# getanteon/alaz

Measured on AMD Instinct MI355X. Metric: L7 edge-events/s ingested->scored service-map, higher is better.
Workload: dtype u64; 1 GPU; C3 device-resident replay: 10000 pods / 5000 services / 1000000 edges, 10000000 HTTP l7 events per window already in HBM, 2-layer SAGE + MLP score, partitioned K1 (variant 0, 8-byte records, 512 partitions); 2-batch HBM ring (value excludes PCIe: see end_to_end with --full); events_per_window=10000000, layers=2, windows_in_flight=1, parallelism=1 GPU

## Files before the change

### alaz_amd/csrc/servicegraph.hip

```cpp
#include <hip/hip_runtime.h>
#include <hip/hip_ext.h>

#include <algorithm>
#include <cmath>
#include <cstdio>
#include <cstring>
#include <chrono>
#include <condition_variable>
#include <thread>
#include <mutex>
#include <string>
#include <unordered_map>
#include <vector>

#include <dlfcn.h>

#include "join_host.hpp"
#include "sg_plan.hpp"
#include "sg_kernels.h"
#include "sg_sel.h"
#include "sg_trend.h"
#include "sg_node_trend.h"
#include "sg_rank.h"
#include "sg_incident.h"
// ... 72 lines not shown

    sg_stats st{};
    u64 h_ctr[C_COUNT] = {};
    std::vector<u32> last_obips;
    bool warm_on = true;
    u32 cold_streak = 0;
    u32 kw_epoch = 0;
    u32 in_fused_slices = 0;
    u64 closes = 0; u32 timing_stride = 1;
    u32 obip_streak = 0; u64 plain_left = 0;

    unsigned timing = 0;
    hipEvent_t win_ta = nullptr;
    u32 k6_epoch = 0;
    u32 rp_epoch = 0;

    struct WinSlot {
        Dev d{}; hipStream_t stream = nullptr; u32* ob_list = nullptr; u32* ob_n = nullptr; u64 events_in = 0;
        bool closed = false, plain = false;
        u64 halo_ovf_seen = 0;
        u64* h_note = nullptr; u64 note_seen = 0;
        u64* scr_sum = nullptr; u64* scr_max = nullptr; double* scr_mu = nullptr;
    };
    std::vector<WinSlot> slots = std::vector<WinSlot>(1);
    int cur = 0;
    struct LastRun { int slot = -1; hipStream_t stream = nullptr; } last;
    std::vector<TimingRec> trecs;
    std::vector<hipEvent_t> ev_pool;
    struct Xchg { u32* ob_local = nullptr; u32* ob_all = nullptr; u32* req = nullptr; u32* serve = nullptr; float* rows_out = nullptr; float* rows_in = nullptr; u32 capp = 0, ob_stride = 0; } xc;
    struct SelScratch { sgplan::SelPlan plan; u32* keys = nullptr; u32* hist = nullptr; u32* blk = nullptr; u32* state = nullptr; u64* pairs = nullptr;
                        u64* n = nullptr; u64* h_n = nullptr; hipEvent_t ev = nullptr; bool pending = false; };
    struct Sel : SelScratch { sg_edge_out* stage = nullptr; u32* stage_idx = nullptr; u64 stage_cap = 0; } sel;
    template <class Row>
    struct Baseline { bool on = false; sg_trend_params p{}; sgplan::TrendPlan plan; char* mem = nullptr; TrendSoA buf[2] = {}; u64* ctl = nullptr;
                      u32* blk = nullptr; K8Thread* th = nullptr; std::vector<Row*> rows; std::vector<char> valid; u32 w = 0; hipEvent_t ev = nullptr;
                      bool pending = false; Row* stage = nullptr; u32* stage_idx = nullptr; u64 stage_cap = 0; };
    Baseline<sg_edge_trend> trend;
    struct Vanished { bool on = false; sg_vanished_params p{}; sgplan::VanishedPlan plan; char* mem = nullptr; u32* th = nullptr; u32* blk = nullptr;
                      std::vector<sg_edge_vanished*> rows; std::vector<u64*> count; std::vector<char> valid; } vanished;
    struct RollupState { bool on = false; char* mem = nullptr; u32* dst = nullptr; K9Side* tout = nullptr; K9Side* tin = nullptr;
                         K9Side* part = nullptr; u32* blk = nullptr; std::vector<sg_node_out*> rows; std::vector<u64*> count; std::vector<char> valid;
                         hipEvent_t ev = nullptr; bool pending = false; };
    template <class Plan>
    struct Rollup : RollupState { Plan plan; };
    Rollup<sgplan::NodesPlan> nodes;
    Baseline<sg_node_trend> ntrend;
    template <class Row>
    struct IdxSel : SelScratch { u64* ctr = nullptr; u32* idx = nullptr; Row* stage = nullptr; char* mem = nullptr; u64 stage_rows = 0; };
    using NSel = IdxSel<sg_node_out>;
    NSel nsel;
    struct RankState { bool on = false; sg_rank_params p{}; char* mem = nullptr; u32* pos = nullptr; u32* src = nullptr; u32* dst = nullptr;
                       u64* W = nullptr; u64* R = nullptr; u64* base = nullptr; u64* t = nullptr; u64* part = nullptr; u64* seed_sum = nullptr;
                       sg_node_rank* stage = nullptr; u32* stage_idx = nullptr; std::vector<sg_node_rank*> rows; std::vector<char> valid;
                       hipEvent_t ev = nullptr; bool pending = false; };
    template <class Plan>
    struct Rank : RankState { Plan plan; typename Plan::Weight* w = nullptr; };
    Rank<sgplan::RankPlan> rank;
    struct IncidentState { bool on = false; sg_incident_params p{}; char* mem = nullptr; u32* pos = nullptr; u32* parent = nullptr;
                           u32* flag = nullptr; u32* lab = nullptr; u32* num = nullptr; u32* kinc = nullptr; u32* esrc = nullptr;
                           K12Keys* keys = nullptr; u32* blk = nullptr; u32* stage = nullptr; u32* stage_idx = nullptr;
                           std::vector<sg_incident_out*> rows; std::vector<u64*> count; std::vector<u32*> node_inc; std::vector<char> valid;
                           hipEvent_t ev = nullptr; bool pending = false; };
    template <class Plan>
    struct Incidents : IncidentState { Plan plan; };
    Incidents<sgplan::IncidentPlan> inc;
    struct Tracks { bool on = false; sg_track_params p{}; sgplan::TrackPlan plan; char* mem = nullptr; u32* mtrack = nullptr; u32* mlast = nullptr;
                    sg_track_entry* tab[2] = {nullptr, nullptr}; TrkState* st[2] = {nullptr, nullptr}; u32 cur = 0; u64 w = 0;
                    u32* cand = nullptr; u32* kept = nullptr; u32* moved = nullptr; u32* joined = nullptr; u32* pos = nullptr; u32* tv = nullptr;
                    u64* claim = nullptr; u32* blk = nullptr; std::vector<sg_incident_track*> rows; std::vector<sg_track_entry*> ended;
                    std::vector<u64*> ended_count; std::vector<char> valid; hipEvent_t ev = nullptr; bool pending = false; };
    Tracks trk;
    struct Groups { bool on = false; sg_group_params p{}; sgplan::GroupPlan plan; char* mem = nullptr; u32* map = nullptr; void* keys[2] = {nullptr, nullptr};
                    u32* idx[2] = {nullptr, nullptr}; u32* hist = nullptr; u32* chunkcnt = nullptr; K14Acc* part = nullptr; uint2* meta = nullptr;
                    u32* blk = nullptr; u32* stage = nullptr; u32* stage_idx = nullptr; std::vector<sg_group_edge*> rows; std::vector<u64*> count;
                    std::vector<u32*> row_group, perm; std::vector<char> valid; hipEvent_t ev = nullptr; bool pending = false;
                    std::vector<u32> h_map; u32* h_up = nullptr; hipEvent_t up_ev = nullptr; bool up_pending = false; u32 dirty_lo = 0, dirty_hi = 0;
                    u32 hi_group = 0; } grp;
    Baseline<sg_edge_trend> gtrend;
    Vanished gvanished;
    IdxSel<sg_group_edge> gsel;
    Rollup<sgplan::GroupNodesPlan> gnodes;
    Baseline<sg_node_trend> gntrend;
    NSel gnsel;
    Rank<sgplan::GroupRankPlan> grank;
    Incidents<sgplan::GroupIncidentPlan> ginc;
    Tracks gtrk;
    struct QuantSpace { bool on = false; char* mem = nullptr; u32* pos = nullptr; u32* tgt[2] = {nullptr, nullptr}; u64* part = nullptr;
                        unsigned char* stage = nullptr; u32* stage_idx = nullptr; std::vector<u64*> hist; std::vector<u32*> quant;
                        std::vector<char> valid; hipEvent_t ev = nullptr; bool pending = false; };
    struct Quantiles { sgplan::QuantPlan plan; u32 n_q = 0; u32 qm[SG_Q_MAX] = {}; QuantSpace sp[3]; } qnt;
    struct QuantTrend { u32 qi = 0; Baseline<sg_node_trend> nodes; Baseline<sg_edge_trend> groups; Baseline<sg_node_trend> workloads; } qtr;
};

namespace {

sg_engine::WinSlot& work(sg_engine* e) { return e->slots[e->cur]; }
int ran_slot(const sg_engine* e) { return e->last.slot >= 0 ? e->last.slot : e->cur; }
sg_engine::WinSlot& ran(sg_engine* e) { return e->slots[ran_slot(e)]; }

#define HIP_TRY(e, call)                                                                       \
    do {                                                                                       \
        hipError_t _r = (call);                                                                \
        if (_r != hipSuccess) {                                                                \
            (e)->err = std::string(#call) + ": " + hipGetErrorString(_r);                      \
            return _r == hipErrorOutOfMemory ? SG_ENOMEM : SG_ENODEV;                          \
        }                                                                                      \
    } while (0)

template <typename T>
int dev_alloc(sg_engine* e, T** p, size_t n, int fill = 0) {
    void* q = nullptr;
    size_t bytes = std::max<size_t>(n, 1) * sizeof(T);
    constexpr size_t kArenaMax = (size_t)32 << 20, kArenaChunk = (size_t)256 << 20, kArenaAlign = 4096;
    if (e->plan.arena_on && bytes < kArenaMax) {
        const size_t need = (bytes + kArenaAlign - 1) & ~(kArenaAlign - 1);
        if (need > e->arena_left) {
            void* c = nullptr;
            HIP_TRY(e, hipMalloc(&c, kArenaChunk));
            e->allocs.push_back(c);
            e->arena_base = static_cast<char*>(c); e->arena_left = kArenaChunk;
        }
        q = e->arena_base; e->arena_base += need; e->arena_left -= need;
    } else {
        HIP_TRY(e, hipMalloc(&q, bytes));
        e->allocs.push_back(q);
    }
    HIP_TRY(e, hipMemsetAsync(q, fill, bytes, e->slots[0].stream));
    *p = (T*)q;
    return SG_OK;
}

hipStream_t pick(sg_engine* e, void* s) { return s ? (hipStream_t)s : work(e).stream; }
hipStream_t pick_ran(sg_engine* e, void* s) { return s ? (hipStream_t)s : e->last.slot >= 0 ? e->last.stream : work(e).stream; }

hipEvent_t get_event(sg_engine* e) {
    if (!e->ev_pool.empty()) { hipEvent_t v = e->ev_pool.back(); e->ev_pool.pop_back(); return v; }
    hipEvent_t v; hipEventCreate(&v); return v;
}

struct Timed {
    sg_engine* e; hipStream_t s; TimingRec r; bool on;
    Timed(sg_engine* e_, hipStream_t s_, int kernel) : e(e_), s(s_), on(e_ && ((e_->timing >> kernel) & 1u)) {
        if (on) { r.kernel = kernel; r.a = get_event(e); r.b = get_event(e); hipEventRecord(r.a, s); }
    }
    ~Timed() { if (on) { hipEventRecord(r.b, s); e->trecs.push_back(r); } }
};

static_assert(sgplan::kK1bWarmU == K1B_WARM_U, "sg_plan.hpp's copy of pass B's warm U");
constexpr int k4_threads(int fi, bool proj, bool split) { return split ? (proj ? 512 : 256) : (fi == 32 ? 1024 : 512); }
template <class FnT, const auto& Keys> struct Family { typedef FnT Fn; static constexpr auto& keys = Keys; };
struct K1aWide : Family<K1aFn, sgplan::kK1aWideKeys> { template <size_t I> static Fn at() { constexpr auto k = keys[I]; return k1a_partition<(bool)k[0], (bool)k[1], (bool)k[2]>; } };
struct K1aTile : Family<K1aFn, sgplan::kK1aTileKeys> { template <size_t I> static Fn at() { constexpr auto k = keys[I]; return k1a_tile_partition<k[0], (bool)k[1], k[2]>; } };
struct K1aTeam : Family<K1aFn, sgplan::kK1aTeamKeys> { template <size_t I> static Fn at() { constexpr auto k = keys[I]; return k1a_team_partition<k[0], (bool)k[1], 2, 1024, k[2]>; } };
struct K1bMerge : Family<K1bFn, sgplan::kK1bMergeKeys> { template <size_t I> static Fn at() {
    constexpr auto k = keys[I]; if constexpr (k[2]) return k1b_merge<k[0], (bool)k[1]>; else return k1b_merge_wide<k[0], (bool)k[1]>; } };
struct K1bStream : Family<K1bFn, sgplan::kK1bStreamKeys> { template <size_t I> static Fn at() {
    constexpr auto k = keys[I]; if constexpr (k[4]) return k1b_stream_merge<k[0], k[1], (bool)k[2], k[3]>; else return k1b_stream_merge_wide<k[0], k[1], (bool)k[2], k[3]>; } };
struct K4Layer : Family<K4LayerFn, sgplan::kK4LayerKeys> { template <size_t I> static Fn at() {
    constexpr auto k = keys[I]; return k4_sage_layer<k[0], (bool)k[1], (bool)k[2], k4_threads(k[0], k[2], k[3]), (bool)k[3]>; } };
constexpr K2RowptrFn kK2Rowptr[2] = {k2_rowptr<K2_RP_ROWS, false>, k2_rowptr<K2_RP_ROWS_DH, true>};
constexpr K4GatherFn kK4Gather[2] = {k4_gather<32>, k4_gather<64>};
constexpr K5ProjFn kK5Proj[2] = {k5_node_proj<false>, k5_node_proj<true>};
constexpr K5ScoreFn kK5Score[2] = {k5_edge_score<false>, k5_edge_score<true>};
template <class F, size_t... I>
const std::array<typename F::Fn, sizeof...(I)>& kernel_table(std::index_sequence<I...>) {
    static const std::array<typename F::Fn, sizeof...(I)> t{{F::template at<I>()...}};
    return t;
}
template <class F> const auto& kernel_table() { return kernel_table<F>(std::make_index_sequence<F::keys.size()>{}); }
template <class F, class... A>
typename F::Fn kernel_of(bool& ok, A... args) {
    const int i = sgplan::find_key(F::keys, sgplan::Key<sizeof...(A)>{{(int)args...}});
    if (i < 0) ok = false;
    return i < 0 ? nullptr : kernel_table<F>()[i];
}
template <class... K>
hipError_t lds_limit(size_t bytes, K... kernels) {
    for (const void* f : {reinterpret_cast<const void*>(kernels)...}) {
        const hipError_t r = hipFuncSetAttribute(f, hipFuncAttributeMaxDynamicSharedMemorySize, (int)bytes);
        if (r != hipSuccess) return r;
    }
    return hipSuccess;
}
template <class F>
hipError_t lds_limit_all(size_t bytes) { hipError_t r = hipSuccess; for (const auto f : kernel_table<F>()) if (r == hipSuccess) r = lds_limit(bytes, f); return r; }

int plan_pass_a(sg_engine* e) {
    sgplan::PassA pa = e->pa;
    if (!sgplan::plan_pass_a(e->plan, e->jt.l1_entries, e->jt.blocks_bytes(), e->ov, &pa)) { e->err = "K1 pass A: the join tables' level 1 and the piece counters do not fit a CU's LDS (fewer partitions / IP blocks needed)"; return SG_ENOSPC; }
    const sgplan::PassAKernel k = sgplan::choose_pass_a(e->plan, pa, e->cfg);
    bool ok = true;
    const K1aFn f = k.family == sgplan::K1A_TEAM ? kernel_of<K1aTeam>(ok, k.l2, k.sharded, k.pb)
                  : k.family == sgplan::K1A_TILE ? kernel_of<K1aTile>(ok, k.l2, k.sharded, k.nsub) : kernel_of<K1aWide>(ok, k.l2, k.sharded, k.hist);
    if (!ok) { e->err = "K1 pass A: the library holds no kernel for family " + std::to_string(k.family) + ", level 2 mode " + std::to_string(k.l2); return SG_ENODEV; }
    e->pa = pa; e->kn.k1a = k; e->fn.k1a = f;
    return SG_OK;
}
int resolve_kernels(sg_engine* e) {
    const sgplan::Kernels& k = e->kn;
    sg_engine::Fns& f = e->fn;
    bool ok = true;
    if (k.k1b_family == sgplan::K1B_STREAM) {
        f.k1b = kernel_of<K1bStream>(ok, k.k1b_u, k.k1b_spt, k.k1b_pack, 0, k.k1b_share);
        if (k.k1b_warm) f.k1b_try = kernel_of<K1bStream>(ok, sgplan::kK1bWarmU, k.k1b_spt, k.k1b_pack, 1, k.k1b_share);
        if (k.k1b_warm) f.k1b_cold = kernel_of<K1bStream>(ok, sgplan::kK1bWarmU, k.k1b_spt, k.k1b_pack, 2, k.k1b_share);
    } else if (k.k1b_family == sgplan::K1B_MERGE) f.k1b = kernel_of<K1bMerge>(ok, k.k1b_u, k.k1b_hist, k.k1b_share);
    f.k2_rowptr = kK2Rowptr[k.k2_dh]; f.k5_proj = kK5Proj[k.k5_mfma];
    for (int w = 0; w < 2; w++) for (int pj = 0; pj < 2; pj++) f.k4_layer[w][pj] = kernel_of<K4Layer>(ok, w ? 64 : 32, k.k4_mfma, pj, k.k4_split);
    if (!ok) { e->err = "the library holds no kernel for one of the plan's choices (sg_plan.hpp choose_kernels)"; return SG_ENODEV; }
    return SG_OK;
}


void join_view(const sg_engine* e, Dev& d) {
    d.jl1mask = e->jt.l1_entries - 1;
    d.jl2_words = e->jt.use_blocks ? e->jt.blocks_used * 256u : 0u;
    d.ck_n = e->jt.ck_n;
    d.jstage_bytes = (u32)((size_t)e->jt.l1_entries * 8 + (e->pa.l2_in_lds ? e->jt.blocks_bytes() : 0));
    d.jl2_in_lds = e->pa.l2_in_lds ? 1u : 0u;
    d.k1a_ct = e->pa.k1a_ct;
}

int sync_tables(sg_engine* e, hipStream_t s) {
    sgjoin::Table& jt = e->jt;
    if (!jt.need_full && jt.dirty.empty()) return SG_OK;
    for (hipStream_t ks : e->k1_streams) if (ks != s) { HIP_TRY(e, hipEventRecord(e->k1_ev, ks)); HIP_TRY(e, hipStreamWaitEvent(s, e->k1_ev, 0)); }
    e->k1_streams.clear();
    if (jt.rebuilds == 0 && !jt.rebuild()) { e->err = "join table build failed: raise max_ips"; return SG_ENOSPC; }
    if (jt.need_full) {
        HIP_TRY(e, hipEventSynchronize(e->blob_ev));
        std::memcpy(e->h_blob, jt.blob, (size_t)jt.L.words * 4);
        HIP_TRY(e, hipMemcpyAsync(e->d_blob, e->h_blob, (size_t)jt.L.words * 4, hipMemcpyHostToDevice, s));
        HIP_TRY(e, hipEventRecord(e->blob_ev, s));
        jt.uploaded_full();
        e->st.join_full_uploads++;
    } else {
        std::vector<std::pair<u32, u32>> log;
        jt.take_dirty(log);
        std::unordered_map<u32, u32> last;
        last.reserve(log.size() * 2);
        for (auto& kv : log) last[kv.first] = kv.second;
        const int slot = e->upd_next; e->upd_next = (slot + 1) % kUpdSlots;
        HIP_TRY(e, hipEventSynchronize(e->upd_ev[slot]));
        u32 n = 0;
        for (auto& kv : last) e->h_upd[slot][n++] = make_uint2(kv.first, kv.second);
        HIP_TRY(e, hipMemcpyAsync(e->d_upd[slot], e->h_upd[slot], (size_t)n * sizeof(uint2), hipMemcpyHostToDevice, s));
        hipLaunchKernelGGL(k_join_apply, dim3((n + 255) / 256), dim3(256), 0, s, e->d_blob, (const uint2*)e->d_upd[slot], n);
        HIP_TRY(e, hipEventRecord(e->upd_ev[slot], s));
        e->st.join_word_updates += n;
    }
    HIP_TRY(e, hipEventRecord(e->tab_ev, s));
    e->tab_seq++; e->tab_stream = s;
    return e->plan.variant == 0 ? plan_pass_a(e) : SG_OK;
}
int order_after_tables(sg_engine* e, hipStream_t s) {
    if (e->tab_seq) {
        u64* seen = nullptr;
        for (auto& kv : e->seen_seq) if (kv.first == s) seen = &kv.second;
        if (!seen) { e->seen_seq.push_back({s, 0}); seen = &e->seen_seq.back().second; }
        if (*seen != e->tab_seq) { if (e->tab_stream != s) HIP_TRY(e, hipStreamWaitEvent(s, e->tab_ev, 0)); *seen = e->tab_seq; }
    }
    if (std::find(e->k1_streams.begin(), e->k1_streams.end(), s) == e->k1_streams.end()) e->k1_streams.push_back(s);
    return SG_OK;
}

void rotate_window(sg_engine* e) { e->cur = (e->cur + 1) % (int)e->slots.size(); }

int launch_k1(sg_engine* e, const sg_event* d_ev, size_t n, hipStream_t s) {
    if (n == 0) return SG_OK;
    sg_engine::WinSlot& w = work(e);
    const size_t kMaxHist = (size_t)65535 * 256;
    if (w.d.hist && w.d.variant == 0 && n > kMaxHist) {
        for (size_t o = 0; o < n; o += kMaxHist) { const int rc = launch_k1(e, d_ev + o, std::min(kMaxHist, n - o), s); if (rc) return rc; }
        return SG_OK;
    }
    const size_t kMaxTeam = (size_t)1 << 25;
    if (w.d.variant == 0 && w.d.narrow && e->pa.k1a_team && n > kMaxTeam) {
        for (size_t o = 0; o < n; o += kMaxTeam) { const int rc = launch_k1(e, d_ev + o, std::min(kMaxTeam, n - o), s); if (rc) return rc; }
        return SG_OK;
    }
    int rc = sync_tables(e, s);
    if (rc) return rc;
    if ((rc = order_after_tables(e, s))) return rc;
    if (((e->timing >> 10) & 1u) && w.events_in == 0 && !e->win_ta) { e->win_ta = get_event(e); hipEventRecord(e->win_ta, s); }
    Dev da = w.d;
    join_view(e, da);
    u32 rot0 = w.d.k1a_rot, tb0 = w.d.k1a_ticket_base;
    if (w.d.variant == 0) {
        const bool tk = ((e->timing >> 1) & 1u) && e->closes % e->timing_stride == 0;
        hipEvent_t ta = tk ? get_event(e) : nullptr, tb = tk ? get_event(e) : nullptr;
        da.batch_state = w.events_in == 0 ? 1u : 0u;
        da.k1a_rot = w.d.k1a_rot;
        rot0 = w.d.k1a_rot; tb0 = w.d.k1a_ticket_base;
        if (w.d.narrow && !e->pa.k1a_team) {
            const u64 per = (n + w.d.nwg - 1) / w.d.nwg, chunk = per >= 4096 ? 4096 : (per + 1023) / 1024 * 1024;
            w.d.k1a_rot = (u32)((w.d.k1a_rot + (n + chunk - 1) / chunk) % w.d.nwg);
        }
        if (w.d.narrow && e->pa.k1a_team) {
            w.d.k1a_rot = (u32)((w.d.k1a_rot + k1m_tiles(n, w.d.nwg, e->pa.k1a_teams, e->pa.k1a_nt)) % ((u64)e->pa.k1a_teams * w.d.nwg));
            da.k1a_ticket_base = w.d.k1a_ticket_base;
            {
                const unsigned long long nt_ = k1m_tiles(n, w.d.nwg, e->pa.k1a_teams, e->pa.k1a_nt), units_ = (unsigned long long)e->pa.k1a_teams * w.d.nwg;
                if (!(w.d.ablate & 0x4u)) w.d.k1a_ticket_base += (u32)((nt_ > units_ ? nt_ - units_ : 0) + std::min(units_, nt_));
            }
        }
        const u32 threads = !w.d.narrow ? K1A_THREADS : e->pa.k1a_team ? 1024 : K1T_THREADS;
        hipExtLaunchKernelGGL(e->fn.k1a, dim3(w.d.nwg), dim3(threads), (uint32_t)e->pa.k1a_lds, s, ta, tb, 0u, da, d_ev, (u64)n);
        if (tk) { TimingRec r; r.a = ta; r.b = tb; r.kernel = 1; e->trecs.push_back(r); }
    } else {
        Timed t(e, s, 1);
        u64 want = (n + 255) / 256;
        int grid = (int)std::min<u64>(want, (u64)e->plan.k1_grid);
        hipLaunchKernelGGL(k1_resolve_aggregate, dim3(grid), dim3(256), 0, s, da, d_ev, (u64)n);
    }
    {
        const hipError_t lr = hipGetLastError();
        if (lr != hipSuccess) {
            w.d.k1a_rot = rot0; w.d.k1a_ticket_base = tb0;
            e->err = std::string("K1 pass A launch: ") + hipGetErrorString(lr);
            return lr == hipErrorOutOfMemory ? SG_ENOMEM : SG_ENODEV;
        }
    }
    e->st.events_in += n;
    w.events_in += n;
    return SG_OK;
}

int table_upsert(sg_engine* e, bool svc, u32 ip, u32 node_id, uint8_t kind) {
    if (node_id >= e->cfg.max_known_nodes) { e->err = "node_id beyond max_known_nodes"; return SG_ENOSPC; }
    auto& m = svc ? e->jt.svc_ip : e->jt.pod_ip;
    if (m.find(ip) == m.end() && e->jt.pod_ip.size() + e->jt.svc_ip.size() >= e->cfg.max_ips) { e->err = "join table full (max_ips)"; return SG_ENOSPC; }
    if (!e->jt.upsert(svc, ip, node_id)) { e->err = "join table build failed: raise max_ips"; return SG_ENOSPC; }
    e->jt.set_kind(node_id, kind);
    e->n_known = std::max(e->n_known, node_id + 1);
    return SG_OK;
}

size_t weights_count(u32 L) {
    size_t n = 0;
    for (u32 l = 0; l < L; l++) n += 2 * (size_t)(l == 0 ? SG_F_IN : SG_F_HID) * SG_F_HID + SG_F_HID;
    return n + 2 * SG_F_HID * SG_F_HID + SG_F_EDGE * SG_F_HID + SG_F_HID + SG_F_HID + 1;
}
size_t layer_offset(u32 l) {
    size_t n = 0;
    for (u32 k = 0; k < l; k++) n += 2 * (size_t)(k == 0 ? SG_F_IN : SG_F_HID) * SG_F_HID + SG_F_HID;
    return n;
}

void launch_halo_lists(sg_engine* e, hipStream_t s, u32* req, u32 capp) {
    sg_engine::WinSlot& w = work(e);
    if (e->plan.k6_one_wg) {
        if (w.d.ncap <= K6_FLAGS_LDS) hipLaunchKernelGGL(k6_halo_build_padded<true>, dim3(1), dim3(1024), 0, s, w.d, req, capp);
        else hipLaunchKernelGGL(k6_halo_build_padded<false>, dim3(1), dim3(1024), 0, s, w.d, req, capp);
        return;
    }
    hipLaunchKernelGGL(k6_halo_lists, dim3(((size_t)w.d.ncap + 1023) / 1024), dim3(1024), 0, s, w.d, req, capp, ++e->k6_epoch, 1u);
}
int do_close(sg_engine* e, hipStream_t s, const u32* d_union, const u32* d_union_n, u32 ob_mode = 1, u32 stride = 0, u32 gworld = 0, bool fuse_in = false) {
    sg_engine::WinSlot& w = work(e);
    int rc = sync_tables(e, s);
    if (rc) return rc;
    Dev dloc = w.d;
    if (dloc.warm && w.h_note) {
        volatile u64* note = w.h_note;
        const u64 seq = note[0];
        if (seq != w.note_seen) {
            w.note_seen = seq;
            const u64 v = note[1];
            const u32 cold = (u32)(v & 0xFFu); const bool obip = (v & 0x100ull) != 0;
            e->cold_streak = cold == 2 ? e->cold_streak + 1 : 0;
            e->obip_streak = (cold == 1 && obip) ? e->obip_streak + 1 : 0;
            if (e->cold_streak >= 3) { e->plain_left = 32; e->cold_streak = 0; }
            if (e->obip_streak >= 4) { e->plain_left = 64; e->obip_streak = 0; }
        }
    }
    if (dloc.warm && e->plain_left) { e->plain_left--; dloc.warm = 0; }
    w.plain = w.d.warm && !dloc.warm;
    const u32 par = w.d.k1b_par & 1u;
    if (e->plan.prepare_fold && dloc.k1b_order) { dloc.k1b_cnt += (size_t)par * dloc.np; dloc.k1b_order += (size_t)par * dloc.np; }
    const Dev& d = dloc;
    bool warm_try = d.warm && e->warm_on;
    const u32 wt = warm_try ? 1u : 0u;
    const bool fold = sgplan::close_folds(e->plan, d.warm != 0, warm_try, ob_mode);
    if (!fold) {
        Timed tp(e, s, 2);
        if (ob_mode == 1) hipLaunchKernelGGL(kc_prepare, dim3(1), dim3(1024), 0, s, d, (u64)e->n_known, (u64)e->n_labels_decl, w.ob_list, (const u32*)w.ob_n, e->plan.ob_list_cap, 1u, (const u32*)nullptr, 0u, 0u, wt);
        else if (ob_mode == 0) hipLaunchKernelGGL(kc_prepare, dim3(1), dim3(1024), 0, s, d, (u64)e->n_known, (u64)e->n_labels_decl, const_cast<u32*>(d_union), d_union_n, e->plan.ob_list_cap, 0u, (const u32*)nullptr, 0u, 0u, wt);
        else hipLaunchKernelGGL(kc_prepare, dim3(1), dim3(1024), 0, s, d, (u64)e->n_known, (u64)e->n_labels_decl, w.ob_list, (const u32*)w.ob_n, e->plan.ob_list_cap, 2u, d_union, stride, gworld, wt);
    }
    if (d.variant == 0) {
        const bool tk = ((e->timing >> 7) & 1u) && e->closes % e->timing_stride == 0;
        hipEvent_t ta = tk ? get_event(e) : nullptr, tb = tk ? get_event(e) : nullptr;
        Dev db = d; db.batch_state = w.events_in == 0 ? 2u : 0u;
        db.kept_compact = d.warm;
        const dim3 grid(d.narrow ? d.npb : d.np), block(e->plan.k1b_threads);
        if (d.warm && warm_try) {
            Dev dt = db; dim3 gt = grid;
            if (fold) {
                dt.fold = 1u; dt.warm_try = wt; gt.x += 1;
                dt.pf_n_known = (u64)e->n_known; dt.pf_n_labels_decl = (u64)e->n_labels_decl; dt.pf_list = w.ob_list; dt.pf_list_cap = e->plan.ob_list_cap;
                dt.k1b_cnt_prev = w.d.k1b_order ? w.d.k1b_cnt + (size_t)(par ^ 1u) * d.np : nullptr;
                dt.k1b_order_next = w.d.k1b_order ? w.d.k1b_order + (size_t)(par ^ 1u) * d.np : nullptr;
            }
            hipExtLaunchKernelGGL(e->fn.k1b_try, gt, block, (uint32_t)e->plan.k1b_lds, s, ta, tb, 0u, dt);
            if (tk) { TimingRec r; r.a = ta; r.b = tb; r.kernel = 7; e->trecs.push_back(r); ta = get_event(e); tb = get_event(e); }
        }
        hipExtLaunchKernelGGL(d.warm ? e->fn.k1b_cold : e->fn.k1b, grid, block, (uint32_t)e->plan.k1b_lds, s, ta, tb, 0u, db);
        if (tk) { TimingRec r; r.a = ta; r.b = tb; r.kernel = 7; e->trecs.push_back(r); }
    }
    {
        Timed t(e, s, 2);
        Dev dk = d;
        dk.kept_compact = d.warm;
        if (d.warm) {
            dk.rowptr = d.k_rowptr; dk.col = d.k_col; dk.csr_from = d.k_from; dk.acc_csr = d.k_acc; dk.max_edges = (u64)d.npb * d.pcap;
            dk.st_sum = w.scr_sum; dk.st_max = w.scr_max; dk.row_mu = w.scr_mu; dk.row_sd = w.scr_mu + d.ncap + 1;
        }
        if (d.variant == 1) {
            const u32 ntiles = e->plan.ecap / K2_TILE;
            hipLaunchKernelGGL(k2_edge_count, dim3(ntiles), dim3(256), 0, s, d);
            hipLaunchKernelGGL(k2_scan_tiles, dim3(1), dim3(1024), 0, s, d, ntiles);
            hipLaunchKernelGGL(k2_edge_compact, dim3(ntiles), dim3(256), 0, s, d);
        }
        if (d.dh_g) hipLaunchKernelGGL(k2_deg_hist, dim3(d.dh_g), dim3(K2_DH_THREADS), ((size_t)d.ncap + 1) * sizeof(u32), s, dk);
        const size_t rpr = d.dh_g ? K2_RP_ROWS_DH : K2_RP_ROWS;
        hipLaunchKernelGGL(e->fn.k2_rowptr, dim3(((size_t)d.ncap + rpr) / rpr), dim3(1024), 0, s, dk, ++e->rp_epoch);
        if (d.variant == 1) hipLaunchKernelGGL(k2_scatter_table, dim3(grid_for(e->cfg.max_edges, 256)), dim3(256), 0, s, d);
        else hipLaunchKernelGGL(k2_scatter_parts, dim3(d.npb), dim3(256), 0, s, dk);
        hipLaunchKernelGGL(k2_rowsort_gather, dim3(std::max(2, std::min(4096, 2 * K2_LONG_WGS + grid_for(d.ncap, 8)))), dim3(256), 2 * (size_t)d.k2_sortw * sizeof(u32), s, dk);
        if (d.warm) {
            const unsigned kg = (unsigned)(((u64)d.npb * d.pcap + KW_CH - 1) / KW_CH) + KW_CAPW;
            hipLaunchKernelGGL(kw_compact, dim3(kg), dim3(KW_THREADS), (size_t)KW_ROWS * 5 * sizeof(u64), s, d, ++e->kw_epoch, dk.st_sum, dk.st_max, (u64)(e->closes + 1), e->slots.size() > 1 ? 1u : 0u);
        }
    }
    {
        Timed t3(e, s, 8);
        const u32 fin = d.warm ? (u32)std::min<u64>(64, ((u64)d.ncap + 255) / 256) : 1u;
        if (fuse_in && e->plan.k3_fuse_allowed) {
            const u32 finp = d.warm ? (fin + 3) / 4 : 1u;
            hipLaunchKernelGGL(k3_in_part, dim3(e->plan.k3_ranges * e->plan.k3_slices + finp), dim3(1024), e->plan.k3in_lds, s, d, e->plan.k3_slices, finp);
            e->in_fused_slices = e->plan.k3_slices;
        } else {
            hipLaunchKernelGGL(k3_in_part, dim3(e->plan.k3_ranges * e->plan.k3_slices), dim3(1024), e->plan.k3in_lds, s, d, e->plan.k3_slices, 0u);
            hipLaunchKernelGGL(k3_in_reduce, dim3(grid_for((u64)d.ncap * 6, 256, 1024) + fin), dim3(256), 0, s, d, e->plan.k3_slices, fin);
            e->in_fused_slices = 0;
        }
    }
    HIP_TRY(e, hipGetLastError());
    w.closed = true;
    w.events_in = 0;
    e->closes++;
    if (e->plan.prepare_fold) w.d.k1b_par ^= 1u;
    return SG_OK;
}

int do_features(sg_engine* e, hipStream_t s) {
    const Dev& d = work(e).d;
    Timed t(e, s, 3);
    const int nbn = grid_for(d.ncap, 128), nbe = grid_for(e->cfg.max_edges, 256, 4096);
    hipLaunchKernelGGL(k3_node_features, dim3(nbn + nbe), dim3(256), 0, s, d, (u32)nbn, e->in_fused_slices);
// ... 1217 lines not shown
    return copy_counted(e, x.count[e->cur], x.rows[e->cur], sizeof(sg_incident_out), out, cap, n);
}
int node_incident_read(sg_engine* e, const NodeSpace& ns, const char* call, const uint32_t* node_index, size_t n_index, uint32_t* out, size_t cap, size_t* n) {
    const sg_engine::IncidentState& x = *ns.inc;
    if (const int rc = stage_ready(e, x, call, ns.inc_w)) return rc;
    u64 cnt = 0;
    HIP_TRY(e, hipMemcpy(&cnt, ns.roll->count[e->cur], sizeof(u64), hipMemcpyDeviceToHost));
    const std::string beyond = std::string(call) + ": a node index beyond the window's " + ns.rows_of;
    return copy_indexed(e, (const u32*)x.node_inc[e->cur], (size_t)cnt, node_index, n_index, out, cap, n, x.stage, x.stage_idx,
                        std::max<size_t>(ns.cap, 1), beyond.c_str());
}
int incidents_buffer(sg_engine* e, const NodeSpace& ns, const char* call, void** d_incidents, void** d_count, void** d_node_incident) {
    const sg_engine::IncidentState& x = *ns.inc;
    int slot;
    if (const int rc = stage_slot(e, x, call, ns.inc_w, &slot)) return rc;
    *d_incidents = x.rows[slot]; *d_count = x.count[slot]; *d_node_incident = x.node_inc[slot];
    return SG_OK;
}
template <class MakePlan>
int tracks_set(sg_engine* e, const NodeSpace& ns, const char* call, const sg_track_params* p, u32 ncap, MakePlan plan) {
    if (!ns.inc->on) { e->err = std::string(call) + ": " + ns.inc_w.off; return SG_ESTATE; }
    if (e->closing || e->flush_open) { e->err = std::string(call) + " while a flush is open"; return SG_ESTATE; }
    sg_track_params q{};
    if (p && sgplan::check_tracks(*p, ncap, &q)) { e->err = std::string(call) + ": bad parameters"; return SG_EINVAL; }
    sg_engine::Tracks& x = *ns.trk;
    free_stage(x);
    if (!p) return SG_OK;
    const u32 slots = (u32)e->slots.size();
    x.p = q;
    x.plan = plan(q.max_tracks, slots);
    const sgplan::TrackPlan& P = x.plan;
    HIP_TRY(e, hipEventCreateWithFlags(&x.ev, hipEventDisableTiming));
    if (const int rc = alloc_block(e, &x.mem, P.total_bytes, call, [&x] { free_stage(x); })) return rc;
    x.mtrack = at<u32>(x.mem, P.member_off[0]); x.mlast = at<u32>(x.mem, P.member_off[1]);
    for (int k = 0; k < 2; k++) { x.tab[k] = at<sg_track_entry>(x.mem, P.table_off[k]); x.st[k] = at<TrkState>(x.mem, P.state_off[k]); }
    x.cand = at<u32>(x.mem, P.inc_off[0]); x.kept = at<u32>(x.mem, P.inc_off[1]); x.moved = at<u32>(x.mem, P.inc_off[2]);
    x.joined = at<u32>(x.mem, P.inc_off[3]); x.pos = at<u32>(x.mem, P.inc_off[4]); x.tv = at<u32>(x.mem, P.inc_off[5]);
    x.claim = at<u64>(x.mem, P.claim_off);
    x.blk = at<u32>(x.mem, P.blk_off);
    for (u32 k = 0; k < slots; k++) {
        char* s = x.mem + P.slot.off + k * P.slot.bytes;
        x.rows.push_back(at<sg_incident_track>(s, P.slot_rows)); x.ended.push_back(at<sg_track_entry>(s, P.slot_ended));
        x.ended_count.push_back(at<u64>(s, P.slot_count));
    }
    hipError_t rc = hipMemset(x.mtrack, 0xFF, P.member_bytes);
    if (rc == hipSuccess) rc = hipDeviceSynchronize();
    if (rc != hipSuccess) { free_stage(x); e->err = std::string(call) + ": hipMemset: " + hipGetErrorString(rc); return SG_ENODEV; }
    x.valid.assign(slots, 0);
    x.on = true;
    return SG_OK;
}
int tracks_read(sg_engine* e, const NodeSpace& ns, const char* call, sg_incident_track* out, size_t cap, size_t* n) {
    const sg_engine::Tracks& x = *ns.trk;
    if (const int rc = stage_ready(e, x, call, ns.trk_w)) return rc;
    return copy_counted(e, ns.inc->count[e->cur], x.rows[e->cur], sizeof(sg_incident_track), out, cap, n);
}
int tracks_ended(sg_engine* e, const NodeSpace& ns, const char* call, sg_track_entry* out, size_t cap, size_t* n) {
    const sg_engine::Tracks& x = *ns.trk;
    if (const int rc = stage_ready(e, x, call, ns.trk_w)) return rc;
    return copy_counted(e, x.ended_count[e->cur], x.ended[e->cur], sizeof(sg_track_entry), out, cap, n);
}
int tracks_buffer(sg_engine* e, const NodeSpace& ns, const char* call, void** d_tracks, void** d_ended, void** d_ended_count) {
    const sg_engine::Tracks& x = *ns.trk;
    int slot;
    if (const int rc = stage_slot(e, x, call, ns.trk_w, &slot)) return rc;
    *d_tracks = x.rows[slot]; *d_ended = x.ended[slot]; *d_ended_count = x.ended_count[slot];
    return SG_OK;
}
int track_state(sg_engine* e, const NodeSpace& ns, const char* call, TrkState* st) {
    sg_engine::Tracks& x = *ns.trk;
    if (!x.on) { e->err = std::string(call) + ": " + ns.trk_w.off; return SG_ESTATE; }
    if (x.pending) HIP_TRY(e, hipEventSynchronize(x.ev));
    HIP_TRY(e, hipMemcpy(st, x.st[x.cur], sizeof(TrkState), hipMemcpyDeviceToHost));
    return SG_OK;
}
int track_entries(sg_engine* e, const NodeSpace& ns, const char* call, sg_track_entry* out, size_t cap, size_t* n) {
    TrkState st{};
    if (const int rc = track_state(e, ns, call, &st)) return rc;
    const sg_engine::Tracks& x = *ns.trk;
    if (n) *n = st.n;
    const size_t take = std::min((size_t)st.n, cap);
    if (out && take) HIP_TRY(e, hipMemcpy(out, x.tab[x.cur], take * sizeof(sg_track_entry), hipMemcpyDeviceToHost));
    return SG_OK;
}
int track_stats(sg_engine* e, const NodeSpace& ns, const char* call, sg_track_stats* out) {
    TrkState st{};
    if (const int rc = track_state(e, ns, call, &st)) return rc;
    out->windows = ns.trk->w; out->live = st.n; out->opened = st.opened; out->dropped_cap = st.dropped;
    return SG_OK;
}
}

extern "C" {

uint32_t sg_abi_version(void) { return SG_ABI_VERSION; }
size_t sg_weights_count(uint32_t layers) { return weights_count(layers); }
uint32_t sg_hash32(uint32_t x) { return sg_fmix32(x); }

const char* sg_last_error(sg_handle h) { return h ? h->err.c_str() : "null handle"; }

int sg_create(const sg_config* cfg_in, sg_handle* out) {
    if (!cfg_in || !out) return SG_EINVAL;
    *out = nullptr;
    sg_config c;
    if (const int rc = sgplan::check_config(*cfg_in, &c)) return rc;
    const sg_config* cfg = &c;
    int ndev = 0;
    if (hipGetDeviceCount(&ndev) != hipSuccess || ndev <= 0 || cfg->device < 0 || cfg->device >= ndev) return SG_ENODEV;
    hipDeviceProp_t prop;
    if (hipGetDeviceProperties(&prop, cfg->device) != hipSuccess) return SG_ENODEV;
    if (std::strncmp(prop.gcnArchName, "gfx950", 6) != 0) return SG_ENODEV;
    sg_engine* e = new sg_engine();
    e->cfg = *cfg;
    auto fail = [&](int rc) { std::fprintf(stderr, "sg_create: %s\n", e->err.c_str()); sg_destroy(e); return rc; };
#define CR(call) do { int _rc = (call); if (_rc) return fail(_rc); } while (0)
#define CH(call) do { hipError_t _r = (call); if (_r != hipSuccess) { e->err = std::string(#call) + ": " + hipGetErrorString(_r); return fail(_r == hipErrorOutOfMemory ? SG_ENOMEM : SG_ENODEV); } } while (0)
#ifdef SG_DEV_KNOBS
    e->ov = sgplan::from_env();
#endif
    sgplan::DeviceFacts facts;
    facts.cus = prop.multiProcessorCount; facts.lds_bytes = kLdsBytes;
    CR(sgplan::make_plan(*cfg, facts, e->ov, &e->plan, &e->err));
    const sgplan::Plan& P = e->plan;
    CH(hipSetDevice(cfg->device));
    e->slots.resize(P.n_slots);
    CH(hipStreamCreateWithFlags(&e->slots[0].stream, hipStreamNonBlocking));
    CH(hipEventCreateWithFlags(&e->tab_ev, hipEventDisableTiming));

    Dev base{}; Dev& d = base;
    sgplan::plan_to_dev(P, *cfg, d);
    const u64 ME = cfg->max_edges;
    {
        const sgjoin::Layout L = sgjoin::Table::make_layout(cfg->max_ips, cfg->max_known_nodes, P.max_blocks);
        e->jt_mirror.assign(L.words, 0);
        e->jt.init(L, e->jt_mirror.data(), d.variant == 0);
        e->jt.max_dirty = kUpdCap;
        CR(dev_alloc(e, &e->d_blob, L.words));
        CH(hipHostMalloc((void**)&e->h_blob, (size_t)L.words * 4));
        CH(hipEventCreateWithFlags(&e->blob_ev, hipEventDisableTiming));
        CH(hipEventCreateWithFlags(&e->k1_ev, hipEventDisableTiming));
        for (int i = 0; i < kUpdSlots; i++) {
            CH(hipHostMalloc((void**)&e->h_upd[i], (size_t)2 * kUpdCap * sizeof(uint2)));
            CR(dev_alloc(e, &e->d_upd[i], (size_t)2 * kUpdCap));
            CH(hipEventCreateWithFlags(&e->upd_ev[i], hipEventDisableTiming));
        }
        d.jl1 = reinterpret_cast<const u64*>(e->d_blob + L.off_l1);
        d.jl2 = e->d_blob + L.off_l2;
        d.iptab = reinterpret_cast<const u64*>(e->d_blob + L.off_ck); d.ipmask = L.ipcap - 1;
        d.iptab2 = reinterpret_cast<const u64*>(e->d_blob + L.off_ck2); d.ipmask2 = L.ip2cap - 1;
        d.kind = reinterpret_cast<const uint8_t*>(e->d_blob + L.off_kind);
    }
    if (d.variant == 0) {
        CR(plan_pass_a(e));
        CH(lds_limit_all<K1aWide>(kLdsBytes)); CH(lds_limit_all<K1aTile>(kLdsBytes)); CH(lds_limit_all<K1aTeam>(kLdsBytes));
        CH(lds_limit_all<K1bMerge>(P.k1b_lds)); CH(lds_limit_all<K1bStream>(P.k1b_lds));
        CH(lds_limit((size_t)KW_ROWS * 5 * sizeof(u64), kw_compact));
    }
    e->kn = sgplan::choose_kernels(P, e->pa, *cfg);
    CR(resolve_kernels(e));
    CH(lds_limit(2 * (size_t)d.k2_sortw * sizeof(u32), k2_rowsort_gather));
    if (d.dh_g) CH(lds_limit(((size_t)d.ncap + 1) * sizeof(u32), k2_deg_hist));
    CH(lds_limit(P.k3in_lds, k3_in_part));
    CR(dev_alloc(e, &d.dbg, (size_t)4 * 4096 * 8));
    CR(dev_alloc(e, &d.clk, (size_t)4));
    CR(dev_alloc(e, &e->d_W, weights_count(cfg->layers)));
    d.W = e->d_W;
    {
        float* tab = nullptr;
        CR(dev_alloc(e, &tab, (size_t)SG_L1P_TAB));
        hipLaunchKernelGGL(k_l1p_table, dim3((SG_L1P_TAB + 255) / 256), dim3(256), 0, e->slots[0].stream, tab);
        CH(hipStreamSynchronize(e->slots[0].stream));
        d.l1p_tab = tab;
    }
    auto alloc_window = [&](sg_engine::WinSlot& slot) -> int {
        Dev& w = slot.d;
#define LR(call) do { int _rc = (call); if (_rc) return _rc; } while (0)
        size_t eslots = ME;
        if (w.variant == 0) {
            eslots = std::max<size_t>(ME, (size_t)w.npb * w.pcap);
            if (w.narrow) { LR(dev_alloc(e, &w.slab8, (size_t)w.np * w.nwg * w.punits)); LR(dev_alloc(e, &w.hdr8, (size_t)w.np * w.nwg));
                            if (P.k1b_order) {
                                const size_t halves = P.prepare_fold ? 2 : 1;
                                LR(dev_alloc(e, &w.k1b_cnt, halves * w.np)); LR(dev_alloc(e, &w.k1b_order, halves * w.np));
                                std::vector<u32> ident(halves * w.np);
                                for (size_t i = 0; i < ident.size(); i++) ident[i] = (u32)(i % w.np);
                                HIP_TRY(e, hipStreamSynchronize(e->slots[0].stream));
                                HIP_TRY(e, hipMemcpy(w.k1b_order, ident.data(), ident.size() * sizeof(u32), hipMemcpyHostToDevice));
                            } }
            else { LR(dev_alloc(e, &w.slab_s, (size_t)w.np * w.nwg * w.pslots)); LR(dev_alloc(e, &w.hdr, (size_t)w.np * w.nwg)); }
            LR(dev_alloc(e, &w.ovf, (size_t)w.ovf_cap * 9));
            LR(dev_alloc(e, &w.ovf_p, (size_t)w.ovf_cap));
            LR(dev_alloc(e, &w.part_n, w.npb));
            LR(dev_alloc(e, &w.acc_src, (size_t)w.npb * w.pcap * 4));
            LR(dev_alloc(e, &w.e_rank, (size_t)w.npb * w.pcap));
            if (w.dh_g) LR(dev_alloc(e, &w.dh_hist, (size_t)w.dh_g * w.dh_ns));
            if (w.warm) {
                const size_t KC = (size_t)w.npb * w.pcap;
                LR(dev_alloc(e, &w.wk_keys, (size_t)w.npb * w.k1b_ht, 0xFF)); LR(dev_alloc(e, &w.wk_pos, (size_t)w.npb * w.k1b_ht, 0xFF));
                LR(dev_alloc(e, &w.pos_of_slot, KC, 0xFF));
                LR(dev_alloc(e, &w.k_acc, KC * 4)); LR(dev_alloc(e, &w.k_col, KC)); LR(dev_alloc(e, &w.k_from, KC)); LR(dev_alloc(e, &w.k_rowptr, (size_t)w.ncap + 2));
                LR(dev_alloc(e, &w.kw_tot, (KC + KW_CH - 1) / KW_CH + 2));
                LR(dev_alloc(e, &w.k_col2, KC)); LR(dev_alloc(e, &w.k_from2, KC)); LR(dev_alloc(e, &w.k_rowptr2, (size_t)w.ncap + 2));
                LR(dev_alloc(e, &w.k_slot, 2 * KC));
                LR(dev_alloc(e, &w.dc_rowptr, (size_t)w.ncap + 2)); LR(dev_alloc(e, &w.dc_col, KC)); LR(dev_alloc(e, &w.dc_from, KC)); LR(dev_alloc(e, &w.dc_acc, KC * 4));
                LR(dev_alloc(e, &w.dc_slot, KC)); LR(dev_alloc(e, &w.dc_ip, KC)); LR(dev_alloc(e, &w.dl_img, KC));
                LR(dev_alloc(e, &w.deg2, ((size_t)w.ncap + 1) * SG_DEG_REP * SG_DEG_STRIDE));
                LR(dev_alloc(e, &slot.scr_sum, (size_t)w.ncap * SG_NODE_STAT_SUM_WORDS)); LR(dev_alloc(e, &slot.scr_max, (size_t)w.ncap * SG_NODE_STAT_MAX_WORDS)); LR(dev_alloc(e, &slot.scr_mu, 2 * ((size_t)w.ncap + 1)));
                void* dn = nullptr;
                HIP_TRY(e, hipHostMalloc((void**)&slot.h_note, 64, hipHostMallocMapped));
                slot.h_note[0] = slot.h_note[1] = 0;
                HIP_TRY(e, hipHostGetDevicePointer(&dn, slot.h_note, 0));
                w.host_note = (u64*)dn;
            }
        }
        const size_t KE = P.kept_edges;
        LR(dev_alloc(e, &w.ekeys, P.ecap, 0xFF));
        LR(dev_alloc(e, &w.eacc, (size_t)P.ecap * 4));
        if (w.variant == 1) w.acc_src = w.eacc;
        LR(dev_alloc(e, &w.obkeys, P.obcap));
        LR(dev_alloc(e, &w.wgstat, (size_t)SG_MAX_K1_WGS * WS_WORDS));
        LR(dev_alloc(e, &w.ctr, C_COUNT));
        LR(dev_alloc(e, &w.ob_sorted, w.max_obip));
        LR(dev_alloc(e, &slot.ob_list, P.ob_list_cap));
        LR(dev_alloc(e, &slot.ob_n, 4));
        LR(dev_alloc(e, &w.tile_cnt, P.ecap / K2_TILE));
        LR(dev_alloc(e, &w.tile_off, P.ecap / K2_TILE));
        LR(dev_alloc(e, &w.e_slot, ME)); LR(dev_alloc(e, &w.e_from, eslots)); LR(dev_alloc(e, &w.e_to, eslots));
        LR(dev_alloc(e, &w.longrows, (size_t)w.ncap + 1));
        LR(dev_alloc(e, &w.deg, ((size_t)w.ncap + 1) * SG_DEG_REP * SG_DEG_STRIDE)); LR(dev_alloc(e, &w.rp_tot, ((size_t)w.ncap + K2_RP_ROWS_DH) / K2_RP_ROWS_DH + 1)); LR(dev_alloc(e, &w.k6_tot, (((size_t)w.ncap + 1023) / 1024 + 1) * 16)); LR(dev_alloc(e, &w.k1a_ticket, 4)); LR(dev_alloc(e, &w.lb_ticket, 4)); w.k1a_ticket_base = 0; w.k1a_rot = 0; LR(dev_alloc(e, &w.rowptr, (size_t)w.ncap + 1)); LR(dev_alloc(e, &w.cursor, (size_t)w.ncap + 1));
        LR(dev_alloc(e, &w.col, ME)); LR(dev_alloc(e, &w.cs, KE)); LR(dev_alloc(e, &w.csr_from, ME));
        LR(dev_alloc(e, &w.sort_k, 2 * KE)); LR(dev_alloc(e, &w.sort_v, 2 * KE));
        LR(dev_alloc(e, &w.acc_csr, ME * 4));
        if (w.hist) { LR(dev_alloc(e, &w.hist_src, (w.variant == 0 ? (size_t)w.npb * w.pcap : (size_t)P.ecap) * SG_HIST_BINS)); LR(dev_alloc(e, &w.hist_csr, ME * SG_HIST_BINS)); }
        LR(dev_alloc(e, &w.st_sum, (size_t)w.ncap * SG_NODE_STAT_SUM_WORDS)); LR(dev_alloc(e, &w.st_max, (size_t)w.ncap * SG_NODE_STAT_MAX_WORDS));
        LR(dev_alloc(e, &w.x0, (size_t)w.ncap * SG_F_IN));
        for (u32 l = 1; l <= cfg->layers; l++) LR(dev_alloc(e, &w.h[l], (size_t)w.ncap * SG_F_HID));
        LR(dev_alloc(e, &w.P, (size_t)w.ncap * SG_F_HID)); LR(dev_alloc(e, &w.Q, (size_t)w.ncap * SG_F_HID));
        LR(dev_alloc(e, &w.nmean, (size_t)w.ncap * SG_F_HID));
        LR(dev_alloc(e, &w.hub_items, w.hub_cap)); LR(dev_alloc(e, &w.hub_base, (size_t)w.ncap + 1)); LR(dev_alloc(e, &w.hub_part, (size_t)w.hub_cap * SG_F_HID));
        LR(dev_alloc(e, &w.efeat, ME * SG_F_EDGE)); LR(dev_alloc(e, &w.latz, ME)); LR(dev_alloc(e, &w.errr, ME));
        LR(dev_alloc(e, &w.row_mu, (size_t)w.ncap + 1)); LR(dev_alloc(e, &w.row_sd, (size_t)w.ncap + 1));
        LR(dev_alloc(e, &w.rows, ME));
        LR(dev_alloc(e, &w.in_part, (size_t)P.k3_ranges * P.k3_slices * K3_IN_NR * 6));
        LR(dev_alloc(e, &w.alive_keys, w.alive_cap)); LR(dev_alloc(e, &w.alive_csr, KE));
        LR(dev_alloc(e, &w.act_l, (size_t)w.ncap + 1)); LR(dev_alloc(e, &w.act_p, (size_t)w.ncap + 1));
        std::vector<u64> init((size_t)SG_MAX_K1_WGS * WS_WORDS, 0);
        for (int i = 0; i < SG_MAX_K1_WGS; i++) init[(size_t)i * WS_WORDS + WS_TMIN] = ~0ull;
        HIP_TRY(e, hipMemcpy(w.wgstat, init.data(), init.size() * sizeof(u64), hipMemcpyHostToDevice));
#undef LR
        return SG_OK;
    };
    CH(hipStreamSynchronize(e->slots[0].stream));
    for (sg_engine::WinSlot& slot : e->slots) {
        slot.d = base;
        if (!slot.stream) CH(hipStreamCreateWithFlags(&slot.stream, hipStreamNonBlocking));
        CR(alloc_window(slot));
    }
    CH(hipStreamCreateWithFlags(&e->copy_stream, hipStreamNonBlocking)); CH(hipStreamCreateWithFlags(&e->copy_stream2, hipStreamNonBlocking));
    CH(hipStreamCreateWithFlags(&e->rd_stream, hipStreamNonBlocking)); CH(hipEventCreateWithFlags(&e->score_ev, hipEventDisableTiming));
    CH(hipHostMalloc((void**)&e->h_ctr_pin, sizeof(e->h_ctr)));
    for (int i = 0; i < P.n_stage; i++) {
        CH(hipEventCreateWithFlags(&e->copied_ev[i], hipEventDisableTiming));
        CH(hipHostMalloc((void**)&e->h_stage[i], (size_t)e->cfg.max_batch * sizeof(sg_event)));
        CR(dev_alloc(e, &e->d_stage[i], e->cfg.max_batch));
        CH(hipEventCreateWithFlags(&e->stage_ev[i], hipEventDisableTiming));
    }
    CH(hipDeviceSynchronize());
#undef CR
#undef CH
    *out = e;
    return SG_OK;
}

int sg_destroy(sg_handle e) {
    if (!e) return SG_EINVAL;
    hipDeviceSynchronize();
    for (sg_engine::WinSlot& w : e->slots) { if (w.stream) hipStreamDestroy(w.stream); if (w.h_note) hipHostFree(w.h_note); }
    for (void* p : e->allocs) hipFree(p);
    if (e->h_blob) hipHostFree(e->h_blob);
    for (int i = 0; i < kUpdSlots; i++) { if (e->h_upd[i]) hipHostFree(e->h_upd[i]); if (e->upd_ev[i]) hipEventDestroy(e->upd_ev[i]); }
    if (e->blob_ev) hipEventDestroy(e->blob_ev);
    if (e->k1_ev) hipEventDestroy(e->k1_ev);
    for (int i = 0; i < kStageSlots; i++) { if (e->h_stage[i]) hipHostFree(e->h_stage[i]); if (e->stage_ev[i]) hipEventDestroy(e->stage_ev[i]); if (e->copied_ev[i]) hipEventDestroy(e->copied_ev[i]); }
    for (auto& r : e->registered) hipHostUnregister(const_cast<char*>(r.first));
    if (e->copy_stream) hipStreamDestroy(e->copy_stream);
    if (e->copy_stream2) hipStreamDestroy(e->copy_stream2);
    if (e->rd_stream) hipStreamDestroy(e->rd_stream);
    if (e->score_ev) hipEventDestroy(e->score_ev);
    for (auto& r : e->w_readers) hipEventDestroy(r.second);
    if (e->h_ctr_pin) hipHostFree(e->h_ctr_pin);
    if (e->h_rows) hipHostFree(e->h_rows);
    if (e->h_rows_old) hipHostFree(e->h_rows_old);
    if (e->sel.stage) hipFree(e->sel.stage);
    if (e->sel.stage_idx) hipFree(e->sel.stage_idx);
    if (e->sel.h_n) hipHostFree(e->sel.h_n);
    if (e->sel.ev) hipEventDestroy(e->sel.ev);
    free_edge_trend(edge_space(e));
    free_nodes(e);
    free_groups(e);
    free_idxsel(e->nsel);
    free_idxsel(e->gsel);
    for (auto& r : e->trecs) { hipEventDestroy(r.a); hipEventDestroy(r.b); }
    for (auto v : e->ev_pool) hipEventDestroy(v);
    if (e->tab_ev) hipEventDestroy(e->tab_ev);
    delete e;
    return SG_OK;
}

int sg_geometry_get(sg_handle e, sg_geometry* out) {
    if (!e || !out) return SG_EINVAL;
    std::lock_guard<std::mutex> g(e->mu);
    const sgplan::Plan& p = e->plan; const sgplan::PassA& a = e->pa;
    out->k1_variant = p.variant; out->k1_narrow = p.narrow; out->partitions = p.np; out->table_slots = p.k1b_ht; out->pass_b_split = p.k1b_split;
    out->pass_a_workgroups = p.nwg; out->cache_slots = a.k1a_ct; out->join_l2_in_lds = a.l2_in_lds ? (p.narrow && a.l2_u16 ? 2u : 1u) : 0u;
    out->tile_records = p.narrow ? (a.k1a_team ? 4u * a.k1a_nt / a.k1a_teams : K1T_TS(a.k1a_nsub)) : 0u; out->pass_a_teams = p.narrow && a.k1a_team ? a.k1a_teams : 0u; out->endpoint_bits = p.narrow ? p.nb : 0u;
    out->piece_bytes = p.variant != 0 ? 0u : (p.narrow ? p.punits * 8u : p.pslots * 16u);
    out->warm_windows = p.warm;
    return SG_OK;
}

int sg_prepare_fold_get(sg_handle e, uint32_t* out) {
    if (!e || !out) return SG_EINVAL;
    std::lock_guard<std::mutex> g(e->mu);
    *out = e->plan.prepare_fold ? 1u : 0u;
    return SG_OK;
}

int sg_upsert_pod(sg_handle e, uint32_t ip, uint32_t node_id) {
    if (!e) return SG_EINVAL;
    std::lock_guard<std::mutex> g(e->mu);
    return table_upsert(e, false, ip, node_id, SG_NODE_POD);
}
int sg_upsert_service(sg_handle e, uint32_t ip, uint32_t node_id) {
    if (!e) return SG_EINVAL;
    std::lock_guard<std::mutex> g(e->mu);
    return table_upsert(e, true, ip, node_id, SG_NODE_SERVICE);
}
int sg_delete_pod(sg_handle e, uint32_t ip) {
    if (!e) return SG_EINVAL;
    std::lock_guard<std::mutex> g(e->mu);
    if (!e->jt.erase(false, ip)) { e->err = "join table rebuild failed"; return SG_ENOSPC; }
    return SG_OK;
}
int sg_delete_service(sg_handle e, uint32_t ip) {
    if (!e) return SG_EINVAL;
    std::lock_guard<std::mutex> g(e->mu);
    if (!e->jt.erase(true, ip)) { e->err = "join table rebuild failed"; return SG_ENOSPC; }
    return SG_OK;
}

int sg_set_clock(sg_handle e, uint64_t first_kernel_ns, uint64_t first_user_ns) {
    if (!e) return SG_EINVAL;
    std::lock_guard<std::mutex> g(e->mu);
    e->first_kernel = first_kernel_ns; e->first_user = first_user_ns;
    return SG_OK;
}

int sg_set_label_count(sg_handle e, uint32_t n_labels) {
    if (!e) return SG_EINVAL;
    std::lock_guard<std::mutex> g(e->mu);
    if (n_labels > e->cfg.max_labels) { e->err = "label count beyond max_labels"; return SG_ENOSPC; }
    e->n_labels_decl = std::max(e->n_labels_decl, n_labels);
    return SG_OK;
}

int sg_load_weights(sg_handle e, const float* w, size_t n) {
    if (!e || !w) return SG_EINVAL;
    std::lock_guard<std::mutex> g(e->mu);
    if (n != weights_count(e->cfg.layers)) { e->err = "weight count mismatch"; return SG_EINVAL; }
    for (auto& r : e->w_readers) HIP_TRY(e, hipEventSynchronize(r.second));
    for (auto& r : e->w_readers) hipEventDestroy(r.second);
    e->w_readers.clear();
    HIP_TRY(e, hipMemcpy(e->d_W, w, n * sizeof(float), hipMemcpyHostToDevice));
    e->have_w = true;
    return SG_OK;
}

namespace {
int stage_take(sg_engine* e) {
    for (int k = 0; k < e->plan.n_stage; k++) {
        const int c = (e->stage_next + k) % e->plan.n_stage;
        if (!e->stage_busy[c] && hipEventQuery(e->stage_ev[c]) != hipErrorNotReady) { e->stage_busy[c] = true; e->stage_next = (c + 1) % e->plan.n_stage; e->pending_copies++; return c; }
    }
    return -1;
}
hipStream_t stage_stream(sg_engine* e) { return (e->plan.n_copy == 2 && (e->copy_rr++ & 1)) ? e->copy_stream2 : e->copy_stream; }
int stage_finish(sg_engine* e, int slot, size_t n, hipStream_t cs, bool copy_ok) {
    sg_engine::WinSlot& w = work(e);
    int rc = SG_OK;
    if (!copy_ok) { e->err = "hipMemcpyAsync (staging ring)"; rc = SG_ENODEV; }
    if (rc == SG_OK) {
        hipEventRecord(e->copied_ev[slot], cs);
        hipStreamWaitEvent(w.stream, e->copied_ev[slot], 0);
        e->st.h2d_bytes += n * sizeof(sg_event);
        rc = launch_k1(e, e->d_stage[slot], n, w.stream);
    }
    hipEventRecord(e->stage_ev[slot], w.stream);
    e->stage_busy[slot] = false; e->pending_copies--;
    e->cv.notify_all();
    return rc;
}
int stage_submit(sg_engine* e, int slot, const sg_event* src, size_t n) {
    hipStream_t cs = stage_stream(e);
    const bool ok = hipMemcpyAsync(e->d_stage[slot], src, n * sizeof(sg_event), hipMemcpyHostToDevice, cs) == hipSuccess;
    return stage_finish(e, slot, n, cs, ok);
}
constexpr size_t kStagePiece = ((size_t)4 << 20) / sizeof(sg_event);
}

int sg_ingest(sg_handle e, const sg_event* events, size_t n) {
    if (!e || (!events && n)) return SG_EINVAL;
    std::unique_lock<std::mutex> g(e->mu);
    if (n > e->cfg.max_batch) { e->err = "batch larger than max_batch"; return SG_EINVAL; }
    if (n == 0) return SG_OK;
    if (e->closing) { e->st.ingest_waits++; e->cv.wait(g, [&] { return !e->closing; }); }
    const int slot = stage_take(e);
    if (slot < 0) {
        e->st.events_dropped_ring += n;
        return SG_EAGAIN;
    }
    hipStream_t cs = stage_stream(e);
    g.unlock();
    bool ok = true;
    for (size_t o = 0; o < n && ok; o += kStagePiece) {
        const size_t m = std::min(kStagePiece, n - o);
        std::memcpy(e->h_stage[slot] + o, events + o, m * sizeof(sg_event));
        ok = hipMemcpyAsync(e->d_stage[slot] + o, e->h_stage[slot] + o, m * sizeof(sg_event), hipMemcpyHostToDevice, cs) == hipSuccess;
    }
    g.lock();
    return stage_finish(e, slot, n, cs, ok);
}

int sg_ingest_pinned(sg_handle e, const sg_event* events, size_t n) {
    if (!e || (!events && n)) return SG_EINVAL;
    std::unique_lock<std::mutex> g(e->mu);
    if (n > e->cfg.max_batch) { e->err = "batch larger than max_batch"; return SG_EINVAL; }
    if (n == 0) return SG_OK;
    {
        const char* p = reinterpret_cast<const char*>(events);
        bool ok = false;
        for (auto& r : e->registered) ok |= p >= r.first && p + n * sizeof(sg_event) <= r.first + r.second;
        if (!ok) { e->err = "sg_ingest_pinned: the events are not inside memory registered with sg_host_register"; return SG_EINVAL; }
    }
    if (e->closing) { e->st.ingest_waits++; e->cv.wait(g, [&] { return !e->closing; }); }
    const int slot = stage_take(e);
    if (slot < 0) { e->st.events_dropped_ring += n; return SG_EAGAIN; }
    return stage_submit(e, slot, events, n);
}
int sg_ingest_bulk(sg_handle e, const sg_event* events, size_t n, int pinned, uint64_t* retries) {
    if (!e || (!events && n)) return SG_EINVAL;
    const size_t step = e->cfg.max_batch;
    uint64_t waits = 0;
    for (size_t o = 0; o < n; o += step) {
        const size_t m = std::min(step, n - o);
        for (;;) {
            const int rc = pinned ? sg_ingest_pinned(e, events + o, m) : sg_ingest(e, events + o, m);
            if (rc == SG_OK) break;
            if (rc != SG_EAGAIN) { if (retries) *retries = waits; return rc; }
            { std::lock_guard<std::mutex> g(e->mu); e->st.events_dropped_ring -= m; }
            waits++;
            std::this_thread::sleep_for(std::chrono::microseconds(20));
        }
    }
    if (retries) *retries = waits;
    return SG_OK;
}
int sg_host_register(sg_handle e, void* p, size_t bytes) {
    if (!e || !p || !bytes) return SG_EINVAL;
    std::lock_guard<std::mutex> g(e->mu);
    if (hipHostRegister(p, bytes, hipHostRegisterDefault) != hipSuccess) { e->err = "hipHostRegister failed"; return SG_ENOMEM; }
    e->registered.push_back({reinterpret_cast<const char*>(p), bytes});
    return SG_OK;
}
int sg_host_unregister(sg_handle e, void* p) {
    if (!e || !p) return SG_EINVAL;
    std::lock_guard<std::mutex> g(e->mu);
    for (size_t i = 0; i < e->registered.size(); i++) if (e->registered[i].first == reinterpret_cast<const char*>(p)) {
        hipDeviceSynchronize();
        hipHostUnregister(p);
        e->registered.erase(e->registered.begin() + (long)i);
// ... 1497 lines not shown
```

### alaz_amd/csrc/sg_k1_team.h

```cpp
#pragma once

#define K1M_OOB     0x80000000u
#define K1M_RARE    0xFFFFFFFEu

static inline unsigned long long k1m_tiles(unsigned long long n, unsigned nwg, unsigned teams, unsigned nt) {
    const unsigned long long units = (unsigned long long)teams * nwg, tt = nt / teams, per = (n + units - 1) / units;
    const unsigned long long grp = per >= 4 * tt ? 4 * tt : (per + tt - 1) / tt * tt;
    return (n + grp - 1) / grp;
}
template <int L2M, bool SHARDED, int TEAMS, int NT, int NPB>
__global__ __launch_bounds__(NT) void k1a_team_partition(Dev d, const sg_event* __restrict__ ev, u64 n) {
    constexpr u32 K1M_THREADS = NT;
    constexpr u32 K1M_TILE_ALL = 4 * NT;
    constexpr u32 K1M_TT = K1M_THREADS / TEAMS;
    constexpr u32 K1M_TW = K1M_TT / 64;
    constexpr u32 K1M_GROUP = 4 * K1M_TT;
    constexpr u32 K1M_TS = K1M_TILE_ALL / TEAMS;
    constexpr u32 K1M_NR = 4;
    extern __shared__ __attribute__((aligned(16))) unsigned char smem[];
    const u32 CT = d.k1a_ct;
    constexpr u32 NP = 1u << NPB;
    u32* fcn = reinterpret_cast<u32*>(smem);
    u32* fcw = fcn + NP;
    u32* tcnt = fcw + NP;
    u64* red = reinterpret_cast<u64*>(tcnt + 4 * TEAMS * NP);
    u32* bar = reinterpret_cast<u32*>(red + 8);
    u64* tiles = reinterpret_cast<u64*>(bar + 16);
    uint4* jl = reinterpret_cast<uint4*>(tiles + K1M_TILE_ALL + 4);
    const u32 jl1_bytes = (d.jl1mask + 1) * 8u;
    const u32 jlds = L2M == 2 ? jl1_bytes + ((d.jstage_bytes - jl1_bytes) >> 1) : d.jstage_bytes;
    u64* ckey = reinterpret_cast<u64*>(reinterpret_cast<unsigned char*>(jl) + ((jlds + 15u) & ~15u));
    u64* cacc = ckey + CT;
    const u64* l1 = reinterpret_cast<const u64*>(jl);
    const u32* l2 = L2M == 1 ? reinterpret_cast<const u32*>(l1 + d.jl1mask + 1) : d.jl2;
    const unsigned short* l2h = reinterpret_cast<const unsigned short*>(l1 + d.jl1mask + 1);
    const u32 w = blockIdx.x, t = threadIdx.x, lane = t & 63u;
    const u32 wave_all = (u32)__builtin_amdgcn_readfirstlane((int)(t >> 6)), team = TEAMS == 2 ? (wave_all >= K1M_TW ? 1u : 0u) : 0u, wv = wave_all - team * K1M_TW;
    const u32 tt = t - team * K1M_TT;
    u32* bcnt = tcnt + team * 4 * NP;
    u32* boff = bcnt + 2 * NP;
    u32* pbase = boff + NP;
    u64* tile = tiles + team * (K1M_TS + 2);
    u32* mybar = bar + 8 * team;
    const uint4* __restrict__ pe = reinterpret_cast<const uint4*>(ev);
    const u32 units = (u32)TEAMS * d.nwg;
    const u64 per = (n + units - 1) / units;
    const u32 grp = per >= K1M_GROUP ? K1M_GROUP : (u32)((per + K1M_TT - 1) / K1M_TT * K1M_TT);
    const u64 ngroup = (n + grp - 1) / grp, ntile = ngroup;
    const u32 rot = d.k1a_rot % units;
    const u32 unit = (team * d.nwg + w + units - rot) % units, unit_other = ((1u - team) * d.nwg + w + units - rot) % units;
    const bool first = d.batch_state == 1u;
    if ((u64)unit >= ntile && (TEAMS == 1 || (u64)unit_other >= ntile)) {
        if (first) for (u32 p = t; p < NP; p += K1M_THREADS) d.hdr8[(size_t)p * d.nwg + w] = make_uint2(0u, 0u);
        return;
    }
    SG_STAMP(d, 0, 0);
    auto kd = [&]() -> const Dev& {
        const __attribute__((address_space(4))) Dev* kp = (const __attribute__((address_space(4))) Dev*)__builtin_amdgcn_kernarg_segment_ptr();
        asm volatile("" : "+s"(kp));
        return *(const Dev*)kp;
    };
    const bool clk_me = w == 0 && t == 0;
    const u64 clk_c0 = clk_me ? __builtin_readcyclecounter() : 0ull, clk_r0 = clk_me ? wall_clock64() : 0ull;
    u32 st_acc = 0, st_dsrc = 0, st_maxlabel = 0, st_misr = 0; u64 st_tmin = ~0ull, st_tmax = 0;
    const u32 nb = d.nb, nbmask = (1u << nb) - 1u, pshift = nb - d.pb, rbmask = (1u << d.rb) - 1u, bmask = CT / 2 - 1, jm = d.jl1mask;
    const u32 max_known = d.max_known, max_labels = d.max_labels, sn = d.sn;
    const bool ck_any = d.ck_n != 0;
    u32 bar_target = 0;
    auto team_barrier = [&]() {
        if constexpr (TEAMS == 1) { lds_barrier(); return; }
        bar_target += K1M_TW;
        asm volatile("s_waitcnt lgkmcnt(0)" : : : "memory");
        if (lane == 0) __hip_atomic_fetch_add(mybar, 1u, __ATOMIC_RELAXED, __HIP_MEMORY_SCOPE_WORKGROUP);
        while ((int)(lds_fresh_u32(mybar) - bar_target) < 0) __builtin_amdgcn_s_sleep(1);
        asm volatile("" : : : "memory");
    };

    auto general = [&](const u64 idx) {
        const Dev& d = kd();
        const uint4* q2 = pe + 2 * idx;
        const uint4 xa = q2[0], xb = q2[1];
        K1Ev e;
        K1Local L;
        const bool ok = k1_resolve(d, xa, xb, L, e);
        if (!ok) { k1_red_add(red, L); return; }
        u32 Lm, Rm;
        sg_kmix(ci_of_ref(d, (u32)(e.key >> 32)), ci_of_ref(d, (u32)e.key), nbmask, &Lm, &Rm);
        const u32 part = Lm >> pshift;
        const u64 mk = ((u64)Lm << nb) | Rm;
        if (e.alive) { emit_wide(d, fcw, w, part, mk, 0ull, 0u, 1u, L); k1_red_add(red, L); return; }
        const u32 bkt = Rm & bmask;
        const int slot = cache_claim(ckey, bkt, mk, lds_fresh_u64(&ckey[2 * bkt]), lds_fresh_u64(&ckey[2 * bkt + 1]));
        if (slot >= 0) k1a_cache_add<false>(cacc, (u32)slot, e.dur, e.err);
        else if (e.dur >> 32) emit_wide(d, fcw, w, part, mk, e.dur, e.err, 0u, L);
        else emit_narrow_direct(d, fcn, w, part, (u32)mk & rbmask, (u32)e.dur, e.err, L);
        k1_red_add(red, L);
    };
    constexpr u32 KSH = L2M == 2 ? 14u : 30u, IDM = L2M == 2 ? 0x3FFFu : 0x3FFFFFFFu;

#define K1M_F_ACC 1u
#define K1M_F_RARE 2u
#define K1M_F_ERR 4u
    auto front2 = [&](const u32 tq, const u32 i0, const u32 gcount, const v4u_t A0, const v4u_t B0, const v4u_t A1, const v4u_t B1,
                      u32 (&Lm)[2], u32 (&Rm)[2], u32 (&dur)[2], u32 (&fl)[2]) {
        const v4u_t A[2] = {A0, A1}, B[2] = {B0, B1};
        u32 vs[2], vd[2];
        {
            u64 s1[2], s2[2], d1[2], d2[2];
#pragma unroll
            for (int i = 0; i < 2; i++) {
                const u32 b = A[i].x >> 8, c = A[i].y >> 8;
                s1[i] = l1[(__umul24(b, SG_JL1_K1) >> 9) & jm]; s2[i] = l1[(__umul24(b, SG_JL1_K2) >> 11) & jm];
                d1[i] = l1[(__umul24(c, SG_JL1_K1) >> 9) & jm]; d2[i] = l1[(__umul24(c, SG_JL1_K2) >> 11) & jm];
            }
#pragma unroll
            for (int i = 0; i < 2; i++) {
                const u32 b = A[i].x >> 8, c = A[i].y >> 8;
                const u32 blk = (u32)s1[i] == b ? (u32)(s1[i] >> 32) : ((u32)s2[i] == b ? (u32)(s2[i] >> 32) : 0u);
                const u32 blkd = (u32)d1[i] == c ? (u32)(d1[i] >> 32) : ((u32)d2[i] == c ? (u32)(d2[i] >> 32) : 0u);
                const u32 ix = (blk << 8) | (A[i].x & 255u), ixd = (blkd << 8) | (A[i].y & 255u);
                vs[i] = L2M == 2 ? (u32)l2h[ix] : l2[ix];
                vd[i] = L2M == 2 ? (u32)l2h[ixd] : l2[ixd];
            }
        }
#pragma unroll
        for (int i = 0; i < 2; i++) {
            const bool inr = tq + (i0 + (u32)i) * K1M_TT < gcount;
            const u32 flags = A[i].w >> 24, label = A[i].z;
            const u32 ks = vs[i] >> KSH, kd = vd[i] >> KSH;
            bool r = ((flags & SG_EV_ALIVE) != 0) | (ks == 3u) | (kd == 3u) | (B[i].y != 0u) |
                     ((kd == 0u) & ((label == 0u) | (label > max_labels))) | (ck_any & ((vs[i] == 0u) | (vd[i] == 0u)));
            r &= inr;
            const bool fastv = inr & !r;
            bool a = fastv & (ks == 1u);
            st_dsrc += (fastv & (ks != 1u)) ? 1u : 0u;
            u32 cf = vs[i] & IDM;
            u32 ct = kd ? (vd[i] & IDM) : (max_known + label - 1u);
            { const u32 lb = (a & (kd == 0u)) ? label : 0u; st_maxlabel = lb > st_maxlabel ? lb : st_maxlabel; }
            if (flags & SG_EV_REVERSE) { const u32 x_ = cf; cf = ct; ct = x_; }
            if (SHARDED) { const bool mine = (owner_hash_ref(ref_of_ci(d, cf)) % d.world) == d.rank; st_misr += (a & !mine) ? 1u : 0u; a &= mine; }
            const u32 status = A[i].w & 0xFFFFu, proto = (A[i].w >> 16) & 0xFFu;
            const u32 err = is_error(proto, status);
            const u64 wt = (u64)B[i].z | ((u64)B[i].w << 32);
            st_acc += a ? 1u : 0u;
            st_tmin = (a && wt < st_tmin) ? wt : st_tmin; st_tmax = (a && wt > st_tmax) ? wt : st_tmax;
            sg_kmix(cf & nbmask, ct & nbmask, nbmask, &Lm[i], &Rm[i]);
            dur[i] = B[i].x;
            fl[i] = (a ? K1M_F_ACC : 0u) | (r ? K1M_F_RARE : 0u) | (err ? K1M_F_ERR : 0u);
        }
    };
    auto back2 = [&](const u32 (&Lm)[2], const u32 (&Rm)[2], const u32 (&dur)[2], const u32 (&fl)[2], u32* bc, u32* lo, u32* hi, u32* pr) {
        ulonglong2 kk[2]; u64 mk[2];
#pragma unroll
        for (int i = 0; i < 2; i++) { mk[i] = ((u64)Lm[i] << nb) | Rm[i]; kk[i] = reinterpret_cast<const ulonglong2*>(ckey)[Rm[i] & bmask]; }
        int slot[2]; bool claim = false;
#pragma unroll
        for (int i = 0; i < 2; i++) {
            const u32 bk = Rm[i] & bmask;
            slot[i] = kk[i].x == mk[i] ? (int)(2u * bk) : (kk[i].y == mk[i] ? (int)(2u * bk + 1u) : -1);
            claim |= ((fl[i] & K1M_F_ACC) != 0) & (slot[i] < 0) & ((kk[i].x == SG_EKEY_EMPTY) | (kk[i].y == SG_EKEY_EMPTY));
        }
        if (__builtin_amdgcn_ballot_w64(claim)) {
#pragma unroll
            for (int i = 0; i < 2; i++)
                if ((fl[i] & K1M_F_ACC) && slot[i] < 0 && (kk[i].x == SG_EKEY_EMPTY || kk[i].y == SG_EKEY_EMPTY)) slot[i] = cache_claim(ckey, Rm[i] & bmask, mk[i], kk[i].x, kk[i].y);
        }
        u32 rank[2];
#pragma unroll
        for (int i = 0; i < 2; i++) rank[i] = atomicAdd(&bc[Lm[i] >> pshift], ((fl[i] & K1M_F_ACC) && slot[i] < 0) ? 1u : 0u);
#pragma unroll
        for (int i = 0; i < 2; i++) if ((fl[i] & K1M_F_ACC) && slot[i] >= 0) k1a_cache_add<false>(cacc, (u32)slot[i], (u64)dur[i], (fl[i] >> 2) & 1u);
#pragma unroll
        for (int i = 0; i < 2; i++) {
            const bool travel = (fl[i] & K1M_F_ACC) && slot[i] < 0;
            lo[i] = dur[i]; hi[i] = ((u32)mk[i] & rbmask) | ((fl[i] & K1M_F_ERR) ? 0x80000000u : 0u);
            pr[i] = travel ? ((Lm[i] >> pshift) | (rank[i] << K1T_RANK_SHIFT)) : ((fl[i] & K1M_F_RARE) ? K1M_RARE : K1T_NONE);
        }
    };

    {
        for (u32 p = t; p < NP; p += K1M_THREADS) {
            uint2 h = make_uint2(0u, 0u);
            if (!first) h = d.hdr8[(size_t)p * d.nwg + w];
            fcn[p] = h.x; fcw[p] = h.y;
        }
        for (u32 k = t; k < 4 * TEAMS * NP; k += K1M_THREADS) tcnt[k] = 0u;
        for (u32 k = t; k < CT; k += K1M_THREADS) ckey[k] = SG_EKEY_EMPTY;
        for (u32 k = t; k < CT * 4; k += K1M_THREADS) cacc[k] = 0;
        if (t < 8) red[t] = t == WS_TMIN ? ~0ull : 0ull;
        if (t < 16) bar[t] = 0u;
        k1a_stage_join<K1M_THREADS, L2M>(d, jl, t);
        lds_barrier();
        SG_STAMP(d, 0, 1);
    }
    const bool packb = 2u * nb <= 31u;
    const u32 rb = d.rb;
    u64* const slab_w = d.slab8 + (size_t)w * d.punits;
    const u32 nwpun = d.nwg * d.punits;
    const __amdgpu_buffer_rsrc_t slab_rsrc = __builtin_amdgcn_make_buffer_rsrc(slab_w, 0, (int)(u32)(((size_t)NP * d.nwg - w) * d.punits * 8u), 0x00020000);
    auto ovf_record = [&](const u32 b, const u32 remv, const u32 dur, const u32 err) { const Dev& d = kd(); K1Local L; ovf8_single(d, b, ((u64)b << d.rb) | remv, (u64)dur, err, 0u, L); k1_red_add(red, L); };
    auto copy_out = [&](const u32 pc) {
        const u32* bc = bcnt + pc * NP;
        if (packb) {
            u32 tq = tt; asm volatile("" : "+v"(tq));
            const u32 total = boff[NP - 1] + bc[NP - 1];
            const u32 pbm = (1u << d.pb) - 1u, strip = ~(pbm << rb);
            constexpr u32 NPOS = K1M_TS / K1M_TT;
            u64 rec[NPOS]; u32 pb_[NPOS], bo_[NPOS];
#pragma unroll
            for (u32 k = 0; k < NPOS; k++) rec[k] = tile[tq + k * K1M_TT];
#pragma unroll
            for (u32 k = 0; k < NPOS; k++) { const u32 b = ((u32)(rec[k] >> 32) >> rb) & pbm; pb_[k] = pbase[b]; bo_[k] = boff[b]; }
            u32 ovm = 0;
#pragma unroll
            for (u32 k = 0; k < NPOS; k++) {
                const u32 i = tq + k * K1M_TT, h = (u32)(rec[k] >> 32), b = (h >> rb) & pbm;
                const u32 pos = pb_[k] + (i - bo_[k]);
                const bool valid = i < total;
                if SG_ABL(d, 0x2u) { if (valid & (pos < sn)) slab_w[(u64)b * nwpun + pos] = (rec[k] & 0xFFFFFFFFull) | ((u64)(h & strip) << 32); }
                else { v2u_t dv; dv.x = (u32)rec[k]; dv.y = h & strip;
                  __builtin_amdgcn_raw_buffer_store_b64(dv, slab_rsrc, (valid & (pos < sn)) ? (b * nwpun + pos) * 8u : K1M_OOB, 0, 0); }
                ovm |= (valid & (pos >= sn)) ? (1u << k) : 0u;
            }
            if (__builtin_amdgcn_ballot_w64(ovm != 0)) {
#pragma unroll 1
                for (u32 k = 0; k < NPOS; k++) if ((ovm >> k) & 1u) {
                    const u64 r = tile[tq + k * K1M_TT];
                    const u32 h = (u32)(r >> 32);
                    ovf_record((h >> rb) & pbm, h & rbmask, (u32)r, h >> 31);
                }
            }
        } else {
            const u32 bpw = NP / K1M_TW;
#pragma unroll 1
            for (u32 b4 = 0; b4 < bpw; b4 += 4) {
                const u32 b = wv * bpw + b4 + (lane >> 4), j0 = lane & 15u;
                const u32 cnt = bc[b], off = boff[b], pos0 = pbase[b];
                u64* dst = piece8(d, b, w);
#pragma unroll 1
                for (u32 j = j0; j < cnt; j += 16) {
                    const u64 rec = tile[off + j];
                    const u32 pos = pos0 + j;
                    if (pos < sn) dst[pos] = rec;
                    else ovf_record(b, (u32)(rec >> 32) & rbmask, (u32)rec, (u32)(rec >> 63));
                }
            }
        }
    };
    bool havep = false; u32 pcur = 0, cur = 0;
    u64 tk_p1 = 0, tk_wait = 0, tk_scan = 0, tk_p3 = 0, tk_b3 = 0, tk_p4 = 0, tk_ld = 0, tk_fa = 0;
#ifdef SG_K1_PHASE_STAMPS
    const bool stamp = SG_ABL(d, 0x100u) != 0;
#else
    constexpr bool stamp = false;
#endif
    const u32 n32 = (u32)n, ngroup32 = (u32)ngroup;
    auto gbounds = [&](const u32 g, u32& first, u32& count) {
        first = g * grp; count = g < ngroup32 ? (first + grp < n32 ? grp : n32 - first) : 0u;
    };
    const bool dyn = !SG_ABL(d, 0x4u);
    u32* nxt2 = bar + 8 * team + 4;
    const u32 ntile32 = (u32)ntile;
    for (u32 j = unit; j < ntile32; cur ^= 1u) {
        u32* bc = bcnt + cur * NP;
        u32 lo[K1M_NR], hi[K1M_NR], pr[K1M_NR];
        u32 ttl = tt, lanel = lane; asm volatile("" : "+v"(ttl), "+v"(lanel));
        const u64 tk0 = stamp ? wall_clock64() : 0ull;
        {
            if (havep) { const u64 tq = stamp ? wall_clock64() : 0ull; copy_out(pcur); if (stamp) tk_p4 += wall_clock64() - tq; }
            u32 f0, c0;
            gbounds(j, f0, c0);
            v4u_t eaa0, eba0, eaa1, eba1, eaa2, eba2, eaa3, eba3;
            {
                const u32 x0 = ttl, x1 = x0 + K1M_TT, x2 = x1 + K1M_TT, x3 = x2 + K1M_TT, fb = f0 * 32u;
                const u32 o0 = x0 < c0 ? fb + x0 * 32u : 0u, o1 = x1 < c0 ? fb + x1 * 32u : 0u, o2 = x2 < c0 ? fb + x2 * 32u : 0u, o3 = x3 < c0 ? fb + x3 * 32u : 0u;
#define K1M_LD2(A, B, vo) asm volatile("global_load_dwordx4 %0, %2, %3\n\tglobal_load_dwordx4 %1, %2, %3 offset:16" : "=&v"(A), "=&v"(B) : "v"(vo), "s"(pe) : "memory")
                K1M_LD2(eaa0, eba0, o0); K1M_LD2(eaa1, eba1, o1); K1M_LD2(eaa2, eba2, o2); K1M_LD2(eaa3, eba3, o3);
#undef K1M_LD2
            }
            u32 tkv = 0;
            const bool drawer = dyn && wv == 0 && lanel == 0;
            if (drawer) asm volatile("global_atomic_add %0, %1, %2, off sc0" : "=&v"(tkv) : "v"(d.k1a_ticket), "v"(1u) : "memory");
            const u64 tl0 = stamp ? wall_clock64() : 0ull;
            asm volatile("s_waitcnt vmcnt(0)" : "+v"(eaa0), "+v"(eba0), "+v"(eaa1), "+v"(eba1), "+v"(eaa2), "+v"(eba2), "+v"(eaa3), "+v"(eba3), "+v"(tkv) : : "memory");
            if (stamp) tk_ld += wall_clock64() - tl0;
            if (drawer) { asm volatile("" : "+v"(tkv)); nxt2[cur] = tkv - d.k1a_ticket_base + units; }
            {
                u32 Lm[2], Rm[2], du[2], fl[2];
                front2(ttl, 0u, c0, eaa0, eba0, eaa1, eba1, Lm, Rm, du, fl);
                back2(Lm, Rm, du, fl, bc, lo, hi, pr);
            }
            __builtin_amdgcn_sched_barrier(0);
            {
                u32 Lm[2], Rm[2], du[2], fl[2];
                front2(ttl, 2u, c0, eaa2, eba2, eaa3, eba3, Lm, Rm, du, fl);
                back2(Lm, Rm, du, fl, bc, lo + 2, hi + 2, pr + 2);
            }
        }
        const u64 tk1 = stamp ? wall_clock64() : 0ull;
        team_barrier();
        const u64 tk2 = stamp ? wall_clock64() : 0ull;
        tk_p1 += tk1 - tk0; tk_wait += tk2 - tk1;
        {
            constexpr u32 pl = NP >> 6; const u32 b0 = lanel * pl;
            const bool own = (lanel % K1M_TW) == wv;
            u32* bprev = bcnt + (cur ^ 1u) * NP;
            if constexpr ((pl & 3u) == 0 && pl <= 16) {
                constexpr u32 nq = pl >> 2;
                uint4 cq[4];
                u32 s = 0;
#pragma unroll
                for (u32 k = 0; k < 4; k++) { cq[k] = k < nq ? reinterpret_cast<const uint4*>(bc + b0)[k] : make_uint4(0u, 0u, 0u, 0u); s += cq[k].x + cq[k].y + cq[k].z + cq[k].w; }
                const u32 incl = wave_incl_scan_u32(s, lanel);
                u32 run = incl - s;
                uint4 pbv[4];
                if (own) {
#pragma unroll
                    for (u32 k = 0; k < 4; k++) if (k < nq) {
                        pbv[k].x = atomicAdd(&fcn[b0 + 4 * k], cq[k].x); pbv[k].y = atomicAdd(&fcn[b0 + 4 * k + 1], cq[k].y);
                        pbv[k].z = atomicAdd(&fcn[b0 + 4 * k + 2], cq[k].z); pbv[k].w = atomicAdd(&fcn[b0 + 4 * k + 3], cq[k].w);
                    }
                }
#pragma unroll
                for (u32 k = 0; k < 4; k++) if (k < nq) {
                    uint4 o; o.x = run; run += cq[k].x; o.y = run; run += cq[k].y; o.z = run; run += cq[k].z; o.w = run; run += cq[k].w;
                    reinterpret_cast<uint4*>(boff + b0)[k] = o;
                }
                if (own) {
#pragma unroll
                    for (u32 k = 0; k < 4; k++) if (k < nq) {
                        reinterpret_cast<uint4*>(pbase + b0)[k] = pbv[k];
                        reinterpret_cast<uint4*>(bprev + b0)[k] = make_uint4(0u, 0u, 0u, 0u);
                    }
                }
            } else {
                u32 s = 0;
                for (u32 k = 0; k < pl; k++) s += bc[b0 + k];
                const u32 incl = wave_incl_scan_u32(s, lane);
                u32 run = incl - s;
                for (u32 k = 0; k < pl; k++) {
                    const u32 c = bc[b0 + k]; boff[b0 + k] = run; run += c;
                    if (own) { pbase[b0 + k] = atomicAdd(&fcn[b0 + k], c); bprev[b0 + k] = 0u; }
                }
            }
        }
        const u64 tk3 = stamp ? wall_clock64() : 0ull;
        {
            u32 of_[K1M_NR];
#pragma unroll
            for (int i = 0; i < (int)K1M_NR; i++) of_[i] = boff[pr[i] < K1M_RARE ? (pr[i] & ((1u << K1T_RANK_SHIFT) - 1u)) : 0u];
#pragma unroll
            for (int i = 0; i < (int)K1M_NR; i++) {
                const u32 pt_ = pr[i] & ((1u << K1T_RANK_SHIFT) - 1u);
                const u32 at = pr[i] < K1M_RARE ? of_[i] + (pr[i] >> K1T_RANK_SHIFT) : K1M_TS;
                tile[at] = (u64)lo[i] | ((u64)(hi[i] | (packb ? pt_ << rb : 0u)) << 32);
            }
        }
        const u64 tk4 = stamp ? wall_clock64() : 0ull;
        team_barrier();
        const u64 tk5 = stamp ? wall_clock64() : 0ull;
        {
            u32 rmask = 0;
#pragma unroll
            for (int i = 0; i < (int)K1M_NR; i++) rmask |= (pr[i] == K1M_RARE) ? (1u << i) : 0u;
            if (__builtin_amdgcn_ballot_w64(rmask != 0)) {
                const u64 e0 = (u64)j * grp + ttl;
#pragma unroll 1
                for (u32 k = 0; k < K1M_NR; k++) if ((rmask >> k) & 1u) general(e0 + (u64)k * K1M_TT);
            }
        }
        {
            const u64 tmin = wave_min_u64(st_tmin), tmax = wave_max_u64(st_tmax);
            const u32 ac = wave_sum_u32(st_acc);
            if (lanel == 0 && ac) { atomicMin(&red[WS_TMIN], tmin); atomicMax(&red[WS_TMAX], tmax); atomicAdd(&red[WS_ACCEPTED], (u64)ac); }
            if (__builtin_amdgcn_ballot_w64((st_dsrc | st_misr | st_maxlabel) != 0u)) {
                if (st_dsrc) atomicAdd(&red[WS_DROPPED_SRC], (u64)st_dsrc);
                if (st_misr) atomicAdd(&red[WS_MISROUTED], (u64)st_misr);
                if (st_maxlabel) atomicMax(&red[WS_MAXLABEL], (u64)st_maxlabel);
            }
            st_acc = st_dsrc = st_maxlabel = st_misr = 0; st_tmin = ~0ull; st_tmax = 0;
        }
        havep = true; pcur = cur;
        if (stamp) { tk_scan += tk3 - tk2; tk_p3 += tk4 - tk3; tk_b3 += tk5 - tk4; }
        j = dyn ? (u32)__builtin_amdgcn_readfirstlane((int)lds_fresh_u32(nxt2 + cur)) : j + units;
    }
    if (havep) copy_out(pcur);
    SG_STAMP(d, 0, 3);
    if (stamp && tt == 0 && blockIdx.x < 2048) { u64* g = d.dbg + ((size_t)2 * 4096 + blockIdx.x * 2 + team) * 8; g[0] = tk_p1; g[1] = tk_wait; g[2] = tk_scan; g[3] = tk_p3; g[4] = tk_b3; g[5] = tk_p4; g[6] = tk_ld; g[7] = tk_fa; }
    lds_barrier();
    SG_STAMP(d, 0, 4);
    {
    const Dev& d = kd();
    K1Local L;
    for (u32 s = t; s < CT; s += K1M_THREADS) {
        const u64 k = ckey[s];
        if (k == SG_EKEY_EMPTY) continue;
        const u64 x0 = cacc[s * 4];
        const u32 part = (u32)(k >> d.rb), rem = (u32)k & rbmask;
        if ((x0 & 0xFFFFFFFFull) == 1ull) {
            const u64 dur = cacc[s * 4 + 1];
            if (dur >> 32) emit_wide(d, fcw, w, part, k, dur, (u32)(x0 >> 32), 0u, L);
            else emit_narrow_direct(d, fcn, w, part, rem, (u32)dur, (u32)(x0 >> 32), L);
        } else if ((x0 & 0xFFFFFFFFull) != 0ull) emit_agg8(d, fcw, w, part, k, x0, cacc[s * 4 + 1], cacc[s * 4 + 2], cacc[s * 4 + 3], L, first);
    }
    k1_red_add(red, L);
    {
        const u64 tmin = wave_min_u64(st_tmin), tmax = wave_max_u64(st_tmax);
        const u32 ac = wave_sum_u32(st_acc), ds = wave_sum_u32(st_dsrc), mr = wave_sum_u32(st_misr);
        const u32 ml = (u32)wave_max_u64((u64)st_maxlabel);
        if (lane == 0) {
            if (ac) { atomicMin(&red[WS_TMIN], tmin); atomicMax(&red[WS_TMAX], tmax); atomicAdd(&red[WS_ACCEPTED], (u64)ac); }
            if (ds) atomicAdd(&red[WS_DROPPED_SRC], (u64)ds);
            if (mr) atomicAdd(&red[WS_MISROUTED], (u64)mr);
            if (ml) atomicMax(&red[WS_MAXLABEL], (u64)ml);
        }
    }
    lds_barrier();
    for (u32 p = t; p < NP; p += K1M_THREADS) { const u32 c = fcn[p]; d.hdr8[(size_t)p * d.nwg + w] = make_uint2(c < sn ? c : sn, fcw[p]); }
    SG_STAMP(d, 0, 5);
    if (t == 0) k1_publish_wg(d, red);
    SG_STAMP(d, 0, 6);
    if (clk_me) { atomicAdd(&d.clk[0], __builtin_readcyclecounter() - clk_c0); atomicAdd(&d.clk[1], wall_clock64() - clk_r0); }
    }
}
```

### alaz_amd/csrc/sg_plan.hpp

```cpp
#pragma once
#include <algorithm>
#include <array>
#include <cmath>
#include <cstdint>
#include <cstdlib>
#include <cstring>
#include <initializer_list>
#include <optional>
#include <string>
#include <vector>

#include "../../include/servicegraph.h"
#include "sg_sizes.h"

namespace sgplan {

typedef uint32_t u32;
typedef uint64_t u64;

constexpr size_t kLdsBytes = 160 * 1024;
constexpr int kStageSlots = 32;
constexpr size_t kPrepareLds = 4096;

inline u32 next_pow2(u64 v) { u64 p = 1; while (p < v) p <<= 1; return (u32)p; }
inline int grid_for(u64 items, int per_block, int cap = 2048) {
    u64 g = (items + per_block - 1) / per_block;
    return (int)std::max<u64>(1, std::min<u64>(g, (u64)cap));
}

struct DeviceFacts {
    int cus = 256;
    size_t lds_bytes = kLdsBytes;
};

struct Overrides {
    typedef std::optional<std::string> Knob;
    Knob ablate, np, ht, ct, nwg, nsub, split, warm, k1a, k1_narrow, k1_legacy, k1b_u, k1b_threads, k1b_pack, k1b_no_order,
         l2_global, l2_u32, dh_g, k3_slices, k3_no_fuse, k4_fused, k5_grid, k6_one_wg, dense_valu, copy_streams, stage_slots, arena, no_fold;
};
struct KnobName { const char* name; Overrides::Knob Overrides::*field; };
constexpr KnobName kKnobs[] = {
    {"SG_ABLATE", &Overrides::ablate}, {"SG_NP", &Overrides::np}, {"SG_HT", &Overrides::ht}, {"SG_CT", &Overrides::ct},
    {"SG_NWG", &Overrides::nwg}, {"SG_NSUB", &Overrides::nsub}, {"SG_SPLIT", &Overrides::split}, {"SG_WARM", &Overrides::warm},
    {"SG_K1A", &Overrides::k1a}, {"SG_K1_NARROW", &Overrides::k1_narrow}, {"SG_K1_LEGACY", &Overrides::k1_legacy},
    {"SG_K1B_U", &Overrides::k1b_u}, {"SG_K1B_THREADS", &Overrides::k1b_threads}, {"SG_K1B_PACK", &Overrides::k1b_pack},
    {"SG_K1B_NO_ORDER", &Overrides::k1b_no_order}, {"SG_L2_GLOBAL", &Overrides::l2_global}, {"SG_L2_U32", &Overrides::l2_u32},
    {"SG_DH_G", &Overrides::dh_g}, {"SG_K3_SLICES", &Overrides::k3_slices}, {"SG_K3_NO_FUSE", &Overrides::k3_no_fuse},
    {"SG_K4_FUSED", &Overrides::k4_fused}, {"SG_K5_GRID", &Overrides::k5_grid}, {"SG_K6_ONE_WG", &Overrides::k6_one_wg},
    {"SG_DENSE_VALU", &Overrides::dense_valu}, {"SG_COPY_STREAMS", &Overrides::copy_streams}, {"SG_STAGE_SLOTS", &Overrides::stage_slots},
    {"SG_ARENA", &Overrides::arena}, {"SG_NO_FOLD", &Overrides::no_fold},
};
#ifdef SG_DEV_KNOBS
inline Overrides from_env() {
    Overrides o;
    for (const KnobName& k : kKnobs) if (const char* v = std::getenv(k.name)) o.*k.field = std::string(v);
    return o;
}
#endif
inline int ival(const Overrides::Knob& k) { return std::atoi(k->c_str()); }
inline u64 uval(const Overrides::Knob& k) { return std::strtoull(k->c_str(), nullptr, 0); }

struct Plan {
    u32 variant = 0, narrow = 0, hist = 0, agg_slots = 3, nb = 0, np = 0, pb = 0, nwg = 256, k1b_split = 1, k1b_ht = 0, npb = 0, rb = 0,
        pcap = 0, sa = 0, sn = 0, sw = 0, punits = 0, ss = 0, pslots = 0, ovf_cap = 0, warm = 0;
    u32 k1b_threads = 1024, k1b_u = 4;
    bool k1b_pack = false;
    bool k1b_order = false;
    size_t k1b_lds = 0;
    bool prepare_fold = false;
    u32 ecap = 0, obcap = 0, ob_list_cap = 0, ncap = 0, max_obip = 1, alive_cap = 0, hub_cap = 0, max_blocks = 0;
    u64 kept_edges = 0;
    u32 max_known = 0;
    u32 k3_ranges = 1, k3_slices = 8;
    size_t k3in_lds = 0;
    u32 k2_sortw = 0, dh_g = 0, dh_ppw = 0, dh_ns = 0;
    bool k4_split = false;
    u32 k5_grid = 0;
    bool k3_fuse_allowed = true;
    bool k6_one_wg = false;
    bool use_mfma = true;
    u32 cus = 1;
    int k1_grid = 0, n_copy = 1, n_stage = 16;
    bool arena_on = false;
    u32 n_slots = 1;
    u32 ablate = 0;
};

struct PassA {
    bool l2_u16 = false, k1a_team = false, l2_in_lds = false;
    u32 k1a_nsub = 2, k1a_teams = 2, k1a_nt = 1024, k1a_ct = 2048;
    size_t k1a_lds = 0;
};

inline int check_config(const sg_config& in, sg_config* out) {
    constexpr uint32_t kCfgMin = 88;
    if (in.struct_size < kCfgMin || in.struct_size > 4096) return SG_EINVAL;
    sg_config c; std::memset(&c, 0, sizeof c);
    std::memcpy(&c, &in, std::min<size_t>(in.struct_size, sizeof c));
    c.struct_size = (uint32_t)sizeof c;
    if (c.abi_version != SG_ABI_VERSION || c.layers < 1 || c.layers > SG_MAX_LAYERS || c.max_edges == 0 ||
        c.max_known_nodes == 0 || c.world == 0 || c.rank >= c.world || c.max_known_nodes > 0x3FFFFFFFu)
        return SG_EINVAL;
    if (c.max_batch == 0) c.max_batch = 1u << 20;
    if (c.max_ips == 0) c.max_ips = c.max_known_nodes;
    if (c.max_window_events == 0) c.max_window_events = c.max_batch;
    *out = c;
    return SG_OK;
}

inline int make_plan(const sg_config& cfg, const DeviceFacts& dev, const Overrides& ov, Plan* out, std::string* why) {
    sg_config chk;
    if (check_config(cfg, &chk) != SG_OK) { if (why) *why = "invalid config"; return SG_EINVAL; }
    Plan p;
    const size_t lds = dev.lds_bytes;
    if (ov.arena) p.arena_on = ival(ov.arena) != 0;
    p.k1_grid = std::min<int>(SG_MAX_K1_WGS, dev.cus * 8);
    p.cus = (u32)std::max(1, dev.cus);
    p.use_mfma = !(ov.dense_valu && (*ov.dense_valu)[0] == '1');
    p.max_known = cfg.max_known_nodes;

    const u64 ME = cfg.max_edges;
    p.ecap = next_pow2(std::max<u64>(2 * ME, K2_TILE));
    p.obcap = next_pow2(std::max<u64>(2 * (u64)cfg.max_outbound_ips, 64));
    p.ob_list_cap = next_pow2(std::max<u64>((u64)cfg.max_outbound_ips * std::max<u32>(cfg.world, 1), 64));
    p.max_obip = std::max<u32>(cfg.max_outbound_ips, 1);
    p.ncap = cfg.max_known_nodes + cfg.max_labels + p.max_obip;

    p.variant = cfg.k1_variant == 1 ? 1u : 0u;
    p.hist = (cfg.flags & SG_CFG_EDGE_HISTOGRAM) ? 1u : 0u;
    p.agg_slots = p.hist ? 5u : 3u;
    const u64 cn = (u64)cfg.max_known_nodes + cfg.max_labels + p.obcap;
    u32 nb = 12; while ((1ull << nb) < cn && nb < 31) nb++;
    bool narrow = p.variant == 0 && !p.hist && cfg.k1_variant != 2 && !ov.k1_legacy && nb <= 24;
    const bool small_window = ME < (1ull << 18) && cfg.max_window_events <= (2ull << 20);
    if (cfg.k1_variant == 0 && small_window && !ov.k1_narrow) narrow = false;
    u64 np = 0;
    if (narrow) {
        np = next_pow2(std::max<u64>((ME + 2699) / 2700, 256));
        u32 pbt = 0; while ((1ull << pbt) < np) pbt++;
        if (np > 2048 || 2 * nb - pbt > 31) narrow = false;
    }
    p.k1b_split = 1;
    if (narrow) {
        if (ME / np > 1150) { p.k1b_split = 2; p.k1b_ht = 2048; }
        else p.k1b_ht = ME / np > 550 ? 2048 : 1024;
        if (ov.split) { const int x = ival(ov.split); if (x == 1 || x == 2) { p.k1b_split = (u32)x; p.k1b_ht = ME / (np * x) > 1150 ? 4096 : (ME / (np * x) > 550 ? 2048 : 1024); } }
    } else {
        np = next_pow2(std::max<u64>((ME + 1249) / 1250, 256));
        if (np > 4096) np = 4096;
        if (cfg.k1_variant != 1 && ME > (u64)4096 * 1400) p.variant = 1;
        p.k1b_ht = ME / np > 600 ? 2048 : 1024;
        if (p.hist && p.k1b_ht == 2048) { p.k1b_ht = 1024; np = std::min<u64>(4096, np * 2); }
    }
    p.np = (u32)np; p.nwg = 256;
    if (ov.np) { const u64 x = uval(ov.np); if (x >= 64 && x <= (narrow ? 2048u : 4096u) && (x & (x - 1)) == 0) p.np = (u32)x; }
    if (ov.ht) { const u64 x = uval(ov.ht); if (x >= 256 && x <= (narrow ? 4096u : 2048u) && (x & (x - 1)) == 0) p.k1b_ht = (u32)x; }
    if (ov.nwg) { const u64 x = uval(ov.nwg); if (x >= 1 && x <= (u64)SG_MAX_K1_WGS) p.nwg = (u32)x; }
    p.pb = 0; while ((1u << p.pb) < p.np) p.pb++;
    if (narrow && 2 * nb - p.pb > 31) { p.np = (u32)np; p.pb = 0; while ((1u << p.pb) < p.np) p.pb++; }
    p.narrow = (narrow && p.variant == 0) ? 1u : 0u;
    if (!p.narrow) p.k1b_split = 1;
    p.warm = (p.narrow && !p.hist && !(cfg.flags & SG_CFG_NO_WARM) && ((cfg.flags & SG_CFG_WARM) || ME >= (1ull << 18))) ? 1u : 0u;
    if (ov.warm) p.warm = (ival(ov.warm) != 0 && p.narrow && !p.hist) ? 1u : 0u;
    p.npb = p.np * p.k1b_split;
    p.nb = nb; p.rb = 2 * nb - p.pb;
    p.pcap = p.narrow ? p.k1b_ht * 13 / 16 : p.k1b_ht * 3 / 4;
    const double m = (double)cfg.max_window_events / ((double)p.np * p.nwg);
    p.sa = std::min<u32>(24, std::max<u32>(8, (2 * 2048 / p.np + 6 + 1) & ~1u));
    if (p.narrow) {
        p.sn = ((u32)(2.0 * m + 8.0 * std::sqrt(m + 1.0) + 24.0) + 1u) & ~1u;
        p.sn = std::min<u32>(p.sn, (1u << 20) - 16);
        p.sw = std::min<u32>(64, std::max<u32>(8, p.sn / 8));
        p.punits = (p.sn + 2 * p.sw + 5 * p.sa + 15) / 16 * 16;
        p.sn = p.punits - 2 * p.sw - 5 * p.sa;
        p.ss = 0; p.pslots = 0;
    } else {
        p.ss = (u32)(2.0 * m + 8.0 * std::sqrt(m + 1.0) + 24.0);
        p.ss = (p.ss + p.agg_slots * p.sa + 7) / 8 * 8 - p.agg_slots * p.sa;
        p.ss = std::min<u32>(p.ss, (1u << 20) - 8);
        p.pslots = p.ss + p.agg_slots * p.sa;
    }
    p.ovf_cap = 1u << 16;
    p.k1b_threads = 1024u;
    if (p.variant == 0)
        p.k1b_lds = p.narrow ? ((size_t)p.k1b_ht * 36 + 8 + (size_t)p.k1b_ht / 4 + 12 + 15) / 16 * 16 : (size_t)p.k1b_ht * (8 + 32 + (p.hist ? 4 * SG_HIST_BINS : 0));
    if (p.narrow) p.k1b_u = 2 * p.k1b_lds > lds && m > 24.0 ? 8 : 4;
    if (ov.k1b_u) { if (ival(ov.k1b_u) == 8) p.k1b_u = 8; if (ival(ov.k1b_u) == 4) p.k1b_u = 4; }
    if (p.k1b_u == 8) p.warm = 0;
    p.k1b_pack = p.narrow && (u64)p.sn * p.nwg < 65536ull;
    if (ov.k1b_pack) { if (ival(ov.k1b_pack) == 0) p.k1b_pack = false; }
    if (ov.k1b_threads) { const u64 x = uval(ov.k1b_threads); if ((x == 256 && !p.narrow) || x == 512 || x == 1024) p.k1b_threads = (u32)x; }
    if (p.narrow && p.k1b_ht / p.k1b_threads > 4) p.k1b_threads = 1024u;
    p.k1b_order = p.narrow && !ov.k1b_no_order;
    p.prepare_fold = p.warm && p.narrow && p.variant == 0 && cfg.world <= 1 && p.k1b_threads == 1024u && p.k1b_lds >= kPrepareLds &&
                     !(ov.no_fold && ival(ov.no_fold) != 0);
    p.max_blocks = p.variant == 0 ? (u32)std::min<u64>(1024, std::max<u64>(64, (u64)cfg.max_ips / 32)) : 2u;
    if (p.variant == 0) p.ecap = K2_TILE;
    p.alive_cap = cfg.max_alive ? cfg.max_alive : 65536u;
    p.kept_edges = p.warm ? std::max<u64>(ME, (u64)p.npb * p.pcap) : ME;
    p.hub_cap = (u32)std::min<u64>(p.kept_edges / 256 + 16, 1u << 24);

    p.k3_ranges = (p.ncap + K3_IN_NR - 1) / K3_IN_NR;
    p.k3_slices = (u32)std::min<u64>((u64)p.k3_ranges * K3_IN_SMAX <= p.cus ? K3_IN_SMAX : 32, std::max<u64>(8, ME / 8192));
    if (ov.k3_slices) { const u64 x = uval(ov.k3_slices); if (x >= 1 && x <= 256) p.k3_slices = (u32)x; }
    p.k3in_lds = (size_t)K3_IN_NR * 48;
    {
        const u64 bw = ((u64)p.ncap + 31) / 32;
        p.k2_sortw = bw <= K2_SORT_LDS ? K2_SORT_LDS : (u32)std::min<u64>(K2_SORT_LDS_MAX, (bw + 255) / 256 * 256);
    }
    {
        u32 g = std::min<u32>(K2_DH_GMAX, p.variant == 0 ? p.npb : 0u);
        if (ME < (1ull << 19)) g = 0;
        if (p.warm) g = 0;
        else if (ov.dh_g) { const u64 x = uval(ov.dh_g); g = (x >= 16 && x <= K2_DH_GMAX && (x & (x - 1)) == 0 && p.variant == 0 && x <= p.npb) ? (u32)x : 0u; }
        if (g >= 16 && (g & (g - 1)) == 0 && p.npb % g == 0 && ((size_t)p.ncap + 1) * sizeof(u32) <= 128u * 1024u && (u64)p.npb * p.pcap < (1ull << 32)) {
            p.dh_g = g; p.dh_ppw = p.npb / g; p.dh_ns = (p.ncap + 1 + 63u) & ~63u;
        }
    }
    p.ablate = ov.ablate ? (u32)std::strtoul(ov.ablate->c_str(), nullptr, 0) : 0u;
    p.k4_split = cfg.max_edges > (1u << 17);
    if (ov.k4_fused) p.k4_split = ival(ov.k4_fused) == 0;
    p.k5_grid = (u32)grid_for(cfg.max_edges, 32, 3 * (int)p.cus);
    if (ov.k5_grid) { const int x = ival(ov.k5_grid); if (x >= 1 && x <= 65535) p.k5_grid = (u32)std::min(grid_for(cfg.max_edges, 32, 65535), x); }
    p.k3_fuse_allowed = !ov.k3_no_fuse;
    p.k6_one_wg = (bool)ov.k6_one_wg;
    if (ov.copy_streams) p.n_copy = ival(ov.copy_streams) == 2 ? 2 : 1;
    if (ov.stage_slots) p.n_stage = std::min(kStageSlots, std::max(2, ival(ov.stage_slots)));
    p.n_slots = std::min<u32>(std::max<u32>(cfg.windows_in_flight, 1), 8);
    *out = p;
    return SG_OK;
}

inline bool plan_pass_a(const Plan& p, uint32_t l1_entries, size_t l2_bytes, const Overrides& ov, PassA* out) {
    PassA a;
    const size_t lds_cap = kLdsBytes;
    const size_t l1b = (size_t)l1_entries * 8, l2b = l2_bytes;
    const size_t stage_max = (size_t)K1A_NJ * K1A_THREADS * 16;
    if (p.narrow) {
        a.l2_u16 = p.max_known <= 16384 && !ov.l2_u32;
        const size_t l2lds = a.l2_u16 ? l2b / 2 : l2b;
        if (ov.nsub) { const int x = ival(ov.nsub); if (x == 1 || x == 2) a.k1a_nsub = (u32)x; }
        const bool want_tile = ov.k1a && *ov.k1a == "tile", force_team = ov.k1a && *ov.k1a == "team";
        const size_t fixed_tile = (size_t)p.np * 24 + 64 + (size_t)K1T_TS(a.k1a_nsub) * 8 + l1b;
        const int teams = 2, nt = 1024;
        const size_t stage_team = (size_t)K1A_NJ * nt * 16;
        const bool team_ok = (p.np == 256 || p.np == 512 || p.np == 1024) && (size_t)p.np * p.nwg * p.punits * 8 < ((size_t)1 << 31) && l1b <= stage_team;
        a.k1a_teams = (u32)teams; a.k1a_nt = (u32)nt;
        const size_t fixed_team = K1M_LDS_FIXED(p.np, teams, nt) + l1b;
        auto pick = [&](size_t fixed, u32 ct_min, size_t stage_cap, u32& ct, bool& in_lds) {
            ct = 0; in_lds = false;
            for (u32 c : {1024u, 512u, 256u, 128u}) if (c >= ct_min && (size_t)c * 40 + fixed + l2lds <= lds_cap && l1b + l2b <= stage_cap) { in_lds = true; ct = c; break; }
            if (!ct) for (u32 c : {1024u, 512u, 256u, 128u, 64u}) if (c >= ct_min && (size_t)c * 40 + fixed <= lds_cap) { ct = c; break; }
        };
        u32 ct = 0; bool in_lds = false;
        if (!want_tile && team_ok) { pick(fixed_team, force_team ? 64u : 256u, stage_team, ct, in_lds); a.k1a_team = ct != 0; }
        if (!ct) pick(fixed_tile, 64u, stage_max, ct, in_lds);
        const size_t fixed = a.k1a_team ? fixed_team : fixed_tile;
        a.l2_in_lds = in_lds;
        if (ov.l2_global) a.l2_in_lds = false;
        if (ov.ct) { const u32 x = (u32)std::strtoul(ov.ct->c_str(), nullptr, 0); if (x >= 64 && x <= 2048 && (x & (x - 1)) == 0 && (size_t)x * 40 + fixed + (a.l2_in_lds ? l2lds : 0) <= lds_cap) ct = x; }
        if (!ct || l1b > stage_max) return false;
        a.k1a_ct = ct;
        a.k1a_lds = (size_t)ct * 40 + fixed + (a.l2_in_lds ? l2lds : 0);
        *out = a;
        return true;
    }
    const size_t fixed = (size_t)p.np * 4 + 64 + l1b;
    const size_t slot = p.hist ? 72 : 40;
    u32 ct = 0;
    for (u32 c : {2048u, 1024u, 512u}) if ((size_t)c * slot + fixed + l2b <= lds_cap && l1b + l2b <= stage_max) { a.l2_in_lds = true; ct = c; break; }
    if (!ct) for (u32 c : {2048u, 1024u, 512u, 256u, 128u, 64u}) if ((size_t)c * slot + fixed <= lds_cap) { ct = c; break; }
    if (ov.ct) { const u32 x = (u32)std::strtoul(ov.ct->c_str(), nullptr, 0); if (x >= 64 && x <= 2048 && (x & (x - 1)) == 0 && (size_t)x * slot + fixed + (a.l2_in_lds ? l2b : 0) <= lds_cap) ct = x; }
    if (ov.l2_global) a.l2_in_lds = false;
    if (!ct || l1b > stage_max) return false;
    a.k1a_ct = ct;
    a.k1a_lds = (size_t)ct * slot + fixed + (a.l2_in_lds ? l2b : 0);
    *out = a;
    return true;
}

enum K1aFamily { K1A_GLOBAL = 0, K1A_WIDE = 1, K1A_TILE = 2, K1A_TEAM = 3 };
enum K1bFamily { K1B_NONE = 0, K1B_MERGE = 1, K1B_STREAM = 2 };
constexpr int kK1bWarmU = 2;
struct PassAKernel {
    int family = K1A_GLOBAL;
    int l2 = 0;
    bool sharded = false, hist = false;
    int nsub = 0, pb = 0;
};
struct Kernels {
    PassAKernel k1a;
    int k1b_family = K1B_NONE, k1b_u = 0, k1b_spt = 0;
    bool k1b_pack = false, k1b_hist = false, k1b_share = false, k1b_warm = false;
    bool k2_dh = false;
    bool k4_split = false, k4_mfma = true;
    bool k5_mfma = true;
};
inline PassAKernel choose_pass_a(const Plan& p, const PassA& a, const sg_config& cfg) {
    PassAKernel k;
    if (p.variant != 0) return k;
    k.sharded = cfg.world > 1;
    if (!p.narrow) { k.family = K1A_WIDE; k.l2 = a.l2_in_lds ? 1 : 0; k.hist = p.hist != 0; return k; }
    k.l2 = a.l2_in_lds ? (a.l2_u16 ? 2 : 1) : 0;
    if (a.k1a_team) { k.family = K1A_TEAM; k.pb = p.np == 256 ? 8 : p.np == 512 ? 9 : 10; }
    else { k.family = K1A_TILE; k.nsub = a.k1a_nsub == 2 ? 2 : 1; }
    return k;
}
inline Kernels choose_kernels(const Plan& p, const PassA& a, const sg_config& cfg) {
    Kernels k;
    k.k1a = choose_pass_a(p, a, cfg);
    if (p.variant == 0) {
        k.k1b_share = p.npb > p.cus && 2 * p.k1b_lds <= kLdsBytes;
        const u32 spt = p.k1b_ht / p.k1b_threads;
        k.k1b_u = p.k1b_u == 8 ? 8 : 4;
        if (p.warm || p.narrow) { k.k1b_family = K1B_STREAM; k.k1b_spt = spt >= 4 ? 4 : spt == 2 ? 2 : 1; k.k1b_pack = p.k1b_pack; k.k1b_warm = p.warm != 0; }
        else { k.k1b_family = K1B_MERGE; k.k1b_hist = p.hist != 0; if (k.k1b_hist) k.k1b_u = 4; }
    }
    k.k2_dh = p.dh_g != 0;
    k.k4_split = p.k4_split; k.k4_mfma = p.use_mfma; k.k5_mfma = p.use_mfma;
    return k;
}

template <size_t N> using Key = std::array<int, N>;
template <size_t... L>
constexpr std::array<Key<sizeof...(L)>, (L * ...)> product(const int (&... v)[L]) {
    std::array<Key<sizeof...(L)>, (L * ...)> out{};
    for (size_t i = 0; i < out.size(); i++) { size_t r = i, k = 0; ((out[i][k++] = v[r % L], r /= L), ...); }
    return out;
}
template <size_t N, size_t A, size_t B>
constexpr std::array<Key<N>, A + B> concat(const std::array<Key<N>, A>& a, const std::array<Key<N>, B>& b) {
    std::array<Key<N>, A + B> out{};
    for (size_t i = 0; i < A; i++) out[i] = a[i];
    for (size_t i = 0; i < B; i++) out[A + i] = b[i];
    return out;
}
template <size_t N, size_t M>
int find_key(const std::array<Key<N>, M>& dom, const Key<N>& k) { for (size_t i = 0; i < M; i++) if (dom[i] == k) return (int)i; return -1; }

inline constexpr auto kK1aWideKeys = product({0, 1}, {0, 1}, {0, 1});
inline constexpr auto kK1aTileKeys = product({0, 1, 2}, {0, 1}, {1, 2});
inline constexpr auto kK1aTeamKeys = product({0, 1, 2}, {0, 1}, {8, 9, 10});
inline constexpr auto kK1bMergeKeys = concat(product({4, 8}, {0}, {0, 1}), product({4}, {1}, {0, 1}));
inline constexpr auto kK1bStreamKeys = concat(product({4, 8}, {1, 2, 4}, {0, 1}, {0}, {0, 1}),
                                              product({kK1bWarmU}, {1, 2, 4}, {0, 1}, {1, 2}, {0, 1}));
inline constexpr auto kK4LayerKeys = product({32, 64}, {0, 1}, {0, 1}, {0, 1});

constexpr u64 kTrendAlign = 256;
inline u64 trend_align(u64 b) { return (b + kTrendAlign - 1) / kTrendAlign * kTrendAlign; }
struct Piece { const char* name; u64 off, bytes; };
struct Slots { u64 off = 0, bytes = 0; };
struct SlotPiece { const char* name; u64 bytes; u64* rel; };
struct Block {
    u64 align = kTrendAlign, end = 0;
    std::vector<Piece> pieces;
    u64 up(u64 b) const { return (b + align - 1) / align * align; }
    u64 take(const char* name, u64 bytes) {
        const u64 off = up(end);
        pieces.push_back({name, off, bytes});
        end = off + bytes;
        return off;
    }
    Slots slots(u32 n, std::initializer_list<SlotPiece> ps) {
        Slots s;
        for (u32 k = 0; k < std::max<u32>(n, 1); k++) {
            const u64 first = up(end);
            for (const SlotPiece& p : ps) { const u64 off = take(p.name, p.bytes); if (!k) *p.rel = off - first; }
            if (!k) { s.off = first; s.bytes = up(end) - first; }
        }
        return s;
    }
};

constexpr u32 kSelThreads = 256, kSelMaxWgs = 1024, kSelRowsPerWg = 2048, kSelStateWords = 8;
struct SelPlan {
    u32 wgs = 0;
    u64 key_bytes = 0;
    u64 hist_bytes = 0;
    u64 blk_bytes = 0;
    u64 pair_bytes = 0;
    u64 state_bytes = 0;
    u64 scratch_bytes = 0;
    u64 stage_rows = 0;
    u64 pair_off = 0, n_off = 0, state_off = 0, blk_off = 0, hist_off = 0, key_off = 0;
    std::vector<Piece> layout;
};
inline SelPlan plan_select(u64 max_edges, bool used) {
    SelPlan s;
    if (!used) return s;
    s.wgs = (u32)std::max<u64>(1, std::min<u64>(kSelMaxWgs, (max_edges + kSelRowsPerWg - 1) / kSelRowsPerWg));
    s.key_bytes = max_edges * 4;
    s.hist_bytes = (u64)s.wgs * 256 * 4;
    s.blk_bytes = (u64)s.wgs * 4 * 4;
    s.pair_bytes = (u64)SG_SELECT_MAX_K * 8;
    s.state_bytes = kSelStateWords * 4 + 8;
    s.stage_rows = max_edges;
    Block b; b.align = 8;
    s.pair_off = b.take("pairs", s.pair_bytes);
    s.n_off = b.take("state", s.state_bytes); s.state_off = s.n_off + 8;
    s.blk_off = b.take("blk", s.blk_bytes);
    s.hist_off = b.take("hist", s.hist_bytes);
    s.key_off = b.take("keys", s.key_bytes);
    s.scratch_bytes = b.end; s.layout = std::move(b.pieces);
    return s;
}
struct IndexSelPlan {
    SelPlan sel;
    u64 stage_rows = 0;
    u64 stage_bytes = 0;
    u64 ctr_bytes = 0;
    u64 idx_bytes = 0;
    u64 sel_bytes = 0;
    u64 stage_off = 0, ctr_off = 0, idx_off = 0, sel_off = 0;
    u64 total_bytes = 0;
    std::vector<Piece> layout;
};
inline IndexSelPlan plan_index_select(u64 rows, u64 stage_rows, u64 row_bytes, u64 counter_bytes) {
    IndexSelPlan n;
    n.sel = plan_select(rows, true);
    n.stage_rows = stage_rows;
    n.stage_bytes = trend_align(stage_rows * row_bytes);
    n.ctr_bytes = trend_align(counter_bytes);
    n.idx_bytes = trend_align(rows * 4);
    n.sel_bytes = trend_align(n.sel.scratch_bytes);
    Block b;
    n.stage_off = b.take("stage", n.stage_bytes);
    n.ctr_off = b.take("ctr", n.ctr_bytes);
    n.idx_off = b.take("idx", n.idx_bytes);
    n.sel_off = b.take("sel", n.sel_bytes);
    n.total_bytes = b.end; n.layout = std::move(b.pieces);
    return n;
}
using NodeSelPlan = IndexSelPlan;
inline NodeSelPlan plan_node_select(u32 ncap, u64 counter_bytes) {
    const u64 NC = std::max<u32>(ncap, 1);
    return plan_index_select(NC, NC, sizeof(sg_node_out), counter_bytes);
}
inline size_t select_sort_lds(u32 k) { return (size_t)next_pow2(std::max<u32>(k, 1)) * 8; }

constexpr u32 kTrendThreads = 256, kTrendMaxWgs = 1024, kTrendPerThread = 8, kTrendCtlWords = 8;
constexpr u64 kTrendMaxEntries = 1ull << 31;
inline int check_trend(const sg_trend_params& p, u64 max_edges, sg_trend_params* out) {
    if (p.struct_size != sizeof(sg_trend_params) || p.reserved != 0 || p.shift > 10 || p.max_entries > kTrendMaxEntries) return SG_EINVAL;
    sg_trend_params r = p;
    if (!r.shift) r.shift = 4;
    if (!r.warmup) r.warmup = 4;
    if (!r.ttl) r.ttl = 64;
    if (!r.max_entries) r.max_entries = std::min<u64>(kTrendMaxEntries, 2 * std::max<u64>(max_edges, 1));
    if (!r.lat_floor_ns) r.lat_floor_ns = 1000;
    if (!r.err_floor) r.err_floor = 10486;
    *out = r;
    return SG_OK;
}
struct TrendPlan {
    u64 entries = 0;
    u32 wgs = 0;
    u64 soa_bytes = 0;
    u64 ctl_bytes = 0;
    u64 blk_bytes = 0;
    u64 thread_bytes = 0;
    u64 rows_bytes = 0;
    u64 total_bytes = 0;
    u64 soa_off[2] = {}, ctl_off = 0, blk_off = 0, thread_off = 0;
    Slots slot; u64 slot_rows = 0;
    u64 soa_from_key = 0, soa_to_key = 0, soa_stat[4] = {}, soa_n = 0, soa_last = 0;
    std::vector<Piece> layout, soa_layout;
};
inline TrendPlan plan_baseline(const sg_trend_params& p, u64 samples, u64 row_bytes, u32 slots) {
    TrendPlan t;
    t.entries = p.max_entries;
    const u64 T = p.max_entries + samples, per_wg = (u64)kTrendThreads * kTrendPerThread;
    t.wgs = (u32)std::max<u64>(1, std::min<u64>(kTrendMaxWgs, (T + per_wg - 1) / per_wg));
    t.soa_bytes = trend_align(p.max_entries * (2 * 8 + 4 * 8 + 2 * 4));
    t.ctl_bytes = trend_align(kTrendCtlWords * 8);
    t.blk_bytes = trend_align((u64)t.wgs * 4 * 4);
    t.thread_bytes = trend_align((u64)t.wgs * kTrendThreads * 16);
    t.rows_bytes = trend_align(row_bytes);
    Block b;
    t.soa_off[0] = b.take("soa0", t.soa_bytes); t.soa_off[1] = b.take("soa1", t.soa_bytes);
    t.ctl_off = b.take("ctl", t.ctl_bytes);
    t.blk_off = b.take("blk", t.blk_bytes);
    t.thread_off = b.take("thread", t.thread_bytes);
    t.slot = b.slots(slots, {{"rows", t.rows_bytes, &t.slot_rows}});
    t.total_bytes = b.end; t.layout = std::move(b.pieces);
    Block q; q.align = 4;
    const u64 C = p.max_entries;
    t.soa_from_key = q.take("from_key", C * 8); t.soa_to_key = q.take("to_key", C * 8);
    const char* const stat[4] = {"lat_mean", "lat_dev", "err_mean", "err_dev"};
    for (int k = 0; k < 4; k++) t.soa_stat[k] = q.take(stat[k], C * 8);
    t.soa_n = q.take("n", C * 4); t.soa_last = q.take("last", C * 4);
    t.soa_layout = std::move(q.pieces);
    return t;
}
inline TrendPlan plan_trend(u64 max_edges, u32 slots, const sg_trend_params& p) {
    return plan_baseline(p, max_edges, std::max<u64>(max_edges, 1) * sizeof(sg_edge_trend), slots);
// ... 628 lines not shown
```

### alaz_amd/csrc/sg_sizes.h

```cpp
#pragma once

#define SG_MAX_K1_WGS 2048

#define K1A_THREADS 1024
#define K1A_NJ      6
#define K1T_THREADS 1024
#define K1T_CHUNK   4096u
#define K1T_TS(NSUB) (K1T_CHUNK * (NSUB))
#define K1M_LDS_FIXED(np, teams, nt) ((size_t)(np) * 4 * (2 + 4 * (teams)) + 128 + ((size_t)(nt) * 4 + 4) * 8)

#define K2_TILE 2048
#define K2_DH_GMAX 128
#define K2_SORT_LDS 4096
#define K2_SORT_LDS_MAX 16384

#define K3_IN_NR    3072
#define K3_IN_SMAX  48

#define KW_ROWS 512
```

### alaz_amd/engine.py

```python
from __future__ import annotations

import ctypes as C
import os
from collections import namedtuple
from typing import Optional, Tuple

import numpy as np

from .replay import EDGE_OUT_DTYPE, EVENT_DTYPE

_HERE = os.path.dirname(os.path.abspath(__file__))
LIB_PATH = os.environ.get("SG_LIB_PATH") or os.path.join(_HERE, "lib", "libservicegraph.so")
LIB_DEV_PATH = os.path.join(_HERE, "lib", "libservicegraph_dev.so")
DEV_KNOBS = ("SG_ABLATE", "SG_NP", "SG_HT", "SG_CT", "SG_NWG", "SG_NSUB", "SG_SPLIT", "SG_WARM", "SG_K1A", "SG_K1_NARROW", "SG_K1_LEGACY", "SG_K1B_U",
             "SG_K1B_THREADS", "SG_K1B_PACK", "SG_K1B_NO_ORDER", "SG_L2_GLOBAL", "SG_L2_U32", "SG_DH_G", "SG_K3_SLICES", "SG_K3_NO_FUSE", "SG_K4_FUSED", "SG_K5_GRID", "SG_K6_ONE_WG", "SG_DENSE_VALU",
             "SG_COPY_STREAMS", "SG_STAGE_SLOTS", "SG_ARENA", "SG_NO_FOLD")

SG_OK, SG_EINVAL, SG_ENOMEM, SG_ENODEV, SG_ENOSPC, SG_EAGAIN, SG_ESTATE = 0, -22, -12, -19, -28, -11, -71
SELECT_MAX_K = 16384
F_IN, F_HID, F_EDGE = 32, 64, 8
STAT_SUM_WORDS, STAT_MAX_WORDS = 12, 2
REF_KNOWN, REF_LABEL, REF_OBIP = 0, 1, 2

TREND_DTYPE = np.dtype([("lat_dev", "<f4"), ("err_dev", "<f4"), ("base_mean_us", "<f4"), ("windows_seen", "<u4")])
TREND_ENTRY_DTYPE = np.dtype([("from_key", "<u8"), ("to_key", "<u8"), ("lat_mean", "<f8"), ("lat_dev", "<f8"), ("err_mean", "<f8"),
                              ("err_dev", "<f8"), ("n", "<u4"), ("last", "<u4")])
NODE_DTYPE = np.dtype([(f"{side}_{f}", "<u8") for f in ("count", "err", "sum_ns", "sumsq_us", "max_ns", "score_q32") for side in ("out", "in")]
                      + [(f, "<u4") for f in ("ref", "out_edges", "in_edges", "out_alive", "in_alive", "out_worst_row", "in_worst_row")]
                      + [(f, "<f4") for f in ("out_score_max", "in_score_max", "score")])
NODE_TREND_DTYPE = np.dtype([(f, "<f4") for f in ("in_lat_dev", "in_err_dev", "out_lat_dev", "out_err_dev", "in_base_mean_us", "out_base_mean_us")]
                            + [("in_seen", "<u4"), ("out_seen", "<u4")])
RANK_DTYPE = np.dtype([("rank", "<u8"), ("ref", "<u4"), ("share", "<f4")])
RANK_SEED = dict(score=0, uniform=1)
RANK_DEFAULTS = dict(iters=0, damping_q8=0, seed="score", seed_min_score=0.0)
INCIDENT_DTYPE = np.dtype([(f, "<u8") for f in ("count", "err", "sum_ns", "score_q32", "rank_sum")]
                          + [(f, "<u4") for f in ("first_node", "nodes", "edges", "worst_row", "top_node", "culprit_node")]
                          + [("value_max", "<f4"), ("reserved", "<u4")])
NO_INCIDENT = 0xFFFFFFFF
INCIDENT_DEFAULTS = dict(by="score", min_value=0.0)
TRACK_DTYPE = np.dtype([(f, "<u4") for f in ("track", "parent", "first_window", "windows", "kept_nodes", "moved_nodes", "joined_nodes", "flags")])
TRACK_ENTRY_DTYPE = np.dtype([(f, "<u4") for f in ("track", "parent", "first_window", "last_window", "windows", "peak_nodes")]
                             + [("count", "<u8"), ("err", "<u8")])
NO_TRACK = 0xFFFFFFFF
TRACK_NEW, TRACK_SPLIT, TRACK_MERGED = 1, 2, 4
TRACK_DEFAULTS = dict(quiet_windows=2, max_tracks=0)
GROUP_EDGE_DTYPE = np.dtype([(f, "<u8") for f in ("count", "err_count", "sum_ns", "sumsq_us", "max_ns", "score_q32")]
                            + [(f, "<u4") for f in ("from_ref", "to_ref", "edges", "from_nodes", "first", "alive", "worst_row")]
                            + [("score_max", "<f4")])
NO_GROUP = 0xFFFFFFFF
REF_GROUP = 3
GROUP_DEFAULTS = dict(max_groups=0)
VANISHED_DTYPE = np.dtype([("from_key", "<u8"), ("to_key", "<u8"), ("lat_mean", "<f8"), ("lat_dev", "<f8"), ("err_mean", "<f8"),
                           ("err_dev", "<f8"), ("n", "<u4"), ("last", "<u4"), ("row", "<u4"), ("reserved", "<u4")])
VANISHED_DEFAULTS = dict(silent_windows=0, min_seen=0, max_rows=0)
SEL_BY = dict(score=0, lat_dev=1, err_dev=2, new=3)
NSEL_BY = dict(score=0, in_lat_dev=1, in_err_dev=2, out_lat_dev=3, out_err_dev=4, new=5)
TREND_DEFAULTS = dict(shift=4, warmup=4, ttl=64, max_entries=0, lat_floor_ns=1000, err_floor=10486)
Q_SPACES = dict(nodes=1, groups=2, group_nodes=4)
Q_MAX = 8


class SgConfig(C.Structure):
    _fields_ = [("struct_size", C.c_uint32), ("abi_version", C.c_uint32), ("device", C.c_int32), ("max_known_nodes", C.c_uint32),
                ("max_labels", C.c_uint32), ("max_outbound_ips", C.c_uint32), ("max_ips", C.c_uint32),
                ("max_edges", C.c_uint64), ("max_batch", C.c_uint32), ("layers", C.c_uint32),
                ("rank", C.c_uint32), ("world", C.c_uint32), ("k1_variant", C.c_uint32),
                ("max_window_events", C.c_uint64), ("windows_in_flight", C.c_uint32), ("max_alive", C.c_uint32), ("flags", C.c_uint32)]


CFG_EDGE_HISTOGRAM = 1
CFG_NO_WARM = 2
CFG_WARM = 4
ABI_VERSION = 6


def make_config(*, max_known_nodes: int, max_edges: int, layers: int = 1, max_labels: int = 256, max_outbound_ips: int = 64,
                max_ips: int = 0, max_batch: int = 1 << 16, device: int = 0, rank: int = 0, world: int = 1, k1_variant: int = 0,
                max_window_events: int = 0, windows_in_flight: int = 1, max_alive: int = 0, flags: int = 0) -> "SgConfig":
    return SgConfig(C.sizeof(SgConfig), ABI_VERSION, device, max_known_nodes, max_labels, max_outbound_ips, max_ips or max_known_nodes,
                    max_edges, max_batch, layers, rank, world, k1_variant, max_window_events, windows_in_flight, max_alive, flags)


class SgGeometry(C.Structure):
    _fields_ = [(n, C.c_uint32) for n in ("k1_variant", "k1_narrow", "partitions", "table_slots", "pass_a_workgroups", "cache_slots",
                                          "join_l2_in_lds", "tile_records", "endpoint_bits", "piece_bytes", "pass_b_split", "pass_a_teams", "warm_windows")]


class SgStats(C.Structure):
    _fields_ = [("events_in", C.c_uint64), ("events_dropped_src", C.c_uint64), ("events_dropped_ring", C.c_uint64),
                ("events_dropped_cap", C.c_uint64), ("windows", C.c_uint64), ("last_window_events", C.c_uint64),
                ("last_window_edges", C.c_uint64), ("last_window_nodes", C.c_uint64),
                ("last_window_tmin_ms", C.c_int64), ("last_window_tmax_ms", C.c_int64), ("h2d_bytes", C.c_uint64),
                ("events_misrouted", C.c_uint64), ("halo_overflow", C.c_uint64),
                ("alive_in", C.c_uint64), ("alive_dropped", C.c_uint64),
                ("join_word_updates", C.c_uint64), ("join_full_uploads", C.c_uint64), ("ingest_waits", C.c_uint64),
                ("windows_warm", C.c_uint64), ("windows_cold", C.c_uint64),
                ("windows_delta", C.c_uint64), ("windows_plain", C.c_uint64), ("last_window_new_edges", C.c_uint64)]


class SgTrendParams(C.Structure):
    _fields_ = [("struct_size", C.c_uint32), ("shift", C.c_uint32), ("warmup", C.c_uint32), ("ttl", C.c_uint32),
                ("max_entries", C.c_uint64), ("lat_floor_ns", C.c_uint64), ("err_floor", C.c_uint32), ("reserved", C.c_uint32)]


class SgVanishedParams(C.Structure):
    _fields_ = [("struct_size", C.c_uint32), ("silent_windows", C.c_uint32), ("min_seen", C.c_uint32), ("max_rows", C.c_uint32)]


class SgRankParams(C.Structure):
    _fields_ = [("struct_size", C.c_uint32), ("iters", C.c_uint32), ("damping_q8", C.c_uint32), ("seed", C.c_uint32),
                ("seed_min_score", C.c_float), ("reserved", C.c_uint32)]


class SgIncidentParams(C.Structure):
    _fields_ = [("struct_size", C.c_uint32), ("by", C.c_uint32), ("min_value", C.c_float), ("reserved", C.c_uint32)]


class SgGroupParams(C.Structure):
    _fields_ = [("struct_size", C.c_uint32), ("max_groups", C.c_uint32), ("reserved", C.c_uint32 * 2)]


class SgTrackParams(C.Structure):
    _fields_ = [("struct_size", C.c_uint32), ("quiet_windows", C.c_uint32), ("max_tracks", C.c_uint32), ("reserved", C.c_uint32)]


class SgTrackStats(C.Structure):
    _fields_ = [(n, C.c_uint64) for n in ("windows", "live", "opened", "dropped_cap")]


class SgTrendStats(C.Structure):
    _fields_ = [(n, C.c_uint64) for n in ("windows", "entries", "inserted", "expired", "dropped")]


def _signatures() -> dict:
    I, H, P, PP = C.c_int, C.c_void_p, C.c_void_p, C.POINTER(C.c_void_p)
    u32, u64, sz, f32 = C.c_uint32, C.c_uint64, C.c_size_t, C.c_float
    Psz, Pu64, Pf64 = C.POINTER(sz), C.POINTER(u64), C.POINTER(C.c_double)
    return {
        "sg_abi_version": (u32, []), "sg_weights_count": (sz, [u32]), "sg_hash32": (u32, [u32]),
        "sg_last_error": (C.c_char_p, [H]),
        "sg_create": (I, [C.POINTER(SgConfig), PP]), "sg_destroy": (I, [H]),
        "sg_upsert_pod": (I, [H, u32, u32]), "sg_delete_pod": (I, [H, u32]),
        "sg_upsert_service": (I, [H, u32, u32]), "sg_delete_service": (I, [H, u32]),
        "sg_set_clock": (I, [H, u64, u64]), "sg_set_label_count": (I, [H, u32]),
        "sg_load_weights": (I, [H, P, sz]),
        "sg_ingest": (I, [H, P, sz]), "sg_ingest_device": (I, [H, P, sz, P]),
        "sg_flush_window": (I, [H, u64, P, sz, Psz]),
        "sg_flush_window_view": (I, [H, u64, PP, Psz]),
        "sg_flush_begin": (I, [H, u64]),
        "sg_flush_end": (I, [H, P, sz, Psz]),
        "sg_flush_end_view": (I, [H, PP, Psz]),
        "sg_window_run": (I, [H, P]), "sg_window_rows_buffer": (I, [H, PP]),
        "sg_window_close": (I, [H, P]),
        "sg_window_obip_list": (I, [H, P, u32, P, P]),
        "sg_bind_buffers": (I, [H, P, P, PP, u32]),
        "sg_window_close_sharded": (I, [H, P, P, P]),
        "sg_window_features": (I, [H, P]), "sg_window_layer": (I, [H, u32, P]),
        "sg_window_score": (I, [H, P]), "sg_window_score_reset": (I, [H, P]), "sg_window_read": (I, [H, P, sz, Psz]),
        "sg_window_reset": (I, [H, P]),
        "sg_window_buffers": (I, [H, PP, PP, PP, Psz]),
        "sg_window_feat_buffer": (I, [H, u32, PP, Psz]),
        "sg_halo_build": (I, [H, P, u32, P, P]), "sg_halo_pack": (I, [H, u32, P, u32, P, P]),
        "sg_halo_unpack": (I, [H, u32, P, u32, P, P]),
        "sg_window_close_gathered": (I, [H, P, u32, u32, P]),
        "sg_halo_build_padded": (I, [H, P, u32, P]), "sg_halo_pack_padded": (I, [H, u32, P, u32, P, P]),
        "sg_halo_unpack_padded": (I, [H, u32, P, u32, P, P]),
        "sg_window_outbound_ips": (I, [H, P, sz, Psz]),
        "sg_stats_get": (I, [H, C.POINTER(SgStats)]),
        "sg_timing_enable": (I, [H, I]), "sg_timing_reset": (I, [H]),
        "sg_timing_get": (I, [H, I, Pf64, Pu64]),
        "sg_set_warm": (I, [H, I]), "sg_timing_stride": (I, [H, u32]),
        "sg_timing_samples": (I, [H, I, Pf64, sz, Psz]),
        "sg_latency_probe": (I, [H, u64, u32, I, Pf64]),
        "sg_debug_stamps": (I, [H, P, sz]),
        "sg_clock_probe": (I, [H, u32, Pf64, Pf64]),
        "sg_comm_probe": (I, []), "sg_window_halo_counts": (I, [H, P, sz]),
        "sg_route": (I, [H, P, sz, u32, P]),
        "sg_window_hist": (I, [H, P, sz, Psz]),
        "sg_geometry_get": (I, [H, C.POINTER(SgGeometry)]),
        "sg_prepare_fold_get": (I, [H, C.POINTER(u32)]),
        "sg_comm_unique_id": (I, [P, sz]), "sg_comm_create": (I, [P, sz, I, I, I, PP]),
        "sg_comm_destroy": (I, [P]), "sg_window_run_sharded": (I, [H, P, P]),
        "sg_host_register": (I, [H, P, sz]), "sg_host_unregister": (I, [H, P]), "sg_ingest_pinned": (I, [H, P, sz]),
        "sg_ingest_bulk": (I, [H, P, sz, I, Pu64]),
        "sg_flush_window_top": (I, [H, u64, u32, f32, P, P, sz, Psz, Psz]),
        "sg_flush_end_top": (I, [H, u32, f32, P, P, sz, Psz, Psz]),
        "sg_window_select": (I, [H, u32, f32, P, P, sz, P, P]),
        "sg_set_trend": (I, [H, P]), "sg_window_trend": (I, [H, P, sz, P, sz, Psz]),
        "sg_window_trend_buffer": (I, [H, PP]), "sg_trend_entries": (I, [H, P, sz, Psz]),
        "sg_trend_stats_get": (I, [H, P]),
        "sg_set_nodes": (I, [H, I]), "sg_window_nodes": (I, [H, P, sz, Psz]),
        "sg_window_nodes_buffer": (I, [H, PP, PP]),
        "sg_set_vanished": (I, [H, P]), "sg_window_vanished": (I, [H, P, sz, Psz]),
        "sg_window_vanished_buffer": (I, [H, PP, PP]),
        "sg_flush_window_top_by": (I, [H, u64, u32, u32, f32, P, P, sz, Psz, Psz]),
        "sg_flush_end_top_by": (I, [H, u32, u32, f32, P, P, sz, Psz, Psz]),
        "sg_window_select_by": (I, [H, u32, u32, f32, P, P, sz, P, P]),
        "sg_set_node_trend": (I, [H, P]), "sg_window_node_trend": (I, [H, P, sz, P, sz, Psz]),
        "sg_window_node_trend_buffer": (I, [H, PP]), "sg_node_trend_entries": (I, [H, P, sz, Psz]),
        "sg_node_trend_stats_get": (I, [H, P]),
        "sg_window_nodes_top": (I, [H, u32, u32, f32, P, P, sz, Psz, Psz]),
        "sg_window_nodes_select": (I, [H, u32, u32, f32, P, P, sz, P, P]),
        "sg_set_rank": (I, [H, P]), "sg_window_rank": (I, [H, P, sz, P, sz, Psz]),
        "sg_window_rank_buffer": (I, [H, PP]),
        "sg_window_rank_top": (I, [H, u32, f32, P, P, P, sz, Psz, Psz]),
        "sg_window_rank_select": (I, [H, u32, f32, P, P, sz, P, P]),
        "sg_set_incidents": (I, [H, P]), "sg_window_incidents": (I, [H, P, sz, Psz]),
        "sg_window_node_incident": (I, [H, P, sz, P, sz, Psz]),
        "sg_window_incidents_buffer": (I, [H, PP, PP, PP]),
        "sg_set_tracks": (I, [H, P]), "sg_window_incident_tracks": (I, [H, P, sz, Psz]),
        "sg_window_tracks_ended": (I, [H, P, sz, Psz]),
        "sg_window_tracks_buffer": (I, [H, PP, PP, PP]),
        "sg_track_entries": (I, [H, P, sz, Psz]), "sg_track_stats_get": (I, [H, P]),
        "sg_set_groups": (I, [H, P]), "sg_group_assign": (I, [H, P, P, sz]),
        "sg_window_groups": (I, [H, P, sz, Psz]), "sg_window_row_group": (I, [H, P, sz, P, sz, Psz]),
        "sg_window_group_perm": (I, [H, P, sz, Psz]),
        "sg_window_groups_buffer": (I, [H] + [PP] * 4),
        "sg_set_group_trend": (I, [H, P]), "sg_window_group_trend": (I, [H, P, sz, P, sz, Psz]),
        "sg_window_group_trend_buffer": (I, [H, PP]), "sg_group_trend_entries": (I, [H, P, sz, Psz]),
        "sg_group_trend_stats_get": (I, [H, P]),
        "sg_set_group_vanished": (I, [H, P]), "sg_window_group_vanished": (I, [H, P, sz, Psz]),
        "sg_window_group_vanished_buffer": (I, [H, PP, PP]),
        "sg_window_groups_top": (I, [H, u32, u32, f32, P, P, sz, Psz, Psz]),
        "sg_window_groups_select": (I, [H, u32, u32, f32, P, P, sz, P, P]),
        "sg_set_group_nodes": (I, [H, I]), "sg_window_group_nodes": (I, [H, P, sz, Psz]),
        "sg_window_group_nodes_buffer": (I, [H, PP, PP]),
        "sg_set_group_node_trend": (I, [H, P]), "sg_window_group_node_trend": (I, [H, P, sz, P, sz, Psz]),
        "sg_window_group_node_trend_buffer": (I, [H, PP]), "sg_group_node_trend_entries": (I, [H, P, sz, Psz]),
        "sg_group_node_trend_stats_get": (I, [H, P]),
        "sg_window_group_nodes_top": (I, [H, u32, u32, f32, P, P, sz, Psz, Psz]),
        "sg_window_group_nodes_select": (I, [H, u32, u32, f32, P, P, sz, P, P]),
        "sg_set_group_rank": (I, [H, P]), "sg_window_group_rank": (I, [H, P, sz, P, sz, Psz]),
        "sg_window_group_rank_buffer": (I, [H, PP]),
        "sg_window_group_rank_top": (I, [H, u32, f32, P, P, P, sz, Psz, Psz]),
        "sg_window_group_rank_select": (I, [H, u32, f32, P, P, sz, P, P]),
        "sg_set_group_incidents": (I, [H, P]), "sg_window_group_incidents": (I, [H, P, sz, Psz]),
        "sg_window_group_node_incident": (I, [H, P, sz, P, sz, Psz]),
        "sg_window_group_incidents_buffer": (I, [H, PP, PP, PP]),
        "sg_set_group_tracks": (I, [H, P]), "sg_window_group_incident_tracks": (I, [H, P, sz, Psz]),
        "sg_window_group_tracks_ended": (I, [H, P, sz, Psz]),
        "sg_window_group_tracks_buffer": (I, [H, PP, PP, PP]),
        "sg_group_track_entries": (I, [H, P, sz, Psz]), "sg_group_track_stats_get": (I, [H, P]),
        "sg_set_quantiles": (I, [H, u32, P, sz]),
        "sg_window_node_hist": (I, [H, P, sz, P, sz, Psz]), "sg_window_node_quantiles": (I, [H, P, sz, P, sz, Psz]),
        "sg_window_group_hist": (I, [H, P, sz, P, sz, Psz]), "sg_window_group_quantiles": (I, [H, P, sz, P, sz, Psz]),
        "sg_window_group_node_hist": (I, [H, P, sz, P, sz, Psz]), "sg_window_group_node_quantiles": (I, [H, P, sz, P, sz, Psz]),
        "sg_window_quantiles_buffer": (I, [H, u32, PP, PP]),
        "sg_set_quantile_trend": (I, [H, u32, u32, P]),
        "sg_window_node_quantile_trend": (I, [H, P, sz, P, sz, Psz]), "sg_window_group_quantile_trend": (I, [H, P, sz, P, sz, Psz]),
        "sg_window_group_node_quantile_trend": (I, [H, P, sz, P, sz, Psz]),
        "sg_window_quantile_trend_buffer": (I, [H, u32, PP]),
        "sg_quantile_trend_entries": (I, [H, u32, P, sz, Psz]), "sg_quantile_trend_stats_get": (I, [H, u32, P]),
        "sg_window_nodes_top_tail": (I, [H, u32, u32, f32, P, P, sz, Psz, Psz]),
        "sg_window_groups_top_tail": (I, [H, u32, u32, f32, P, P, sz, Psz, Psz]),
        "sg_window_group_nodes_top_tail": (I, [H, u32, u32, f32, P, P, sz, Psz, Psz]),
    }


_SIGNATURES = _signatures()
EXPORTS = list(_SIGNATURES)


class ServiceGraphError(RuntimeError):
    def __init__(self, rc: int, msg: str):
        super().__init__(f"servicegraph rc={rc}: {msg}")
        self.rc = rc


def _rank_seed(seed) -> int:
    if not isinstance(seed, str):
        return seed
    if seed not in RANK_SEED:
        raise ValueError(f"seed must be one of {sorted(RANK_SEED)}, not {seed!r}")
    return RANK_SEED[seed]


_Stage = namedtuple("_Stage", "call struct defaults off noun convert", defaults=({},))
_STAGES = dict(
    trend=_Stage("sg_set_trend", SgTrendParams, TREND_DEFAULTS, "set_trend(None) switches the trend off", "trend"),
    node_trend=_Stage("sg_set_node_trend", SgTrendParams, TREND_DEFAULTS, "set_node_trend(None) switches the node trend off", "node trend"),
    vanished=_Stage("sg_set_vanished", SgVanishedParams, VANISHED_DEFAULTS, "set_vanished(None) switches the list off", "vanished"),
    rank=_Stage("sg_set_rank", SgRankParams, RANK_DEFAULTS, "set_rank(None) switches the ranking off", "rank", dict(seed=_rank_seed)),
    incidents=_Stage("sg_set_incidents", SgIncidentParams, INCIDENT_DEFAULTS, "set_incidents(None) switches the incidents off", "incident",
                     dict(by=lambda by: ServiceGraph._by(by) if isinstance(by, str) else by)),
    tracks=_Stage("sg_set_tracks", SgTrackParams, TRACK_DEFAULTS, "set_tracks(None) switches tracking off", "track"),
    groups=_Stage("sg_set_groups", SgGroupParams, GROUP_DEFAULTS, "set_groups(None) switches the groups off", "group",
                  dict(reserved=lambda r: (C.c_uint32 * 2)(*((r, 0) if isinstance(r, int) else tuple(r))))),
    group_trend=_Stage("sg_set_group_trend", SgTrendParams, TREND_DEFAULTS, "set_group_trend(None) switches the group trend off", "group trend"),
    group_vanished=_Stage("sg_set_group_vanished", SgVanishedParams, VANISHED_DEFAULTS, "set_group_vanished(None) switches the list off",
                          "group vanished"),
    group_node_trend=_Stage("sg_set_group_node_trend", SgTrendParams, TREND_DEFAULTS,
                            "set_group_node_trend(None) switches the workload trend off", "workload trend"),
    group_rank=_Stage("sg_set_group_rank", SgRankParams, RANK_DEFAULTS, "set_group_rank(None) switches the workload ranking off",
                      "workload rank", dict(seed=_rank_seed)),
    group_incidents=_Stage("sg_set_group_incidents", SgIncidentParams, INCIDENT_DEFAULTS,
                           "set_group_incidents(None) switches the workload incidents off", "workload incident",
                           dict(by=lambda by: ServiceGraph._by(by) if isinstance(by, str) else by)),
    group_tracks=_Stage("sg_set_group_tracks", SgTrackParams, TRACK_DEFAULTS, "set_group_tracks(None) switches workload tracking off",
                        "workload track"),
    quantile_trend=_Stage("sg_set_quantile_trend", SgTrendParams, TREND_DEFAULTS, "set_quantile_trend(params=None) switches the tail baselines off",
                          "tail trend"),
)

_lib = None
_lib_dev = None


def load_library(path: str = LIB_PATH, dev: bool = False) -> C.CDLL:
    global _lib, _lib_dev
    if dev:
        if _lib_dev is not None:
            return _lib_dev
        path = os.environ.get("SG_LIB_DEV", LIB_DEV_PATH)
        if path == LIB_DEV_PATH:
            from . import build
            build.build_engine(dev=True)
    else:
        if _lib is not None:
            return _lib
        path = os.environ.get("SG_LIB", path)
    if not os.path.exists(path):
        raise RuntimeError(f"{path} is missing: build it with `python -m alaz_amd.build` "
                           "(hipcc, gfx950). The ServiceGraph engine has no CPU fallback.")
    try:
        import torch
    except Exception:
        pass
    lib = C.CDLL(path, mode=C.RTLD_LOCAL if dev else C.RTLD_GLOBAL)
    for name, (res, args) in _SIGNATURES.items():
        f = getattr(lib, name)
        f.restype = res; f.argtypes = args
    if dev:
        _lib_dev = lib
    else:
        _lib = lib
    return lib


class RcclComm:

    @staticmethod
    def probe() -> bool:
        return load_library().sg_comm_probe() == SG_OK

    def __init__(self, rank: int, world: int, device: int, bcast):
        l = load_library()
        buf = (C.c_char * 128)()
        rc = l.sg_comm_unique_id(buf, 128) if rank == 0 else SG_OK
        raw = bcast(bytes(buf.raw) if rc == SG_OK else b"")
        if not raw:
            raise ServiceGraphError(rc if rc != SG_OK else SG_ENODEV, "sg_comm_unique_id: librccl could not be loaded on rank 0")
        idb = (C.c_char * 128).from_buffer_copy(raw)
        p = C.c_void_p()
        rc = l.sg_comm_create(idb, 128, rank, world, device, C.byref(p))
        if rc != SG_OK:
            raise ServiceGraphError(rc, "sg_comm_create (ncclCommInitRank) failed")
        self._l, self.ptr, self.rank, self.world = l, p, rank, world

    def close(self):
        if getattr(self, "ptr", None):
            self._l.sg_comm_destroy(self.ptr); self.ptr = None


def ip_u32(s: str) -> int:
    a, b, c, d = (int(x) for x in s.split("."))
    return (a << 24) | (b << 16) | (c << 8) | d


class ServiceGraph:

    def __init__(self, *, max_known_nodes: int, max_edges: int, layers: int = 1, max_labels: int = 1024,
                 max_outbound_ips: int = 1024, max_ips: int = 0, max_batch: int = 1 << 20, device: int = 0,
                 rank: int = 0, world: int = 1, k1_variant: int = 0, max_window_events: int = 0, windows_in_flight: int = 1,
                 edge_histogram: bool = False, warm: Optional[bool] = None, dev_knobs: Optional[bool] = None):
        if dev_knobs is None:
            dev_knobs = any(k in os.environ for k in DEV_KNOBS)
        self._l = load_library(dev=dev_knobs)
        cfg = make_config(max_known_nodes=max_known_nodes, max_edges=max_edges, layers=layers, max_labels=max_labels,
                          max_outbound_ips=max_outbound_ips, max_ips=max_ips, max_batch=max_batch, device=device, rank=rank, world=world,
                          k1_variant=k1_variant, max_window_events=max_window_events, windows_in_flight=windows_in_flight,
                          flags=(CFG_EDGE_HISTOGRAM if edge_histogram else 0) | (0 if warm is None else (CFG_WARM if warm else CFG_NO_WARM)))
        h = C.c_void_p()
        rc = self._l.sg_create(C.byref(cfg), C.byref(h))
        if rc != SG_OK:
            raise ServiceGraphError(rc, "sg_create failed (no usable gfx950 device, or bad config); there is no CPU fallback")
        self._h = h
        self.layers = layers
        self.max_edges = max_edges
        self.max_batch = max_batch
        self.rank, self.world = rank, world

    def _ck(self, rc: int, allow=()):
        if rc != SG_OK and rc not in allow:
            raise ServiceGraphError(rc, (self._l.sg_last_error(self._h) or b"").decode())
        return rc

    def _set_stage(self, stage: str, params, kw, *lead) -> Optional[dict]:
        st = _STAGES[stage]
        call = getattr(self._l, st.call)
        if params is None:
            if kw:
                raise TypeError(f"{st.off} and takes no parameters")
            self._ck(call(self._h, *lead, None))
            return None
        v = dict(st.defaults)
        v.update(params or {}); v.update(kw)
        unknown = set(v) - {f for f, _ in st.struct._fields_}
        if unknown:
            raise TypeError(f"unknown {st.noun} parameters: {sorted(unknown)}")
        p = st.struct(struct_size=C.sizeof(st.struct))
        for f, x in v.items():
            setattr(p, f, st.convert[f](x) if f in st.convert else x)
        self._ck(call(self._h, *lead, C.byref(p)))
        return v

    def _counted(self, call, dtype, shape_tail=()) -> np.ndarray:
        n = C.c_size_t(0)
        self._ck(call(self._h, None, 0, C.byref(n)))
        out = np.zeros((n.value,) + shape_tail, dtype=dtype)
        if n.value:
            self._ck(call(self._h, out.ctypes.data, n.value, C.byref(n)))
        return out[: n.value]

    def _window_rows(self, call, dtype, index):
        if index is None:
            return self._counted(lambda h, out, cap, n: call(h, None, 0, out, cap, n), dtype)
        idx = np.ascontiguousarray(index, dtype=np.uint32)
        out = np.zeros(len(idx), dtype=dtype)
        if len(idx):
            self._ck(call(self._h, idx.ctypes.data, len(idx), out.ctypes.data, len(idx), C.byref(C.c_size_t(0))))
        return out

    def _capped(self, call, cap: Optional[int]) -> np.ndarray:
        cap = self.max_edges if cap is None else cap
        out = np.zeros(cap, dtype=EDGE_OUT_DTYPE); n = C.c_size_t(0)
        self._ck(call(out.ctypes.data, cap, C.byref(n)))
        return out[: min(n.value, cap)]

    def _top(self, call, cap: int, *dtypes):
        outs = [np.zeros(cap, dtype=d) for d in dtypes]
        ns, nt = C.c_size_t(0), C.c_size_t(0)
        self._ck(call(*[o.ctypes.data for o in outs], cap, C.byref(ns), C.byref(nt)))
        m = min(ns.value, cap)
        return (*[o[:m] for o in outs], nt.value)

    def _node_cap(self, k: int, cap: Optional[int], count=None) -> int:
        if cap is not None:
            return cap
        if k:
            return k
        n = C.c_size_t(0)
        self._ck((count or self._l.sg_window_nodes)(self._h, None, 0, C.byref(n)))
        return n.value

    def _pointers(self, call, n: int) -> tuple:
        p = [C.c_void_p() for _ in range(n)]
        self._ck(call(self._h, *[C.byref(x) for x in p]))
        return tuple(x.value for x in p)

    def _stats(self, call, struct):
        s = struct()
        self._ck(call(self._h, C.byref(s)))
        return s

    def close(self):
        if getattr(self, "_h", None):
            self._l.sg_destroy(self._h); self._h = None

    def __del__(self):
        try:
            self.close()
        except Exception:
            pass

    def geometry(self) -> dict:
        g = SgGeometry()
        self._ck(self._l.sg_geometry_get(self._h, C.byref(g)))
        fold = C.c_uint32(0)
        self._ck(self._l.sg_prepare_fold_get(self._h, C.byref(fold)))
        return {**{n: int(getattr(g, n)) for n, _ in SgGeometry._fields_}, "prepare_fold": int(fold.value)}

    def k1_kernels(self) -> tuple:
        g = self.geometry()
        if g["k1_variant"] == 1: return ("k1_resolve_aggregate",)
        if not g["k1_narrow"]: return ("k1a_partition", "k1b_merge")
        return ("k1a_team_partition" if g["pass_a_teams"] else "k1a_tile_partition", "k1b_stream_merge")

    def upsert_pod(self, ip: int, node_id: int): self._ck(self._l.sg_upsert_pod(self._h, ip, node_id))
    def delete_pod(self, ip: int): self._ck(self._l.sg_delete_pod(self._h, ip))
    def upsert_service(self, ip: int, node_id: int): self._ck(self._l.sg_upsert_service(self._h, ip, node_id))
    def delete_service(self, ip: int): self._ck(self._l.sg_delete_service(self._h, ip))
    def set_clock(self, first_kernel_ns: int, first_user_ns: int): self._ck(self._l.sg_set_clock(self._h, first_kernel_ns, first_user_ns))
    def set_label_count(self, n: int): self._ck(self._l.sg_set_label_count(self._h, n))

    def load_weights(self, w: np.ndarray):
        w = np.ascontiguousarray(w, dtype=np.float32)
        self._ck(self._l.sg_load_weights(self._h, w.ctypes.data, len(w)))

    def ingest(self, events: np.ndarray) -> int:
        ev = np.ascontiguousarray(events)
        assert ev.dtype == EVENT_DTYPE
        return self._ck(self._l.sg_ingest(self._h, ev.ctypes.data, len(ev)), allow=(SG_EAGAIN,))

    def host_register(self, arr: np.ndarray):
        assert arr.flags.c_contiguous
        self._ck(self._l.sg_host_register(self._h, arr.ctypes.data, arr.nbytes))

    def host_unregister(self, arr: np.ndarray): self._ck(self._l.sg_host_unregister(self._h, arr.ctypes.data))

    def ingest_pinned(self, events: np.ndarray) -> int:
        assert events.dtype == EVENT_DTYPE and events.flags.c_contiguous
        return self._ck(self._l.sg_ingest_pinned(self._h, events.ctypes.data, len(events)), allow=(SG_EAGAIN,))

    def ingest_bulk(self, events: np.ndarray, pinned: bool = False) -> int:
        assert events.dtype == EVENT_DTYPE and events.flags.c_contiguous
        w = C.c_uint64(0)
        self._ck(self._l.sg_ingest_bulk(self._h, events.ctypes.data, len(events), 1 if pinned else 0, C.byref(w)))
        return int(w.value)

    def ingest_device(self, dev_ptr: int, n: int, stream: int = 0):
        self._ck(self._l.sg_ingest_device(self._h, dev_ptr, n, stream or None))

    def flush_window(self, window_end_ms: int = 0, cap: Optional[int] = None) -> np.ndarray:
        return self._capped(lambda out, c, n: self._l.sg_flush_window(self._h, window_end_ms, out, c, n), cap)

    def flush_window_view(self, window_end_ms: int = 0) -> np.ndarray:
        ptr = C.c_void_p(); n = C.c_size_t(0)
        self._ck(self._l.sg_flush_window_view(self._h, window_end_ms, C.byref(ptr), C.byref(n)))
        return self._rows_view(ptr, n)

    def flush_begin(self, window_end_ms: int = 0):
        self._ck(self._l.sg_flush_begin(self._h, window_end_ms))

    def flush_end_view(self) -> np.ndarray:
        ptr = C.c_void_p(); n = C.c_size_t(0)
        self._ck(self._l.sg_flush_end_view(self._h, C.byref(ptr), C.byref(n)))
        return self._rows_view(ptr, n)

    def flush_end(self, cap: int | None = None) -> np.ndarray:
        return self._capped(lambda out, c, n: self._l.sg_flush_end(self._h, out, c, n), cap)

    @staticmethod
    def _by(by) -> int:
        if by not in SEL_BY:
            raise ValueError(f"by must be one of {sorted(SEL_BY)}, not {by!r}")
        return SEL_BY[by]

    def flush_window_top(self, k: int, min_score: float = float("-inf"), window_end_ms: int = 0, cap: Optional[int] = None,
                         by: str = "score"):
        b = self._by(by)
        cap = (k or self.max_edges) if cap is None else cap
        if b:
            return self._top(lambda *a: self._l.sg_flush_window_top_by(self._h, window_end_ms, b, k, min_score, *a), cap, EDGE_OUT_DTYPE, np.uint32)
        return self._top(lambda *a: self._l.sg_flush_window_top(self._h, window_end_ms, k, min_score, *a), cap, EDGE_OUT_DTYPE, np.uint32)

    def flush_end_top(self, k: int, min_score: float = float("-inf"), cap: Optional[int] = None, by: str = "score"):
        b = self._by(by)
        cap = (k or self.max_edges) if cap is None else cap
        if b:
            return self._top(lambda *a: self._l.sg_flush_end_top_by(self._h, b, k, min_score, *a), cap, EDGE_OUT_DTYPE, np.uint32)
        return self._top(lambda *a: self._l.sg_flush_end_top(self._h, k, min_score, *a), cap, EDGE_OUT_DTYPE, np.uint32)

    def window_select(self, k: int, min_score: float, d_out: int, d_index: int, cap: int, d_n: int, stream: int = 0, by: str = "score"):
        b = self._by(by)
        if b:
            self._ck(self._l.sg_window_select_by(self._h, b, k, min_score, d_out or None, d_index or None, cap, d_n, stream or None))
        else:
            self._ck(self._l.sg_window_select(self._h, k, min_score, d_out or None, d_index or None, cap, d_n, stream or None))

    def set_trend(self, params: Optional[dict] = (), **kw):
        v = self._set_stage("trend", params, kw)
        if v is not None:
            self._trend_entries = v["max_entries"] or min(1 << 31, 2 * max(self.max_edges, 1))

    def window_trend(self, index: Optional[np.ndarray] = None) -> np.ndarray:
        return self._window_rows(self._l.sg_window_trend, TREND_DTYPE, index)

    def trend_buffer(self) -> int:
        return self._pointers(self._l.sg_window_trend_buffer, 1)[0]

    def trend_entries(self) -> np.ndarray:
        return self._counted(self._l.sg_trend_entries, TREND_ENTRY_DTYPE)

    def trend_stats(self) -> SgTrendStats:
        return self._stats(self._l.sg_trend_stats_get, SgTrendStats)

    def set_vanished(self, params: Optional[dict] = (), **kw):
        v = self._set_stage("vanished", params, kw)
        if v is not None:
            self._van_rows = v["max_rows"] or min(65536, self._trend_entries)

    def window_vanished(self, with_count: bool = False):
        out = self._counted(self._l.sg_window_vanished, VANISHED_DTYPE)
        rows = out[: self._van_rows]
        return (rows, len(out)) if with_count else rows

    def vanished_buffer(self) -> Tuple[int, int]:
        return self._pointers(self._l.sg_window_vanished_buffer, 2)

    def set_nodes(self, on: bool = True):
        self._ck(self._l.sg_set_nodes(self._h, 1 if on else 0))

    def window_nodes(self) -> np.ndarray:
        return self._counted(self._l.sg_window_nodes, NODE_DTYPE)

    def nodes_buffer(self) -> Tuple[int, int]:
        return self._pointers(self._l.sg_window_nodes_buffer, 2)

    def set_node_trend(self, params: Optional[dict] = (), **kw):
        self._set_stage("node_trend", params, kw)

    def window_node_trend(self, index: Optional[np.ndarray] = None) -> np.ndarray:
        return self._window_rows(self._l.sg_window_node_trend, NODE_TREND_DTYPE, index)

    def node_trend_buffer(self) -> int:
        return self._pointers(self._l.sg_window_node_trend_buffer, 1)[0]

    def node_trend_entries(self) -> np.ndarray:
        return self._counted(self._l.sg_node_trend_entries, TREND_ENTRY_DTYPE)

    def node_trend_stats(self) -> SgTrendStats:
        return self._stats(self._l.sg_node_trend_stats_get, SgTrendStats)

    @staticmethod
    def _nby(by) -> int:
        if by not in NSEL_BY:
            raise ValueError(f"by must be one of {sorted(NSEL_BY)}, not {by!r}")
        return NSEL_BY[by]

    def window_nodes_top(self, k: int, min_value: float = float("-inf"), by: str = "score", cap: Optional[int] = None):
        b = self._nby(by)
        return self._top(lambda *a: self._l.sg_window_nodes_top(self._h, b, k, min_value, *a), self._node_cap(k, cap), NODE_DTYPE, np.uint32)

# ... 384 lines not shown
```

### include/servicegraph.h

```cpp
#ifndef SERVICEGRAPH_H
#define SERVICEGRAPH_H

#include <stddef.h>
#include <stdint.h>

#ifdef __cplusplus
extern "C" {
#endif

#define SG_ABI_VERSION 6u

#define SG_OK        0
#define SG_EINVAL   (-22)
#define SG_ENOMEM   (-12)
#define SG_ENODEV   (-19)
#define SG_ENOSPC   (-28)
#define SG_EAGAIN   (-11)
#define SG_ESTATE   (-71)

#define SG_PROTO_UNKNOWN  0
#define SG_PROTO_HTTP     1
#define SG_PROTO_AMQP     2
#define SG_PROTO_POSTGRES 3
#define SG_PROTO_HTTP2    4
// ... 303 lines not shown
typedef struct sg_group_params {
    uint32_t struct_size;
    uint32_t max_groups;
    uint32_t reserved[2];
} sg_group_params;
typedef struct sg_group_edge {
    uint64_t count, err_count, sum_ns, sumsq_us, max_ns, score_q32;
    uint32_t from_ref, to_ref;
    uint32_t edges;
    uint32_t from_nodes;
    uint32_t first;
    uint32_t alive;
    uint32_t worst_row;
    float    score_max;
} sg_group_edge;
int sg_set_groups(sg_handle h, const sg_group_params* p);
int sg_group_assign(sg_handle h, const uint32_t* node_ids, const uint32_t* groups, size_t n);
int sg_window_groups(sg_handle h, sg_group_edge* out, size_t cap, size_t* n);
int sg_window_row_group(sg_handle h, const uint32_t* row_index, size_t n_index, uint32_t* out, size_t cap, size_t* n);
int sg_window_group_perm(sg_handle h, uint32_t* out, size_t cap, size_t* n);
int sg_window_groups_buffer(sg_handle h, void** d_edges, void** d_count, void** d_row_group, void** d_perm);

int sg_set_group_trend(sg_handle h, const sg_trend_params* p);
int sg_window_group_trend(sg_handle h, const uint32_t* group_index, size_t n_index, sg_edge_trend* out, size_t cap, size_t* n);
int sg_window_group_trend_buffer(sg_handle h, void** d_trend);
int sg_group_trend_entries(sg_handle h, sg_trend_entry* out, size_t cap, size_t* n);
int sg_group_trend_stats_get(sg_handle h, sg_trend_stats* out);
int sg_set_group_vanished(sg_handle h, const sg_vanished_params* p);
int sg_window_group_vanished(sg_handle h, sg_edge_vanished* out, size_t cap, size_t* n);
int sg_window_group_vanished_buffer(sg_handle h, void** d_rows, void** d_count);
int sg_window_groups_top(sg_handle h, uint32_t by, uint32_t k, float min_value, sg_group_edge* out, uint32_t* group_index,
                         size_t cap, size_t* n_selected, size_t* n_groups);
int sg_window_groups_select(sg_handle h, uint32_t by, uint32_t k, float min_value, sg_group_edge* d_out, uint32_t* d_index,
                            size_t cap, uint64_t* d_n, void* stream);

int sg_set_group_nodes(sg_handle h, int on);
int sg_window_group_nodes(sg_handle h, sg_node_out* out, size_t cap, size_t* n);
int sg_window_group_nodes_buffer(sg_handle h, void** d_nodes, void** d_count);
int sg_set_group_node_trend(sg_handle h, const sg_trend_params* p);
int sg_window_group_node_trend(sg_handle h, const uint32_t* node_index, size_t n_index, sg_node_trend* out, size_t cap, size_t* n);
int sg_window_group_node_trend_buffer(sg_handle h, void** d_trend);
int sg_group_node_trend_entries(sg_handle h, sg_trend_entry* out, size_t cap, size_t* n);
int sg_group_node_trend_stats_get(sg_handle h, sg_trend_stats* out);
int sg_window_group_nodes_top(sg_handle h, uint32_t by, uint32_t k, float min_value, sg_node_out* out, uint32_t* node_index,
                              size_t cap, size_t* n_selected, size_t* n_nodes);
int sg_window_group_nodes_select(sg_handle h, uint32_t by, uint32_t k, float min_value, sg_node_out* d_out, uint32_t* d_index,
                                 size_t cap, uint64_t* d_n, void* stream);

int sg_set_group_rank(sg_handle h, const sg_rank_params* p);
int sg_window_group_rank(sg_handle h, const uint32_t* node_index, size_t n_index, sg_node_rank* out, size_t cap, size_t* n);
int sg_window_group_rank_buffer(sg_handle h, void** d_rank);
int sg_window_group_rank_top(sg_handle h, uint32_t k, float min_share, sg_node_out* out, sg_node_rank* rank_out,
                             uint32_t* node_index, size_t cap, size_t* n_selected, size_t* n_nodes);
int sg_window_group_rank_select(sg_handle h, uint32_t k, float min_share, sg_node_out* d_out, uint32_t* d_index,
                                size_t cap, uint64_t* d_n, void* stream);

int sg_set_group_incidents(sg_handle h, const sg_incident_params* p);
int sg_window_group_incidents(sg_handle h, sg_incident_out* out, size_t cap, size_t* n);
int sg_window_group_node_incident(sg_handle h, const uint32_t* node_index, size_t n_index, uint32_t* out, size_t cap, size_t* n);
int sg_window_group_incidents_buffer(sg_handle h, void** d_incidents, void** d_count, void** d_node_incident);

int sg_set_group_tracks(sg_handle h, const sg_track_params* p);
int sg_window_group_incident_tracks(sg_handle h, sg_incident_track* out, size_t cap, size_t* n);
int sg_window_group_tracks_ended(sg_handle h, sg_track_entry* out, size_t cap, size_t* n);
int sg_window_group_tracks_buffer(sg_handle h, void** d_tracks, void** d_ended, void** d_ended_count);
int sg_group_track_entries(sg_handle h, sg_track_entry* out, size_t cap, size_t* n);
int sg_group_track_stats_get(sg_handle h, sg_track_stats* out);

#define SG_Q_NODES        1u
#define SG_Q_GROUPS       2u
#define SG_Q_GROUP_NODES  4u
#define SG_Q_MAX          8u
int sg_set_quantiles(sg_handle h, uint32_t spaces, const uint32_t* permille, size_t n_q);
int sg_window_node_hist(sg_handle h, const uint32_t* node_index, size_t n_index, uint64_t* out, size_t cap, size_t* n);
int sg_window_node_quantiles(sg_handle h, const uint32_t* node_index, size_t n_index, uint32_t* out_us, size_t cap, size_t* n);
int sg_window_group_hist(sg_handle h, const uint32_t* group_index, size_t n_index, uint64_t* out, size_t cap, size_t* n);
int sg_window_group_quantiles(sg_handle h, const uint32_t* group_index, size_t n_index, uint32_t* out_us, size_t cap, size_t* n);
int sg_window_group_node_hist(sg_handle h, const uint32_t* node_index, size_t n_index, uint64_t* out, size_t cap, size_t* n);
int sg_window_group_node_quantiles(sg_handle h, const uint32_t* node_index, size_t n_index, uint32_t* out_us, size_t cap, size_t* n);
int sg_window_quantiles_buffer(sg_handle h, uint32_t space, void** d_hist, void** d_quantiles);

int sg_set_quantile_trend(sg_handle h, uint32_t spaces, uint32_t permille, const sg_trend_params* p);
int sg_window_node_quantile_trend(sg_handle h, const uint32_t* node_index, size_t n_index, sg_node_trend* out, size_t cap, size_t* n);
int sg_window_group_quantile_trend(sg_handle h, const uint32_t* group_index, size_t n_index, sg_edge_trend* out, size_t cap, size_t* n);
int sg_window_group_node_quantile_trend(sg_handle h, const uint32_t* node_index, size_t n_index, sg_node_trend* out, size_t cap, size_t* n);
int sg_window_quantile_trend_buffer(sg_handle h, uint32_t space, void** d_trend);
int sg_quantile_trend_entries(sg_handle h, uint32_t space, sg_trend_entry* out, size_t cap, size_t* n);
int sg_quantile_trend_stats_get(sg_handle h, uint32_t space, sg_trend_stats* out);
int sg_window_nodes_top_tail(sg_handle h, uint32_t by, uint32_t k, float min_value, sg_node_out* out, uint32_t* node_index, size_t cap, size_t* n_selected, size_t* n_nodes);
int sg_window_groups_top_tail(sg_handle h, uint32_t by, uint32_t k, float min_value, sg_group_edge* out, uint32_t* group_index, size_t cap, size_t* n_selected, size_t* n_groups);
int sg_window_group_nodes_top_tail(sg_handle h, uint32_t by, uint32_t k, float min_value, sg_node_out* out, uint32_t* node_index, size_t cap, size_t* n_selected, size_t* n_nodes);

int sg_flush_begin(sg_handle h, uint64_t window_end_ms);
int sg_flush_end(sg_handle h, sg_edge_out* out, size_t cap, size_t* n);
int sg_flush_end_view(sg_handle h, const sg_edge_out** rows, size_t* n);

int sg_window_run(sg_handle h, void* stream);
int sg_window_rows_buffer(sg_handle h, void** d_rows);

int sg_window_close(sg_handle h, void* stream);
int sg_window_obip_list(sg_handle h, uint32_t* d_list, uint32_t cap, uint32_t* d_n, void* stream);
int sg_window_close_sharded(sg_handle h, const uint32_t* d_union_ips, const uint32_t* d_union_n, void* stream);
int sg_window_close_gathered(sg_handle h, const uint32_t* d_gathered, uint32_t stride, uint32_t world, void* stream);
int sg_window_features(sg_handle h, void* stream);
int sg_window_layer(sg_handle h, uint32_t l, void* stream);
int sg_window_score(sg_handle h, void* stream);
int sg_window_score_reset(sg_handle h, void* stream);
int sg_window_read(sg_handle h, sg_edge_out* out, size_t cap, size_t* n);
int sg_window_reset(sg_handle h, void* stream);

int sg_window_buffers(sg_handle h, void** stats_sum, void** stats_max, void** counters,
                      size_t* n_nodes_cap);
int sg_window_feat_buffer(sg_handle h, uint32_t l, void** rows, size_t* row_floats);

int sg_bind_buffers(sg_handle h, void* stats_sum, void* stats_max, void* const* feat_rows, uint32_t n_feat);

int sg_halo_build(sg_handle h, uint32_t* d_ids, uint32_t cap, uint32_t* d_counts, void* stream);
int sg_halo_build_padded(sg_handle h, uint32_t* d_req, uint32_t capp, void* stream);
int sg_halo_pack_padded(sg_handle h, uint32_t l, const uint32_t* d_serve, uint32_t capp, float* d_rows, void* stream);
int sg_halo_unpack_padded(sg_handle h, uint32_t l, const uint32_t* d_req, uint32_t capp, const float* d_rows, void* stream);
int sg_halo_pack(sg_handle h, uint32_t l, const uint32_t* d_ids, uint32_t n, float* d_rows, void* stream);
int sg_halo_unpack(sg_handle h, uint32_t l, const uint32_t* d_ids, uint32_t n, const float* d_rows, void* stream);

typedef struct sg_comm sg_comm;
int sg_comm_probe(void);
int sg_comm_unique_id(void* id128, size_t bytes);
int sg_comm_create(const void* id128, size_t bytes, int rank, int world, int device, sg_comm** out);
int sg_comm_destroy(sg_comm* c);
int sg_window_run_sharded(sg_handle h, sg_comm* comm, void* stream);
int sg_window_halo_counts(sg_handle h, uint32_t* counts, size_t world);

int sg_window_outbound_ips(sg_handle h, uint32_t* ips, size_t cap, size_t* n);
int sg_window_hist(sg_handle h, uint32_t* bins, size_t cap_rows, size_t* n);

int sg_stats_get(sg_handle h, sg_stats* out);

typedef struct sg_geometry {
    uint32_t k1_variant;
    uint32_t k1_narrow;
    uint32_t partitions;
    uint32_t table_slots;
    uint32_t pass_a_workgroups;
    uint32_t cache_slots;
    uint32_t join_l2_in_lds;
    uint32_t tile_records;
    uint32_t endpoint_bits;
    uint32_t piece_bytes;
    uint32_t pass_b_split;
    uint32_t pass_a_teams;
    uint32_t warm_windows;
} sg_geometry;
int sg_geometry_get(sg_handle h, sg_geometry* out);
int sg_prepare_fold_get(sg_handle h, uint32_t* out);

int sg_timing_enable(sg_handle h, int on);
int sg_timing_reset(sg_handle h);
int sg_timing_stride(sg_handle h, uint32_t n);
int sg_timing_get(sg_handle h, int kernel, double* avg_us, uint64_t* launches);
int sg_set_warm(sg_handle h, int on);
int sg_timing_samples(sg_handle h, int kernel, double* us, size_t cap, size_t* n);
int sg_latency_probe(sg_handle h, uint64_t bytes, uint32_t steps, int warm, double* ns_per_load);
int sg_clock_probe(sg_handle h, uint32_t spin_us, double* spin_mhz, double* k1a_mhz);
int sg_debug_stamps(sg_handle h, uint64_t* out, size_t n);

uint32_t sg_hash32(uint32_t x);
int sg_route(sg_handle h, const sg_event* events, size_t n, uint32_t world, uint32_t* shard_out);

#ifdef __cplusplus
}
#endif
#endif
```

Before: 23.17 billion events/s.

## Process pass-A team tiles in pairs to halve barriers and copy-out rounds

Adds a PAIR variant of the K1 pass-A team partition kernel. Each team now bins two tiles into a double-size LDS tile before one copy-out, which merges the second tile's scan with a record move of the first tile. The variant is enabled by default when the team kernel is in use, ct >= 512, np <= 512 and the extra LDS fits. This is meant to cut per-tile barrier, scan and copy-out overhead, at the cost of more LDS per workgroup, an extra barrier for the in-LDS move, and a more complex control path.

New measurement: 23.41 billion events/s (median of 6 runs). 1.0% higher.

```diff
diff --git a/alaz_amd/csrc/servicegraph.hip b/alaz_amd/csrc/servicegraph.hip
--- a/alaz_amd/csrc/servicegraph.hip
+++ b/alaz_amd/csrc/servicegraph.hip
@@ -248,6 +248,7 @@
 struct K1aWide : Family<K1aFn, sgplan::kK1aWideKeys> { template <size_t I> static Fn at() { constexpr auto k = keys[I]; return k1a_partition<(bool)k[0], (bool)k[1], (bool)k[2]>; } };
 struct K1aTile : Family<K1aFn, sgplan::kK1aTileKeys> { template <size_t I> static Fn at() { constexpr auto k = keys[I]; return k1a_tile_partition<k[0], (bool)k[1], k[2]>; } };
 struct K1aTeam : Family<K1aFn, sgplan::kK1aTeamKeys> { template <size_t I> static Fn at() { constexpr auto k = keys[I]; return k1a_team_partition<k[0], (bool)k[1], 2, 1024, k[2]>; } };
+struct K1aTeamPair : Family<K1aFn, sgplan::kK1aTeamPairKeys> { template <size_t I> static Fn at() { constexpr auto k = keys[I]; return k1a_team_partition<k[0], (bool)k[1], 2, 1024, k[2], 1>; } };
 struct K1bMerge : Family<K1bFn, sgplan::kK1bMergeKeys> { template <size_t I> static Fn at() {
     constexpr auto k = keys[I]; if constexpr (k[2]) return k1b_merge<k[0], (bool)k[1]>; else return k1b_merge_wide<k[0], (bool)k[1]>; } };
 struct K1bStream : Family<K1bFn, sgplan::kK1bStreamKeys> { template <size_t I> static Fn at() {
@@ -286,7 +287,7 @@
     if (!sgplan::plan_pass_a(e->plan, e->jt.l1_entries, e->jt.blocks_bytes(), e->ov, &pa)) { e->err = "K1 pass A: the join tables' level 1 and the piece counters do not fit a CU's LDS (fewer partitions / IP blocks needed)"; return SG_ENOSPC; }
     const sgplan::PassAKernel k = sgplan::choose_pass_a(e->plan, pa, e->cfg);
     bool ok = true;
-    const K1aFn f = k.family == sgplan::K1A_TEAM ? kernel_of<K1aTeam>(ok, k.l2, k.sharded, k.pb)
+    const K1aFn f = k.family == sgplan::K1A_TEAM ? (k.pair ? kernel_of<K1aTeamPair>(ok, k.l2, k.sharded, k.pb) : kernel_of<K1aTeam>(ok, k.l2, k.sharded, k.pb))
                   : k.family == sgplan::K1A_TILE ? kernel_of<K1aTile>(ok, k.l2, k.sharded, k.nsub) : kernel_of<K1aWide>(ok, k.l2, k.sharded, k.hist);
     if (!ok) { e->err = "K1 pass A: the library holds no kernel for family " + std::to_string(k.family) + ", level 2 mode " + std::to_string(k.l2); return SG_ENODEV; }
     e->pa = pa; e->kn.k1a = k; e->fn.k1a = f;
@@ -401,7 +402,7 @@
             }
         }
         const u32 threads = !w.d.narrow ? K1A_THREADS : e->pa.k1a_team ? 1024 : K1T_THREADS;
-        hipExtLaunchKernelGGL(e->fn.k1a, dim3(w.d.nwg), dim3(threads), (uint32_t)e->pa.k1a_lds, s, ta, tb, 0u, da, d_ev, (u64)n);
+        hipExtLaunchKernelGGL(e->fn.k1a, dim3(w.d.nwg), dim3(threads), (uint32_t)(e->pa.k1a_lds + e->pa.k1a_pair_lds), s, ta, tb, 0u, da, d_ev, (u64)n);
         if (tk) { TimingRec r; r.a = ta; r.b = tb; r.kernel = 1; e->trecs.push_back(r); }
     } else {
         Timed t(e, s, 1);
@@ -1925,7 +1926,7 @@
     }
     if (d.variant == 0) {
         CR(plan_pass_a(e));
-        CH(lds_limit_all<K1aWide>(kLdsBytes)); CH(lds_limit_all<K1aTile>(kLdsBytes)); CH(lds_limit_all<K1aTeam>(kLdsBytes));
+        CH(lds_limit_all<K1aWide>(kLdsBytes)); CH(lds_limit_all<K1aTile>(kLdsBytes)); CH(lds_limit_all<K1aTeam>(kLdsBytes)); CH(lds_limit_all<K1aTeamPair>(kLdsBytes));
         CH(lds_limit_all<K1bMerge>(P.k1b_lds)); CH(lds_limit_all<K1bStream>(P.k1b_lds));
         CH(lds_limit((size_t)KW_ROWS * 5 * sizeof(u64), kw_compact));
     }
@@ -2099,6 +2100,13 @@
     return SG_OK;
 }
 
+int sg_pass_a_pair_get(sg_handle e, uint32_t* out) {
+    if (!e || !out) return SG_EINVAL;
+    std::lock_guard<std::mutex> g(e->mu);
+    *out = e->plan.narrow && e->pa.k1a_team && e->pa.k1a_pair ? 1u : 0u;
+    return SG_OK;
+}
+
 int sg_upsert_pod(sg_handle e, uint32_t ip, uint32_t node_id) {
     if (!e) return SG_EINVAL;
     std::lock_guard<std::mutex> g(e->mu);
diff --git a/alaz_amd/csrc/sg_k1_team.h b/alaz_amd/csrc/sg_k1_team.h
--- a/alaz_amd/csrc/sg_k1_team.h
+++ b/alaz_amd/csrc/sg_k1_team.h
@@ -8,7 +8,7 @@
     const unsigned long long grp = per >= 4 * tt ? 4 * tt : (per + tt - 1) / tt * tt;
     return (n + grp - 1) / grp;
 }
-template <int L2M, bool SHARDED, int TEAMS, int NT, int NPB>
+template <int L2M, bool SHARDED, int TEAMS, int NT, int NPB, int PAIR = 0>
 __global__ __launch_bounds__(NT) void k1a_team_partition(Dev d, const sg_event* __restrict__ ev, u64 n) {
     constexpr u32 K1M_THREADS = NT;
     constexpr u32 K1M_TILE_ALL = 4 * NT;
@@ -17,6 +17,8 @@
     constexpr u32 K1M_GROUP = 4 * K1M_TT;
     constexpr u32 K1M_TS = K1M_TILE_ALL / TEAMS;
     constexpr u32 K1M_NR = 4;
+    constexpr u32 K1M_TILE = (PAIR ? 2u : 1u) * K1M_TS;
+    static_assert(!PAIR || (((1u << NPB) >> 6) % 4u == 0 && ((1u << NPB) >> 6) <= 16u), "PAIR: the quad scan only");
     extern __shared__ __attribute__((aligned(16))) unsigned char smem[];
     const u32 CT = d.k1a_ct;
     constexpr u32 NP = 1u << NPB;
@@ -26,7 +28,7 @@
     u64* red = reinterpret_cast<u64*>(tcnt + 4 * TEAMS * NP);
     u32* bar = reinterpret_cast<u32*>(red + 8);
     u64* tiles = reinterpret_cast<u64*>(bar + 16);
-    uint4* jl = reinterpret_cast<uint4*>(tiles + K1M_TILE_ALL + 4);
+    uint4* jl = reinterpret_cast<uint4*>(tiles + TEAMS * K1M_TILE + 4);
     const u32 jl1_bytes = (d.jl1mask + 1) * 8u;
     const u32 jlds = L2M == 2 ? jl1_bytes + ((d.jstage_bytes - jl1_bytes) >> 1) : d.jstage_bytes;
     u64* ckey = reinterpret_cast<u64*>(reinterpret_cast<unsigned char*>(jl) + ((jlds + 15u) & ~15u));
@@ -40,7 +42,7 @@
     u32* bcnt = tcnt + team * 4 * NP;
     u32* boff = bcnt + 2 * NP;
     u32* pbase = boff + NP;
-    u64* tile = tiles + team * (K1M_TS + 2);
+    u64* tile = tiles + team * (K1M_TILE + 2);
     u32* mybar = bar + 8 * team;
     const uint4* __restrict__ pe = reinterpret_cast<const uint4*>(ev);
     const u32 units = (u32)TEAMS * d.nwg;
@@ -199,22 +201,19 @@
     const u32 nwpun = d.nwg * d.punits;
     const __amdgpu_buffer_rsrc_t slab_rsrc = __builtin_amdgcn_make_buffer_rsrc(slab_w, 0, (int)(u32)(((size_t)NP * d.nwg - w) * d.punits * 8u), 0x00020000);
     auto ovf_record = [&](const u32 b, const u32 remv, const u32 dur, const u32 err) { const Dev& d = kd(); K1Local L; ovf8_single(d, b, ((u64)b << d.rb) | remv, (u64)dur, err, 0u, L); k1_red_add(red, L); };
-    auto copy_out = [&](const u32 pc) {
-        const u32* bc = bcnt + pc * NP;
-        if (packb) {
-            u32 tq = tt; asm volatile("" : "+v"(tq));
-            const u32 total = boff[NP - 1] + bc[NP - 1];
+    auto copy_half = [&](const u32 tq, const u32 total, const u32 base) {
+        {
             const u32 pbm = (1u << d.pb) - 1u, strip = ~(pbm << rb);
             constexpr u32 NPOS = K1M_TS / K1M_TT;
             u64 rec[NPOS]; u32 pb_[NPOS], bo_[NPOS];
 #pragma unroll
-            for (u32 k = 0; k < NPOS; k++) rec[k] = tile[tq + k * K1M_TT];
+            for (u32 k = 0; k < NPOS; k++) rec[k] = tile[tq + base + k * K1M_TT];
 #pragma unroll
             for (u32 k = 0; k < NPOS; k++) { const u32 b = ((u32)(rec[k] >> 32) >> rb) & pbm; pb_[k] = pbase[b]; bo_[k] = boff[b]; }
             u32 ovm = 0;
 #pragma unroll
             for (u32 k = 0; k < NPOS; k++) {
-                const u32 i = tq + k * K1M_TT, h = (u32)(rec[k] >> 32), b = (h >> rb) & pbm;
+                const u32 i = tq + base + k * K1M_TT, h = (u32)(rec[k] >> 32), b = (h >> rb) & pbm;
                 const u32 pos = pb_[k] + (i - bo_[k]);
                 const bool valid = i < total;
                 if SG_ABL(d, 0x2u) { if (valid & (pos < sn)) slab_w[(u64)b * nwpun + pos] = (rec[k] & 0xFFFFFFFFull) | ((u64)(h & strip) << 32); }
@@ -225,11 +224,20 @@
             if (__builtin_amdgcn_ballot_w64(ovm != 0)) {
 #pragma unroll 1
                 for (u32 k = 0; k < NPOS; k++) if ((ovm >> k) & 1u) {
-                    const u64 r = tile[tq + k * K1M_TT];
+                    const u64 r = tile[tq + base + k * K1M_TT];
                     const u32 h = (u32)(r >> 32);
                     ovf_record((h >> rb) & pbm, h & rbmask, (u32)r, h >> 31);
                 }
             }
+        }
+    };
+    auto copy_out = [&](const u32 pc) {
+        const u32* bc = bcnt + pc * NP;
+        if (packb) {
+            u32 tq = tt; asm volatile("" : "+v"(tq));
+            const u32 total = boff[NP - 1] + bc[NP - 1];
+            copy_half(tq, total, 0u);
+            if constexpr (PAIR) { if ((u32)__builtin_amdgcn_readfirstlane((int)total) > K1M_TS) copy_half(tq, total, K1M_TS); }
         } else {
             const u32 bpw = NP / K1M_TW;
 #pragma unroll 1
@@ -261,13 +269,9 @@
     const bool dyn = !SG_ABL(d, 0x4u);
     u32* nxt2 = bar + 8 * team + 4;
     const u32 ntile32 = (u32)ntile;
-    for (u32 j = unit; j < ntile32; cur ^= 1u) {
-        u32* bc = bcnt + cur * NP;
-        u32 lo[K1M_NR], hi[K1M_NR], pr[K1M_NR];
-        u32 ttl = tt, lanel = lane; asm volatile("" : "+v"(ttl), "+v"(lanel));
-        const u64 tk0 = stamp ? wall_clock64() : 0ull;
-        {
-            if (havep) { const u64 tq = stamp ? wall_clock64() : 0ull; copy_out(pcur); if (stamp) tk_p4 += wall_clock64() - tq; }
+    auto next_tile = [&](const u32 j, const u32 sel) { return dyn ? (u32)__builtin_amdgcn_readfirstlane((int)lds_fresh_u32(nxt2 + sel)) : j + units; };
+    auto p1 = [&](const u32 j, const u32 sel, u32* bc, const u32 ttl, const u32 lanel, u32 (&lo)[K1M_NR], u32 (&hi)[K1M_NR], u32 (&pr)[K1M_NR]) {
+        {
             u32 f0, c0;
             gbounds(j, f0, c0);
             v4u_t eaa0, eba0, eaa1, eba1, eaa2, eba2, eaa3, eba3;
@@ -284,7 +288,7 @@
             const u64 tl0 = stamp ? wall_clock64() : 0ull;
             asm volatile("s_waitcnt vmcnt(0)" : "+v"(eaa0), "+v"(eba0), "+v"(eaa1), "+v"(eba1), "+v"(eaa2), "+v"(eba2), "+v"(eaa3), "+v"(eba3), "+v"(tkv) : : "memory");
             if (stamp) tk_ld += wall_clock64() - tl0;
-            if (drawer) { asm volatile("" : "+v"(tkv)); nxt2[cur] = tkv - d.k1a_ticket_base + units; }
+            if (drawer) { asm volatile("" : "+v"(tkv)); nxt2[sel] = tkv - d.k1a_ticket_base + units; }
             {
                 u32 Lm[2], Rm[2], du[2], fl[2];
                 front2(ttl, 0u, c0, eaa0, eba0, eaa1, eba1, Lm, Rm, du, fl);
@@ -297,15 +301,27 @@
                 back2(Lm, Rm, du, fl, bc, lo + 2, hi + 2, pr + 2);
             }
         }
-        const u64 tk1 = stamp ? wall_clock64() : 0ull;
-        team_barrier();
-        const u64 tk2 = stamp ? wall_clock64() : 0ull;
-        tk_p1 += tk1 - tk0; tk_wait += tk2 - tk1;
-        {
+    };
+    auto scan = [&](const u32* bc, u32* bprev, const u32 lanel, auto first) -> u32 {
+        {
+            constexpr bool FIRST = decltype(first)::value;
             constexpr u32 pl = NP >> 6; const u32 b0 = lanel * pl;
-            const bool own = (lanel % K1M_TW) == wv;
-            u32* bprev = bcnt + (cur ^ 1u) * NP;
-            if constexpr ((pl & 3u) == 0 && pl <= 16) {
+            const bool own = !FIRST && (lanel % K1M_TW) == wv;
+            if constexpr (FIRST) {
+                constexpr u32 nq = pl >> 2;
+                uint4 cq[4];
+                u32 s = 0;
+#pragma unroll
+                for (u32 k = 0; k < 4; k++) { cq[k] = k < nq ? reinterpret_cast<const uint4*>(bc + b0)[k] : make_uint4(0u, 0u, 0u, 0u); s += cq[k].x + cq[k].y + cq[k].z + cq[k].w; }
+                const u32 incl = wave_incl_scan_u32(s, lanel);
+                u32 run = incl - s;
+#pragma unroll
+                for (u32 k = 0; k < 4; k++) if (k < nq) {
+                    uint4 o; o.x = run; run += cq[k].x; o.y = run; run += cq[k].y; o.z = run; run += cq[k].z; o.w = run; run += cq[k].w;
+                    reinterpret_cast<uint4*>(bprev + b0)[k] = o;
+                }
+                return (u32)__builtin_amdgcn_readlane((int)incl, 63);
+            } else if constexpr ((pl & 3u) == 0 && pl <= 16) {
                 constexpr u32 nq = pl >> 2;
                 uint4 cq[4];
                 u32 s = 0;
@@ -330,7 +346,7 @@
 #pragma unroll
                     for (u32 k = 0; k < 4; k++) if (k < nq) {
                         reinterpret_cast<uint4*>(pbase + b0)[k] = pbv[k];
-                        reinterpret_cast<uint4*>(bprev + b0)[k] = make_uint4(0u, 0u, 0u, 0u);
+                        if constexpr (!PAIR) reinterpret_cast<uint4*>(bprev + b0)[k] = make_uint4(0u, 0u, 0u, 0u);
                     }
                 }
             } else {
@@ -344,21 +360,22 @@
                 }
             }
         }
-        const u64 tk3 = stamp ? wall_clock64() : 0ull;
+        return 0u;
+    };
+    auto place = [&](const u32* offs, const u32 (&lo)[K1M_NR], const u32 (&hi)[K1M_NR], const u32 (&pr)[K1M_NR]) {
         {
             u32 of_[K1M_NR];
 #pragma unroll
-            for (int i = 0; i < (int)K1M_NR; i++) of_[i] = boff[pr[i] < K1M_RARE ? (pr[i] & ((1u << K1T_RANK_SHIFT) - 1u)) : 0u];
+            for (int i = 0; i < (int)K1M_NR; i++) of_[i] = offs[pr[i] < K1M_RARE ? (pr[i] & ((1u << K1T_RANK_SHIFT) - 1u)) : 0u];
 #pragma unroll
             for (int i = 0; i < (int)K1M_NR; i++) {
                 const u32 pt_ = pr[i] & ((1u << K1T_RANK_SHIFT) - 1u);
-                const u32 at = pr[i] < K1M_RARE ? of_[i] + (pr[i] >> K1T_RANK_SHIFT) : K1M_TS;
+                const u32 at = pr[i] < K1M_RARE ? of_[i] + (pr[i] >> K1T_RANK_SHIFT) : K1M_TILE;
                 tile[at] = (u64)lo[i] | ((u64)(hi[i] | (packb ? pt_ << rb : 0u)) << 32);
             }
         }
-        const u64 tk4 = stamp ? wall_clock64() : 0ull;
-        team_barrier();
-        const u64 tk5 = stamp ? wall_clock64() : 0ull;
+    };
+    auto tile_tail = [&](const u32 j, const u32 ttl, const u32 lanel, const u32 (&pr)[K1M_NR]) {
         {
             u32 rmask = 0;
 #pragma unroll
@@ -380,9 +397,91 @@
             }
             st_acc = st_dsrc = st_maxlabel = st_misr = 0; st_tmin = ~0ull; st_tmax = 0;
         }
+    };
+    if constexpr (!PAIR) {
+    for (u32 j = unit; j < ntile32; cur ^= 1u) {
+        u32* bc = bcnt + cur * NP;
+        u32 lo[K1M_NR], hi[K1M_NR], pr[K1M_NR];
+        u32 ttl = tt, lanel = lane; asm volatile("" : "+v"(ttl), "+v"(lanel));
+        const u64 tk0 = stamp ? wall_clock64() : 0ull;
+        if (havep) { const u64 tq = stamp ? wall_clock64() : 0ull; copy_out(pcur); if (stamp) tk_p4 += wall_clock64() - tq; }
+        p1(j, cur, bc, ttl, lanel, lo, hi, pr);
+        const u64 tk1 = stamp ? wall_clock64() : 0ull;
+        team_barrier();
+        const u64 tk2 = stamp ? wall_clock64() : 0ull;
+        tk_p1 += tk1 - tk0; tk_wait += tk2 - tk1;
+        scan(bc, bcnt + (cur ^ 1u) * NP, lanel, std::false_type{});
+        const u64 tk3 = stamp ? wall_clock64() : 0ull;
+        place(boff, lo, hi, pr);
+        const u64 tk4 = stamp ? wall_clock64() : 0ull;
+        team_barrier();
+        const u64 tk5 = stamp ? wall_clock64() : 0ull;
+        tile_tail(j, ttl, lanel, pr);
         havep = true; pcur = cur;
         if (stamp) { tk_scan += tk3 - tk2; tk_p3 += tk4 - tk3; tk_b3 += tk5 - tk4; }
-        j = dyn ? (u32)__builtin_amdgcn_readfirstlane((int)lds_fresh_u32(nxt2 + cur)) : j + units;
+        j = next_tile(j, cur);
+    }
+    } else {
+    u32 tsel = 0;
+    for (u32 j = unit; j < ntile32; cur ^= 1u) {
+        u32* bc = bcnt + cur * NP;
+        u32* offa = bcnt + (cur ^ 1u) * NP;
+        u32 lo[K1M_NR], hi[K1M_NR], pr[K1M_NR];
+        u32 ttl = tt, lanel = lane; asm volatile("" : "+v"(ttl), "+v"(lanel));
+        const u64 tk0 = stamp ? wall_clock64() : 0ull;
+        if (havep) { copy_out(pcur); if (stamp) tk_p4 += wall_clock64() - tk0; }
+        const u64 tka = stamp ? wall_clock64() : 0ull;
+        p1(j, tsel, bc, ttl, lanel, lo, hi, pr);
+        const u64 tk1 = stamp ? wall_clock64() : 0ull;
+        team_barrier();
+        const u64 tk2 = stamp ? wall_clock64() : 0ull;
+        const u32 tot_a = scan(bc, offa, lanel, std::true_type{});
+        const u64 tk3 = stamp ? wall_clock64() : 0ull;
+        place(offa, lo, hi, pr);
+        const u64 tk4 = stamp ? wall_clock64() : 0ull;
+        team_barrier();
+        if (stamp) { tk_p1 += tk1 - tka; tk_wait += tk2 - tk1; tk_scan += tk3 - tk2; tk_p3 += tk4 - tk3; tk_b3 += wall_clock64() - tk4; }
+        tile_tail(j, ttl, lanel, pr);
+        const u32 jb = next_tile(j, tsel);
+        tsel ^= 1u;
+        const bool hasb = jb < ntile32;
+        if (hasb) {
+            asm volatile("" : "+v"(ttl), "+v"(lanel));
+            const u64 tb0 = stamp ? wall_clock64() : 0ull;
+            p1(jb, tsel, bc, ttl, lanel, lo, hi, pr);
+            const u64 tb1 = stamp ? wall_clock64() : 0ull;
+            team_barrier();
+            if (stamp) { tk_p1 += tb1 - tb0; tk_wait += wall_clock64() - tb1; }
+        }
+        const u64 tk5 = stamp ? wall_clock64() : 0ull;
+        scan(bc, nullptr, lanel, std::false_type{});
+        const u64 tk6 = stamp ? wall_clock64() : 0ull;
+        u64 tk_mv = 0;
+        if (hasb) {
+            u64 ra[K1M_NR]; u32 ob_[K1M_NR], oa_[K1M_NR];
+#pragma unroll
+            for (u32 k = 0; k < K1M_NR; k++) ra[k] = tile[ttl + k * K1M_TT];
+#pragma unroll
+            for (u32 k = 0; k < K1M_NR; k++) { const u32 b = ((u32)(ra[k] >> 32) >> rb) & (NP - 1u); ob_[k] = boff[b]; oa_[k] = offa[b]; }
+            const u64 tm0 = stamp ? wall_clock64() : 0ull;
+            team_barrier();
+            if (stamp) tk_mv = wall_clock64() - tm0;
+#pragma unroll
+            for (u32 k = 0; k < K1M_NR; k++) { const u32 i = ttl + k * K1M_TT; tile[i < tot_a ? ob_[k] + (i - oa_[k]) : K1M_TILE] = ra[k]; }
+            place(boff, lo, hi, pr);
+            if ((lanel % K1M_TW) == wv) {
+                constexpr u32 pl = NP >> 6;
+#pragma unroll
+                for (u32 k = 0; k < pl / 4; k++) reinterpret_cast<uint4*>(offa + lanel * pl)[k] = make_uint4(0u, 0u, 0u, 0u);
+            }
+        }
+        const u64 tk7 = stamp ? wall_clock64() : 0ull;
+        team_barrier();
+        if (stamp) { tk_scan += tk6 - tk5; tk_p3 += tk7 - tk6 - tk_mv; tk_b3 += tk_mv + (wall_clock64() - tk7); }
+        havep = true; pcur = cur;
+        if (hasb) { tile_tail(jb, ttl, lanel, pr); j = next_tile(jb, tsel); tsel ^= 1u; }
+        else j = jb;
+    }
     }
     if (havep) copy_out(pcur);
     SG_STAMP(d, 0, 3);
diff --git a/alaz_amd/csrc/sg_plan.hpp b/alaz_amd/csrc/sg_plan.hpp
--- a/alaz_amd/csrc/sg_plan.hpp
+++ b/alaz_amd/csrc/sg_plan.hpp
@@ -36,7 +36,7 @@
 struct Overrides {
     typedef std::optional<std::string> Knob;
     Knob ablate, np, ht, ct, nwg, nsub, split, warm, k1a, k1_narrow, k1_legacy, k1b_u, k1b_threads, k1b_pack, k1b_no_order,
-         l2_global, l2_u32, dh_g, k3_slices, k3_no_fuse, k4_fused, k5_grid, k6_one_wg, dense_valu, copy_streams, stage_slots, arena, no_fold;
+         l2_global, l2_u32, dh_g, k3_slices, k3_no_fuse, k4_fused, k5_grid, k6_one_wg, dense_valu, copy_streams, stage_slots, arena, no_fold, k1a_pair;
 };
 struct KnobName { const char* name; Overrides::Knob Overrides::*field; };
 constexpr KnobName kKnobs[] = {
@@ -48,7 +48,7 @@
     {"SG_DH_G", &Overrides::dh_g}, {"SG_K3_SLICES", &Overrides::k3_slices}, {"SG_K3_NO_FUSE", &Overrides::k3_no_fuse},
     {"SG_K4_FUSED", &Overrides::k4_fused}, {"SG_K5_GRID", &Overrides::k5_grid}, {"SG_K6_ONE_WG", &Overrides::k6_one_wg},
     {"SG_DENSE_VALU", &Overrides::dense_valu}, {"SG_COPY_STREAMS", &Overrides::copy_streams}, {"SG_STAGE_SLOTS", &Overrides::stage_slots},
-    {"SG_ARENA", &Overrides::arena}, {"SG_NO_FOLD", &Overrides::no_fold},
+    {"SG_ARENA", &Overrides::arena}, {"SG_NO_FOLD", &Overrides::no_fold}, {"SG_K1A_PAIR", &Overrides::k1a_pair},
 };
 #ifdef SG_DEV_KNOBS
 inline Overrides from_env() {
@@ -90,6 +90,8 @@
     bool l2_u16 = false, k1a_team = false, l2_in_lds = false;
     u32 k1a_nsub = 2, k1a_teams = 2, k1a_nt = 1024, k1a_ct = 2048;
     size_t k1a_lds = 0;
+    bool k1a_pair = false;
+    size_t k1a_pair_lds = 0;
 };
 
 inline int check_config(const sg_config& in, sg_config* out) {
@@ -231,6 +233,7 @@
     return SG_OK;
 }
 
+constexpr bool kK1aPairDefault = true;
 inline bool plan_pass_a(const Plan& p, uint32_t l1_entries, size_t l2_bytes, const Overrides& ov, PassA* out) {
     PassA a;
     const size_t lds_cap = kLdsBytes;
@@ -262,6 +265,18 @@
         if (!ct || l1b > stage_max) return false;
         a.k1a_ct = ct;
         a.k1a_lds = (size_t)ct * 40 + fixed + (a.l2_in_lds ? l2lds : 0);
+        {
+            const size_t extra = K1M_LDS_PAIR_EXTRA(p.np, teams, nt);
+            const bool able = a.k1a_team && 2 * p.nb <= 31 && (p.np == 256 || p.np == 512 || p.np == 1024);
+            const bool forced = ov.k1a_pair && ival(ov.k1a_pair) != 0;
+            if (able && forced && !ov.ct && ct > 512 && a.k1a_lds + extra > lds_cap && a.k1a_lds - (size_t)(ct - 512) * 40 + extra <= lds_cap) {
+                a.k1a_lds -= (size_t)(ct - 512) * 40; ct = 512; a.k1a_ct = ct;
+            }
+            const bool fits = able && a.k1a_lds + extra <= lds_cap;
+            const bool want = ov.k1a_pair ? forced : (kK1aPairDefault && ct >= 512 && p.np <= 512);
+            a.k1a_pair = fits && want;
+            a.k1a_pair_lds = a.k1a_pair ? extra : 0;
+        }
         *out = a;
         return true;
     }
@@ -287,6 +302,7 @@
     int l2 = 0;
     bool sharded = false, hist = false;
     int nsub = 0, pb = 0;
+    bool pair = false;
 };
 struct Kernels {
     PassAKernel k1a;
@@ -302,7 +318,7 @@
     k.sharded = cfg.world > 1;
     if (!p.narrow) { k.family = K1A_WIDE; k.l2 = a.l2_in_lds ? 1 : 0; k.hist = p.hist != 0; return k; }
     k.l2 = a.l2_in_lds ? (a.l2_u16 ? 2 : 1) : 0;
-    if (a.k1a_team) { k.family = K1A_TEAM; k.pb = p.np == 256 ? 8 : p.np == 512 ? 9 : 10; }
+    if (a.k1a_team) { k.family = K1A_TEAM; k.pb = p.np == 256 ? 8 : p.np == 512 ? 9 : 10; k.pair = a.k1a_pair; }
     else { k.family = K1A_TILE; k.nsub = a.k1a_nsub == 2 ? 2 : 1; }
     return k;
 }
@@ -341,6 +357,7 @@
 inline constexpr auto kK1aWideKeys = product({0, 1}, {0, 1}, {0, 1});
 inline constexpr auto kK1aTileKeys = product({0, 1, 2}, {0, 1}, {1, 2});
 inline constexpr auto kK1aTeamKeys = product({0, 1, 2}, {0, 1}, {8, 9, 10});
+inline constexpr auto kK1aTeamPairKeys = product({0, 1, 2}, {0, 1}, {8, 9, 10});
 inline constexpr auto kK1bMergeKeys = concat(product({4, 8}, {0}, {0, 1}), product({4}, {1}, {0, 1}));
 inline constexpr auto kK1bStreamKeys = concat(product({4, 8}, {1, 2, 4}, {0, 1}, {0}, {0, 1}),
                                               product({kK1bWarmU}, {1, 2, 4}, {0, 1}, {1, 2}, {0, 1}));
diff --git a/alaz_amd/csrc/sg_sizes.h b/alaz_amd/csrc/sg_sizes.h
--- a/alaz_amd/csrc/sg_sizes.h
+++ b/alaz_amd/csrc/sg_sizes.h
@@ -8,6 +8,7 @@
 #define K1T_CHUNK   4096u
 #define K1T_TS(NSUB) (K1T_CHUNK * (NSUB))
 #define K1M_LDS_FIXED(np, teams, nt) ((size_t)(np) * 4 * (2 + 4 * (teams)) + 128 + ((size_t)(nt) * 4 + 4) * 8)
+#define K1M_LDS_PAIR_EXTRA(np, teams, nt) ((size_t)(nt) * 4 * 8)
 
 #define K2_TILE 2048
 #define K2_DH_GMAX 128
diff --git a/alaz_amd/engine.py b/alaz_amd/engine.py
--- a/alaz_amd/engine.py
+++ b/alaz_amd/engine.py
@@ -14,7 +14,7 @@
 LIB_DEV_PATH = os.path.join(_HERE, "lib", "libservicegraph_dev.so")
 DEV_KNOBS = ("SG_ABLATE", "SG_NP", "SG_HT", "SG_CT", "SG_NWG", "SG_NSUB", "SG_SPLIT", "SG_WARM", "SG_K1A", "SG_K1_NARROW", "SG_K1_LEGACY", "SG_K1B_U",
              "SG_K1B_THREADS", "SG_K1B_PACK", "SG_K1B_NO_ORDER", "SG_L2_GLOBAL", "SG_L2_U32", "SG_DH_G", "SG_K3_SLICES", "SG_K3_NO_FUSE", "SG_K4_FUSED", "SG_K5_GRID", "SG_K6_ONE_WG", "SG_DENSE_VALU",
-             "SG_COPY_STREAMS", "SG_STAGE_SLOTS", "SG_ARENA", "SG_NO_FOLD")
+             "SG_COPY_STREAMS", "SG_STAGE_SLOTS", "SG_ARENA", "SG_NO_FOLD", "SG_K1A_PAIR")
 
 SG_OK, SG_EINVAL, SG_ENOMEM, SG_ENODEV, SG_ENOSPC, SG_EAGAIN, SG_ESTATE = 0, -22, -12, -19, -28, -11, -71
 SELECT_MAX_K = 16384
@@ -179,6 +179,7 @@
         "sg_window_hist": (I, [H, P, sz, Psz]),
         "sg_geometry_get": (I, [H, C.POINTER(SgGeometry)]),
         "sg_prepare_fold_get": (I, [H, C.POINTER(u32)]),
+        "sg_pass_a_pair_get": (I, [H, C.POINTER(u32)]),
         "sg_comm_unique_id": (I, [P, sz]), "sg_comm_create": (I, [P, sz, I, I, I, PP]),
         "sg_comm_destroy": (I, [P]), "sg_window_run_sharded": (I, [H, P, P]),
         "sg_host_register": (I, [H, P, sz]), "sg_host_unregister": (I, [H, P]), "sg_ingest_pinned": (I, [H, P, sz]),
@@ -478,7 +479,9 @@
         self._ck(self._l.sg_geometry_get(self._h, C.byref(g)))
         fold = C.c_uint32(0)
         self._ck(self._l.sg_prepare_fold_get(self._h, C.byref(fold)))
-        return {**{n: int(getattr(g, n)) for n, _ in SgGeometry._fields_}, "prepare_fold": int(fold.value)}
+        pair = C.c_uint32(0)
+        self._ck(self._l.sg_pass_a_pair_get(self._h, C.byref(pair)))
+        return {**{n: int(getattr(g, n)) for n, _ in SgGeometry._fields_}, "prepare_fold": int(fold.value), "pass_a_pair": int(pair.value)}
 
     def k1_kernels(self) -> tuple:
         g = self.geometry()
diff --git a/include/servicegraph.h b/include/servicegraph.h
--- a/include/servicegraph.h
+++ b/include/servicegraph.h
@@ -479,6 +479,7 @@
 } sg_geometry;
 int sg_geometry_get(sg_handle h, sg_geometry* out);
 int sg_prepare_fold_get(sg_handle h, uint32_t* out);
+int sg_pass_a_pair_get(sg_handle h, uint32_t* out);
 
 int sg_timing_enable(sg_handle h, int on);
 int sg_timing_reset(sg_handle h);
```
